# ZhengdiYu/Arbitrary-Hands-3D-Reconstruction

Hardware: AMD Instinct MI355X
Metric: frames/sec (2-hand mesh) at 512x512 batch-64; vertex L2 vs ref (higher is better)
Workload: dtype f32; 1 GPU; configs[2]: synthetic 512x512 RGB batch=64 per GPU, HRNet-W32 backbone, fp32; frames_per_gpu=64, global_batch=64, parallelism=frame-sharded x1, gather=none (one rank), contexts_in_turn=2

## Files before the change

arbitrary-hands-3d-reconstruction_amd/csrc/acrmi_ops.hip:

```cpp
#include "acrmi_ctx.h"

int decode_maps_impl(const float* l_center, const float* r_center, int center_cs, const float* l_params,
                     const float* r_params, int params_cs, const float* l_prior, const float* r_prior, int prior_cs,
                     int B, float conf_thresh, const int32_t* prior_gate, const unsigned* poison, float* slots, void* stream) {
  if (!l_center || !r_center || !l_params || !r_params || !l_prior || !r_prior || !slots || B <= 0 || params_cs < 109 ||
      prior_cs < 106 || center_cs < 1 || !(conf_thresh == conf_thresh))
    return fail(nullptr, ACRMI_EINVAL, "acrmi_decode_maps: bad arguments");
  DecodeArgs d{};
  d.center[0] = l_center; d.center[1] = r_center; d.center_cs = center_cs;
  d.params[0] = l_params; d.params[1] = r_params; d.params_cs = params_cs;
  d.prior[0] = l_prior; d.prior[1] = r_prior; d.prior_cs = prior_cs;
  d.B = B; d.slots = slots; d.thresh = conf_thresh;
  d.prior_gate = prior_gate;
  d.poison = poison;
  hipError_t e = launch_decode(d, (hipStream_t)stream);
  if (e != hipSuccess) return fail(nullptr, ACRMI_EHIP, "decode launch: %s", hipGetErrorString(e));
  return ACRMI_OK;
}

extern "C" {

int acrmi_decode_maps_gated(const float* l_center, const float* r_center, int center_cs, const float* l_params,
                            const float* r_params, int params_cs, const float* l_prior, const float* r_prior, int prior_cs,
                            int B, float conf_thresh, const int32_t* prior_gate, float* slots, void* stream) {
  return decode_maps_impl(l_center, r_center, center_cs, l_params, r_params, params_cs, l_prior, r_prior, prior_cs, B, conf_thresh,
                          prior_gate, nullptr, slots, stream);
}

int acrmi_decode_maps(const float* l_center, const float* r_center, int center_cs, const float* l_params,
                      const float* r_params, int params_cs, const float* l_prior, const float* r_prior, int prior_cs,
                      int B, float conf_thresh, float* slots, void* stream) {
  return acrmi_decode_maps_gated(l_center, r_center, center_cs, l_params, r_params, params_cs, l_prior, r_prior, prior_cs, B,
                                 conf_thresh, nullptr, slots, stream);
}

int acrmi_conv2d(const float* in, int B, int H, int W, int in_cs, int in_coff, int cin, const float* w_packed,
                 const float* bias, int bias_frame_stride, const float* res, int res_cs, int res_coff, float* out,
                 int out_cs, int out_coff, int cout, int ksize, int stride, int relu, int groups, int algo,
                 void* stream) {
  if (!in || !w_packed || !bias || !out || B <= 0 || H <= 0 || W <= 0 || cin <= 0 || cout <= 0 || groups <= 0)
    return fail(nullptr, ACRMI_EINVAL, "acrmi_conv2d: bad arguments");
  const int bias_map = algo >= 0 ? (algo & ACRMI_CONV_BIAS_MAP) : 0;
  if (algo >= 0) algo &= ~ACRMI_CONV_BIAS_MAP;
  if (bias_map && (!res || algo == 3))
    return fail(nullptr, ACRMI_EINVAL, "acrmi_conv2d: ACRMI_CONV_BIAS_MAP needs res (the map) and an algo other than 3");
  const bool x3s2 = (algo == 6 || algo == 7) && ksize == 3 && stride == 2;
  if (algo != 0 && !x3s2 && !((algo >= 1 && algo <= 7) && (ksize == 3 || (algo >= 6 && ksize == 1)) && stride == (algo == 5 ? 2 : 1)))
    return fail(nullptr, ACRMI_EINVAL, "acrmi_conv2d: algo %d needs a 3x3 stride-%d convolution", algo, algo == 5 ? 2 : 1);
  if (x3s2 && (cin % 32 || cout % 32 || H % 16 || W % 64))
    return fail(nullptr, ACRMI_EINVAL, "acrmi_conv2d: algo 6 / 7 at stride 2 needs Cin %% 32 = 0, Cout %% 32 = 0, H %% 16 == 0, W %% 64 == 0");
  if ((algo == 6 || algo == 7) && !x3s2 && (cin % 32 || cout % 32 || (ksize == 3 ? ((H % 8 || W % 32) && (H % 16 || W % 16)) : ((H * W) % 256 != 0))))
    return fail(nullptr, ACRMI_EINVAL, "acrmi_conv2d: algo 6 / 7 needs Cin %% 32 = 0, Cout %% 32 = 0, H %% 8 == 0, W %% 32 == 0");
  if (algo == 5 && (cin % 16 || cout % 32 || H % 16 || W % 32))
    return fail(nullptr, ACRMI_EINVAL, "acrmi_conv2d: algo 5 needs Cin %% 16 = 0, Cout %% 32 = 0, H %% 16 == 0, W %% 32 == 0");
  if (algo == 3 && (groups != 1 || cin > 32 || cout != 32 || bias_frame_stride != 0 || H % 8 || W % 16 || out_cs % 4 ||
                    out_coff % 4 || (res && (res_cs % 4 || res_coff % 4))))
    return fail(nullptr, ACRMI_EINVAL, "acrmi_conv2d: algo 3 needs groups 1, Cin <= 32, Cout = 32, H %% 8 == 0, W %% 16 == 0");
  if (algo == 4 && (cin < 32 || (cin == 32 && (cout % 32 || H % 8 || W % 32))))
    return fail(nullptr, ACRMI_EINVAL, "acrmi_conv2d: algo 4 needs Cin > 32 (or Cin = 32, Cout %% 32 = 0 on a map of 8x32-pixel tiles)");
  if ((ksize != 1 && ksize != 3) || (stride != 1 && stride != 2))
    return fail(nullptr, ACRMI_EINVAL, "acrmi_conv2d: only 3x3 and 1x1 at stride 1 / 2 are implemented (got k%d s%d)", ksize, stride);
  if (in_cs % 4 || in_coff % 4 || (groups > 1 && cin % 4))
    return fail(nullptr, ACRMI_EINVAL, "acrmi_conv2d: input channel stride/offset must be multiples of 4");
  if (in_coff < 0 || out_coff < 0 || res_coff < 0 || in_coff + groups * cin > in_cs || out_coff + groups * cout > out_cs ||
      (res && res_coff + groups * cout > res_cs) || bias_frame_stride < 0 ||
      (bias_frame_stride > 0 && bias_frame_stride < groups * cout))
    return fail(nullptr, ACRMI_EINVAL, "acrmi_conv2d: channel slice outside its tensor's channel stride");
  ConvArgs a{};
  a.in = in; a.w = w_packed; a.bias = bias; a.res = res; a.out = out;
  a.B = B; a.H = H; a.W = W;
  const int pad = ksize / 2;
  a.Ho = (H + 2 * pad - ksize) / stride + 1; a.Wo = (W + 2 * pad - ksize) / stride + 1;
  a.in_cs = in_cs; a.in_coff = in_coff; a.Cin = cin;
  a.out_cs = out_cs; a.out_coff = out_coff; a.Cout = cout;
  a.res_cs = res_cs; a.res_coff = res_coff;
  a.ks = ksize; a.stride = stride; a.relu = relu; a.groups = groups;
  a.cin8 = (cin + 7) / 8;
  a.n_tiles = cout <= 32 ? 1 : ((cout + 63) / 64) * 2;
  a.bias_fstride = bias_frame_stride;
  a.algo = algo;
  a.res_bcast = bias_map ? 1 : 0;
  hipError_t e = launch_conv(a, (hipStream_t)stream);
  if (e != hipSuccess) return fail(nullptr, ACRMI_EHIP, "conv launch: %s", hipGetErrorString(e));
  return ACRMI_OK;
}

size_t acrmi_conv2d_splitk_workspace(int B, int H, int W, int cout, int splits) {
  if (B <= 0 || H <= 0 || W <= 0 || cout <= 0 || splits < 2) return 0;
  const size_t cnt = (conv_splitk_counters(B, H, W, cout) * sizeof(unsigned) + 255) / 256 * 256;
  return cnt + conv_splitk_ws_floats(B, H, W, cout, splits) * sizeof(float);
}

int acrmi_conv2d_splitk(const float* in, int B, int H, int W, int in_cs, int in_coff, int cin_slice, int splits,
                        const float* w_packed, const float* bias, const float* res, int res_cs, int res_coff, float* out,
                        int out_cs, int out_coff, int cout, int relu, void* workspace, size_t workspace_bytes, void* stream) {
  if (!in || !w_packed || !bias || !out || !workspace || B <= 0 || H <= 0 || W <= 0 || cout <= 0)
    return fail(nullptr, ACRMI_EINVAL, "acrmi_conv2d_splitk: bad arguments");
  if (splits < 2 || splits > 8 || cin_slice < 64 || cin_slice % 32 || cout == 33)
    return fail(nullptr, ACRMI_EINVAL, "acrmi_conv2d_splitk: 2..8 slices of >= 64 channels (a multiple of 32) each; Cout != 33");
  if (in_cs % 4 || in_coff % 4 || in_coff < 0 || out_coff < 0 || res_coff < 0 || in_coff + splits * cin_slice > in_cs ||
      out_coff + cout > out_cs || (res && res_coff + cout > res_cs))
    return fail(nullptr, ACRMI_EINVAL, "acrmi_conv2d_splitk: channel slice outside its tensor's channel stride");
  if (workspace_bytes < acrmi_conv2d_splitk_workspace(B, H, W, cout, splits) || ((uintptr_t)workspace & 15))
    return fail(nullptr, ACRMI_EINVAL, "acrmi_conv2d_splitk: workspace too small (acrmi_conv2d_splitk_workspace) or unaligned");
  ConvArgs a{};
  a.in = in; a.w = w_packed; a.bias = bias; a.res = res; a.out = out;
  a.B = B; a.H = H; a.W = W; a.Ho = H; a.Wo = W;
  a.in_cs = in_cs; a.in_coff = in_coff; a.Cin = cin_slice;
  a.out_cs = out_cs; a.out_coff = out_coff; a.Cout = cout;
  a.res_cs = res_cs; a.res_coff = res_coff;
  a.ks = 3; a.stride = 1; a.relu = relu; a.groups = splits;
  a.cin8 = cin_slice / 8;
  a.n_tiles = cout <= 32 ? 1 : ((cout + 63) / 64) * 2;
  a.algo = 2;
  a.splitk = 1;
  a.split_cnt = reinterpret_cast<unsigned*>(workspace);
  a.split_ws = reinterpret_cast<float*>(reinterpret_cast<char*>(workspace) +
                                        (conv_splitk_counters(B, H, W, cout) * sizeof(unsigned) + 255) / 256 * 256);
  hipError_t e = launch_conv(a, (hipStream_t)stream);
  if (e != hipSuccess) return fail(nullptr, ACRMI_EHIP, "conv launch: %s", hipGetErrorString(e));
  return ACRMI_OK;
}

int acrmi_conv2d_h16(const void* in, int B, int H, int W, int in_cs, int in_coff, int cin, const void* w_packed,
                     const float* bias, int bias_frame_stride, const void* res, int res_cs, int res_coff, void* out,
                     int out_cs, int out_coff, int cout, int ksize, int stride, int relu, int groups, int dtype,
                     int out_f32, void* stream) {
  if (!in || !w_packed || !bias || !out || B <= 0 || H <= 0 || W <= 0 || cin <= 0 || cout <= 0 || groups <= 0 ||
      (dtype != ACRMI_DT_F16 && dtype != ACRMI_DT_BF16))
    return fail(nullptr, ACRMI_EINVAL, "acrmi_conv2d_h16: bad arguments");
  if ((ksize != 1 && ksize != 3) || (stride != 1 && stride != 2) || (out_f32 && stride != 1))
    return fail(nullptr, ACRMI_EINVAL, "acrmi_conv2d_h16: 3x3 and 1x1 at stride 1 / 2 (fp32 output: stride 1 only); got k%d s%d", ksize, stride);
  const int oq = out_f32 ? 4 : 8;
  if (in_cs % 8 || in_coff % 8 || (groups > 1 && cin % 8) || out_cs % oq || (res && res_cs % oq))
    return fail(nullptr, ACRMI_EINVAL, "acrmi_conv2d_h16: channel strides must be multiples of 16 bytes");
  if (in_coff < 0 || out_coff < 0 || res_coff < 0 || in_coff + groups * cin > in_cs || out_coff + groups * cout > out_cs ||
      (res && res_coff + groups * cout > res_cs) || bias_frame_stride < 0 ||
      (bias_frame_stride > 0 && bias_frame_stride < groups * cout))
    return fail(nullptr, ACRMI_EINVAL, "acrmi_conv2d_h16: channel slice outside its tensor's channel stride");
  ConvArgs a{};
  a.in = reinterpret_cast<const float*>(in); a.w = reinterpret_cast<const float*>(w_packed); a.bias = bias;
  a.res = reinterpret_cast<const float*>(res); a.out = reinterpret_cast<float*>(out);
  a.B = B; a.H = H; a.W = W;
  const int pad = ksize / 2;
  a.Ho = (H + 2 * pad - ksize) / stride + 1; a.Wo = (W + 2 * pad - ksize) / stride + 1;
  a.in_cs = in_cs; a.in_coff = in_coff; a.Cin = cin;
  a.out_cs = out_cs; a.out_coff = out_coff; a.Cout = cout;
  a.res_cs = res_cs; a.res_coff = res_coff;
  a.ks = ksize; a.stride = stride; a.relu = relu; a.groups = groups;
  a.cin8 = (cin + 15) / 16;
  a.n_tiles = cout <= 32 ? 1 : ((cout + 63) / 64) * 2;
  a.bias_fstride = bias_frame_stride;
  a.algo = 0; a.dtype = dtype; a.out_f32 = out_f32 ? 1 : 0;
  hipError_t e = launch_conv(a, (hipStream_t)stream);
  if (e != hipSuccess) return fail(nullptr, ACRMI_EHIP, "conv launch: %s", hipGetErrorString(e));
  return ACRMI_OK;
}

int acrmi_preprocess(const uint8_t* bgr_dev, int n, int H, int W, uint8_t* out_rgb_dev, float* offsets_host,
                     void* stream) {
  if (!bgr_dev || !out_rgb_dev || n <= 0 || H <= 0 || W <= 0)
    return fail(nullptr, ACRMI_EINVAL, "acrmi_preprocess: bad arguments");
  const int S = H > W ? H : W;
  int top = 0, right = 0, bottom = 0, left = 0;
  if (W < H) { const int d = H - W; right = (d + 1) / 2; left = d / 2; }
  else if (H < W) { const int d = W - H; top = d / 2; bottom = (d + 1) / 2; }
  if (offsets_host) {
    for (int i = 0; i < n; ++i) {
      float* o = offsets_host + (size_t)i * 10;
      o[0] = (float)S; o[1] = (float)S; o[2] = o[3] = o[4] = o[5] = 0.f;
      o[6] = (float)top; o[7] = (float)right; o[8] = (float)bottom; o[9] = (float)left;
    }
  }
  hipError_t e = launch_preprocess(bgr_dev, n, H, W, S, top, left, 512, out_rgb_dev, (hipStream_t)stream);
  return e == hipSuccess ? ACRMI_OK : fail(nullptr, ACRMI_EHIP, "preprocess: %s", hipGetErrorString(e));
}

int acrmi_preprocess_frames(const acrmi_frame* frames_host, int n, uint8_t* out_rgb_dev, float* offsets_host, void* stream) {
  if (!frames_host || !out_rgb_dev || n <= 0) return fail(nullptr, ACRMI_EINVAL, "acrmi_preprocess_frames: bad arguments");
  for (int i = 0; i < n; ++i)
    if (!frames_host[i].bgr_dev || frames_host[i].H <= 0 || frames_host[i].W <= 0)
      return fail(nullptr, ACRMI_EINVAL, "acrmi_preprocess_frames: frame %d: null pointer or empty size (%d x %d)", i,
                  frames_host[i].H, frames_host[i].W);
  for (int i0 = 0; i0 < n; i0 += PRE_FRAMES_PER_LAUNCH) {
    const int m = n - i0 < PRE_FRAMES_PER_LAUNCH ? n - i0 : PRE_FRAMES_PER_LAUNCH;
    PreBatch pb{};
    for (int i = 0; i < m; ++i) {
      const acrmi_frame& fr = frames_host[i0 + i];
      pb.f[i].bgr = fr.bgr_dev; pb.f[i].H = fr.H; pb.f[i].W = fr.W;
      if (offsets_host) {
        const int H = fr.H, W = fr.W, S = H > W ? H : W;
        int top = 0, right = 0, bottom = 0, left = 0;
        if (W < H) { const int d = H - W; right = (d + 1) / 2; left = d / 2; }
        else if (H < W) { const int d = W - H; top = d / 2; bottom = (d + 1) / 2; }
        float* o = offsets_host + (size_t)(i0 + i) * 10;
        o[0] = (float)S; o[1] = (float)S; o[2] = o[3] = o[4] = o[5] = 0.f;
        o[6] = (float)top; o[7] = (float)right; o[8] = (float)bottom; o[9] = (float)left;
      }
    }
    hipError_t e = launch_preprocess_frames(pb, m, 512, out_rgb_dev + (size_t)i0 * 512 * 512 * 3, (hipStream_t)stream);
    if (e != hipSuccess) return fail(nullptr, ACRMI_EHIP, "preprocess_frames: %s", hipGetErrorString(e));
  }
  return ACRMI_OK;
}

}

namespace {

const int32_t kNv12Matrix[5][6] = {
    {1220542, 2116026, -409993, -852492, 1673527, 16},
    {1220945, 2115221, -410793, -852458, 1673555, 16},
    {1048576, 1858077, -360853, -748826, 1470104, 0},
    {1220945, 2215014, -223607, -558796, 1879825, 16},
    {1048576, 1945738, -196424, -490864, 1651297, 0},
};

int nv12_coef(const char* who, const int32_t* coef6, Nv12Coef& k) {
  const int32_t* c = coef6 ? coef6 : kNv12Matrix[0];
  auto mag = [](int32_t v) { return v < 0 ? -(long long)v : (long long)v; };
  long long m = mag(c[1]);
  if (mag(c[4]) > m) m = mag(c[4]);
  if (mag(c[2]) + mag(c[3]) > m) m = mag(c[2]) + mag(c[3]);
  if (c[5] < 0 || c[5] > 255)
    return fail(nullptr, ACRMI_EINVAL, "%s: y_off %d outside 0..255", who, (int)c[5]);
  if (255 * mag(c[0]) + 128 * m + (1LL << 19) >= (1LL << 31))
    return fail(nullptr, ACRMI_EINVAL, "%s: coefficient row (%d, %d, %d, %d, %d) could overflow the int32 sums", who, (int)c[0],
                (int)c[1], (int)c[2], (int)c[3], (int)c[4]);
  k.cy = c[0]; k.cub = c[1]; k.cug = c[2]; k.cvg = c[3]; k.cvr = c[4]; k.y_off = c[5];
  return ACRMI_OK;
}

int nv12_check_frames(const char* who, const acrmi_nv12_frame* fr, int n) {
  for (int i = 0; i < n; ++i) {
    const acrmi_nv12_frame& f = fr[i];
    if (!f.y_dev || !f.uv_dev) return fail(nullptr, ACRMI_EINVAL, "%s: frame %d: null plane", who, i);
    if (f.H < 2 || f.W < 2 || (f.H & 1) || (f.W & 1))
      return fail(nullptr, ACRMI_EINVAL, "%s: frame %d: size %d x %d (H x W) must be even and >= 2", who, i, f.H, f.W);
    if (f.y_pitch < f.W || f.uv_pitch < f.W)
      return fail(nullptr, ACRMI_EINVAL, "%s: frame %d: pitch (y %d, uv %d) below the width %d", who, i, f.y_pitch, f.uv_pitch, f.W);
  }
  return ACRMI_OK;
}

}

extern "C" {

int acrmi_nv12_matrix(int which, int32_t coef6[6]) {
  if (!coef6 || which < 0 || which > ACRMI_NV12_BT709_FULL)
    return fail(nullptr, ACRMI_EINVAL, "acrmi_nv12_matrix: bad arguments (matrix %d)", which);
  for (int i = 0; i < 6; ++i) coef6[i] = kNv12Matrix[which][i];
  return ACRMI_OK;
}

int acrmi_preprocess_nv12(const acrmi_nv12_frame* frames_host, int n, const int32_t* coef6_host, uint8_t* out_rgb_dev,
                          float* offsets_host, void* stream) {
  if (!frames_host || !out_rgb_dev || n <= 0) return fail(nullptr, ACRMI_EINVAL, "acrmi_preprocess_nv12: bad arguments");
  Nv12Coef k{};
  int rc = nv12_coef("acrmi_preprocess_nv12", coef6_host, k);
  if (rc == ACRMI_OK) rc = nv12_check_frames("acrmi_preprocess_nv12", frames_host, n);
  if (rc != ACRMI_OK) return rc;
  for (int i0 = 0; i0 < n; i0 += NV12_FRAMES_PER_LAUNCH) {
    const int m = n - i0 < NV12_FRAMES_PER_LAUNCH ? n - i0 : NV12_FRAMES_PER_LAUNCH;
    Nv12Batch pb{};
    for (int i = 0; i < m; ++i) {
      const acrmi_nv12_frame& fr = frames_host[i0 + i];
      pb.f[i].y = fr.y_dev; pb.f[i].uv = fr.uv_dev; pb.f[i].H = fr.H; pb.f[i].W = fr.W;
      pb.f[i].y_pitch = fr.y_pitch; pb.f[i].uv_pitch = fr.uv_pitch;
      if (offsets_host) {
        const int H = fr.H, W = fr.W, S = H > W ? H : W;
        int top = 0, right = 0, bottom = 0, left = 0;
        if (W < H) { const int d = H - W; right = (d + 1) / 2; left = d / 2; }
        else if (H < W) { const int d = W - H; top = d / 2; bottom = (d + 1) / 2; }
        float* o = offsets_host + (size_t)(i0 + i) * 10;
        o[0] = (float)S; o[1] = (float)S; o[2] = o[3] = o[4] = o[5] = 0.f;
        o[6] = (float)top; o[7] = (float)right; o[8] = (float)bottom; o[9] = (float)left;
      }
    }
    hipError_t e = launch_preprocess_nv12(pb, k, m, 512, out_rgb_dev + (size_t)i0 * 512 * 512 * 3, (hipStream_t)stream);
    if (e != hipSuccess) return fail(nullptr, ACRMI_EHIP, "preprocess_nv12: %s", hipGetErrorString(e));
  }
  return ACRMI_OK;
}

int acrmi_nv12_to_rgb(const acrmi_nv12_frame* frames_host, int n, const int32_t* coef6_host, int bgr,
                      uint8_t* const* dst_dev_host, void* stream) {
  if (!frames_host || !dst_dev_host || n <= 0) return fail(nullptr, ACRMI_EINVAL, "acrmi_nv12_to_rgb: bad arguments");
  Nv12Coef k{};
  int rc = nv12_coef("acrmi_nv12_to_rgb", coef6_host, k);
  if (rc == ACRMI_OK) rc = nv12_check_frames("acrmi_nv12_to_rgb", frames_host, n);
  if (rc != ACRMI_OK) return rc;
  for (int i = 0; i < n; ++i)
    if (!dst_dev_host[i]) return fail(nullptr, ACRMI_EINVAL, "acrmi_nv12_to_rgb: frame %d: null destination", i);
  for (int i0 = 0; i0 < n; i0 += NV12_FRAMES_PER_LAUNCH) {
    const int m = n - i0 < NV12_FRAMES_PER_LAUNCH ? n - i0 : NV12_FRAMES_PER_LAUNCH;
    Nv12DstBatch pb{};
    for (int i = 0; i < m; ++i) {
      const acrmi_nv12_frame& fr = frames_host[i0 + i];
      pb.f[i].y = fr.y_dev; pb.f[i].uv = fr.uv_dev; pb.f[i].dst = dst_dev_host[i0 + i]; pb.f[i].H = fr.H; pb.f[i].W = fr.W;
      pb.f[i].y_pitch = fr.y_pitch; pb.f[i].uv_pitch = fr.uv_pitch;
    }
    hipError_t e = launch_nv12_to_rgb(pb, k, m, bgr ? 1 : 0, (hipStream_t)stream);
    if (e != hipSuccess) return fail(nullptr, ACRMI_EHIP, "nv12_to_rgb: %s", hipGetErrorString(e));
  }
  return ACRMI_OK;
}

int acrmi_u8norm(const uint8_t* img, int n_pixels, float* out, void* stream) {
  if (!img || !out || n_pixels <= 0) return fail(nullptr, ACRMI_EINVAL, "acrmi_u8norm: bad arguments");
  hipError_t e = launch_u8norm(img, n_pixels, out, (hipStream_t)stream);
  return e == hipSuccess ? ACRMI_OK : fail(nullptr, ACRMI_EHIP, "u8norm: %s", hipGetErrorString(e));
}

int acrmi_bilinear2x(const float* in, int B, int H, int W, int in_cs, int C, float* out, int out_cs, void* stream) {
  if (!in || !out || B <= 0 || H < 2 || W < 2 || C % 4 || in_cs % 4 || out_cs % 4)
    return fail(nullptr, ACRMI_EINVAL, "acrmi_bilinear2x: bad arguments");
  hipError_t e = launch_bilinear2x(in, B, H, W, in_cs, 0, C, out, out_cs, 0, (hipStream_t)stream);
  return e == hipSuccess ? ACRMI_OK : fail(nullptr, ACRMI_EHIP, "bilinear2x: %s", hipGetErrorString(e));
}

int acrmi_fuse_sum(int nterms, const float* const* terms, const int* term_cs, const int* term_shift, int B, int H,
                   int W, int C, float* out, int out_cs, int relu, void* stream) {
  if (nterms < 1 || nterms > 4 || !terms || !term_cs || !term_shift || !out || C % 4)
    return fail(nullptr, ACRMI_EINVAL, "acrmi_fuse_sum: bad arguments");
  FuseArgs f{};
  f.nterms = nterms; f.B = B; f.H = H; f.W = W; f.C = C; f.out = out; f.out_cs = out_cs; f.relu = relu;
  for (int t = 0; t < nterms; ++t) { f.term[t] = terms[t]; f.cs[t] = term_cs[t]; f.shift[t] = term_shift[t]; }
  hipError_t e = launch_fuse_sum(f, (hipStream_t)stream);
  return e == hipSuccess ? ACRMI_OK : fail(nullptr, ACRMI_EHIP, "fuse_sum: %s", hipGetErrorString(e));
}

int acrmi_stem_conv(const uint8_t* img, int B, int H, int W, const float* w_packed, const float* bias, float* out,
                    int out_cs, int out_coff, int relu, void* stream) {
  if (!img || !w_packed || !bias || !out || B <= 0 || !stem_shape_ok(H, W, out_cs, out_coff))
    return fail(nullptr, ACRMI_EINVAL, "acrmi_stem_conv: bad arguments (H %% 16, W %% 128, 64 channels inside out_cs)");
  hipError_t e = launch_stem(img, B, H, W, w_packed, bias, out, out_cs, out_coff, relu, (hipStream_t)stream);
  return e == hipSuccess ? ACRMI_OK : fail(nullptr, ACRMI_EHIP, "stem: %s", hipGetErrorString(e));
}

size_t acrmi_attpool_ws_floats(int B, int C) { return B > 0 && C > 0 ? attpool_ws_floats(B, C) : 0; }

int acrmi_attpool(const float* segm, int segm_cs, const float* feat, int feat_cs, int C, int B, float* ws,
                  float* pooled, void* stream) {
  if (!segm || !feat || !ws || !pooled || B <= 0) return fail(nullptr, ACRMI_EINVAL, "acrmi_attpool: bad arguments");
  hipError_t e = launch_attpool(segm, segm_cs, feat, feat_cs, C, B, 128, 128, ws, pooled, (hipStream_t)stream);
  return e == hipSuccess ? ACRMI_OK : fail(nullptr, ACRMI_EHIP, "attpool: %s", hipGetErrorString(e));
}

int acrmi_parebias(const float* pooled, int C, int part0, const float* lc_w, const float* lin_w, const float* lin_b,
                   const float* mix_wp, const float* mix_b, int B, float* out, int out_stride, void* stream) {
  if (!pooled || !lc_w || !lin_w || !lin_b || !mix_wp || !mix_b || !out || B <= 0 || (C != 256 && C != 320) ||
      (part0 != 0 && part0 != 16) || out_stride < 109 || out_stride > 256)
    return fail(nullptr, ACRMI_EINVAL, "acrmi_parebias: bad arguments");
  PareArgs a{};
  a.pooled = pooled; a.lc_w = lc_w; a.lin_w = lin_w; a.lin_b = lin_b; a.mix_wp = mix_wp; a.mix_b = mix_b;
  a.out = out; a.B = B; a.C = C; a.part0 = part0; a.out_stride = out_stride;
  hipError_t e = launch_parebias(a, (hipStream_t)stream);
  return e == hipSuccess ? ACRMI_OK : fail(nullptr, ACRMI_EHIP, "parebias: %s", hipGetErrorString(e));
}

int acrmi_cam_trans(const float* joints_dev, const float* pj2d_dev, int n, float focal_length, float img_size,
                    float* trans_dev, void* stream) {
  if (n < 0 || (n > 0 && (!joints_dev || !pj2d_dev || !trans_dev)) || !(focal_length > 0.f) || !(img_size > 0.f))
    return fail(nullptr, ACRMI_EINVAL, "acrmi_cam_trans: bad arguments");
  hipError_t e = launch_cam_trans(joints_dev, pj2d_dev, n, focal_length, img_size, trans_dev, (hipStream_t)stream);
  return e == hipSuccess ? ACRMI_OK : fail(nullptr, ACRMI_EHIP, "cam_trans: %s", hipGetErrorString(e));
}

int acrmi_mesh_topology(const int32_t* faces_host, int n_faces, int n_verts, int32_t* blob_host, int n_ints) {
  if (n_faces <= 0 || n_verts <= 0) return fail(nullptr, ACRMI_EINVAL, "acrmi_mesh_topology: bad arguments");
  const long long need = mesh_topology_ints(n_faces, n_verts);
  if (need > 0x7fffffffll) return fail(nullptr, ACRMI_EINVAL, "acrmi_mesh_topology: mesh too large");
  if (!blob_host) return (int)need;
  if (!faces_host || n_ints < need) return fail(nullptr, ACRMI_EINVAL, "acrmi_mesh_topology: bad arguments (%lld ints needed)", need);
  if (!build_mesh_topology(faces_host, n_faces, n_verts, blob_host))
    return fail(nullptr, ACRMI_EINVAL, "acrmi_mesh_topology: a face names a vertex outside [0, %d)", n_verts);
  return (int)need;
}

size_t acrmi_render_workspace(int n_meshes, int n_faces) {
  return n_meshes > 0 && n_faces > 0 ? render_workspace_bytes(n_meshes, n_faces) : 0;
}

int acrmi_rasterize(const float* verts_dev, const float* trans_dev, int n_meshes, int n_verts, int n_faces,
                    const int32_t* topo_dev, const int32_t* topo2_dev, const int32_t* mesh_topo_dev,
                    const int32_t* mesh_frame_dev, const float* rgb_dev, const float* view_dev, float focal,
                    float visible_weight, const uint8_t* img_in_dev, uint8_t* img_out_dev, int n_frames, int H, int W,
                    int32_t* ids_out_dev, void* ws_dev, void* stream) {
  if (!verts_dev || !topo_dev || !mesh_frame_dev || !rgb_dev || !img_in_dev || !img_out_dev || !ws_dev || n_meshes <= 0 ||
      n_verts <= 0 || n_verts > RENDER_MAX_VERTS || n_faces <= 0 || n_frames <= 0 || H <= 0 || W <= 0 || H > 16384 || W > 16384 ||
      (long long)n_meshes * n_faces > 0x7fffffffll || n_frames > 65535 || !(focal > 0.f) ||
      !(visible_weight >= 0.f && visible_weight <= 1.f))
    return fail(nullptr, ACRMI_EINVAL, "acrmi_rasterize: bad arguments");
  RenderArgs a{};
  a.verts = verts_dev; a.trans = trans_dev; a.topo[0] = topo_dev; a.topo[1] = topo2_dev; a.mesh_topo = mesh_topo_dev;
  a.mesh_frame = mesh_frame_dev; a.rgb = rgb_dev; a.view = view_dev; a.focal = focal; a.visible_weight = visible_weight;
  a.img_in = img_in_dev; a.img_out = img_out_dev; a.ids_out = ids_out_dev; a.ws = (char*)ws_dev;
  a.n_meshes = n_meshes; a.n_verts = n_verts; a.n_faces = n_faces; a.n_frames = n_frames; a.H = H; a.W = W;
  hipError_t e = launch_render(a, (hipStream_t)stream);
  return e == hipSuccess ? ACRMI_OK : fail(nullptr, ACRMI_EHIP, "rasterize: %s", hipGetErrorString(e));
}

int acrmi_overlay_tables(int bgr, uint8_t* colors_host, uint8_t* lut_host) {
  if (colors_host) skeleton_default_colors(bgr != 0, colors_host);
  if (lut_host) heatmap_default_lut(bgr != 0, lut_host);
  return ACRMI_OK;
}

static bool overlay_image_ok(int n, int H, int W) {
  return n > 0 && n <= OVERLAY_MAX_FRAMES && H > 0 && W > 0 && H <= OVERLAY_MAX_DIM && W <= OVERLAY_MAX_DIM;
}

int acrmi_draw_skeletons(const float* kps_dev, const int32_t* hand_frame_dev, int n_hands, const uint8_t* colors_host, int bgr,
                         int line_width, int circle_rad, const uint8_t* img_in_dev, uint8_t* img_out_dev, int n_frames, int H,
                         int W, void* stream) {
  if (!kps_dev || !hand_frame_dev || !img_in_dev || !img_out_dev || n_hands <= 0 || !overlay_image_ok(n_frames, H, W) ||
      line_width < 1 || line_width > OVERLAY_MAX_WIDTH || circle_rad < 0 || circle_rad > OVERLAY_MAX_RAD)
    return fail(nullptr, ACRMI_EINVAL, "acrmi_draw_skeletons: bad arguments (line_width 1..%d, circle_rad 0..%d, H, W <= %d)",
                OVERLAY_MAX_WIDTH, OVERLAY_MAX_RAD, OVERLAY_MAX_DIM);
  SkeletonArgs a{};
  a.kps = kps_dev; a.hand_frame = hand_frame_dev; a.n_hands = n_hands; a.n_frames = n_frames; a.H = H; a.W = W;
  a.line_width = line_width; a.circle_rad = circle_rad; a.img_in = img_in_dev; a.img_out = img_out_dev;
  if (colors_host) std::memcpy(a.colors, colors_host, 63);
  else skeleton_default_colors(bgr != 0, a.colors);
  hipError_t e = launch_skeleton(a, (hipStream_t)stream);
  return e == hipSuccess ? ACRMI_OK : fail(nullptr, ACRMI_EHIP, "draw_skeletons: %s", hipGetErrorString(e));
}

int acrmi_draw_heatmaps(const float* maps_l_dev, const float* maps_r_dev, long long frame_stride, int n, int h, int w,
                        const float* view_dev, float weight, const uint8_t* lut_host, int bgr, const uint8_t* img_in_dev,
                        uint8_t* out_l_dev, uint8_t* out_r_dev, int H, int W, void* stream) {
  if (!maps_l_dev || !img_in_dev || !out_l_dev || (maps_r_dev != nullptr) != (out_r_dev != nullptr) || out_l_dev == out_r_dev ||
      (out_r_dev && out_r_dev == img_in_dev) || !overlay_image_ok(n, H, W) || h <= 0 || w <= 0 || h > OVERLAY_MAX_DIM ||
      w > OVERLAY_MAX_DIM || frame_stride < (long long)h * w || !(weight >= 0.f && weight <= 1.f))
    return fail(nullptr, ACRMI_EINVAL, "acrmi_draw_heatmaps: bad arguments");
  HeatmapArgs a{};
  a.maps[0] = maps_l_dev; a.maps[1] = maps_r_dev; a.frame_stride = frame_stride; a.pix_stride = 1; a.dtype = ACRMI_DT_F32;
  a.n = n; a.h = h; a.w = w; a.H = H; a.W = W; a.view = view_dev; a.weight = weight; a.img_in = img_in_dev;
  a.out[0] = out_l_dev; a.out[1] = out_r_dev;
  if (lut_host) std::memcpy(a.lut, lut_host, 768);
  else heatmap_default_lut(bgr != 0, a.lut);
  hipError_t e = launch_heatmap(a, (hipStream_t)stream);
  return e == hipSuccess ? ACRMI_OK : fail(nullptr, ACRMI_EHIP, "draw_heatmaps: %s", hipGetErrorString(e));
}

}
```

arbitrary-hands-3d-reconstruction_amd/csrc/acrmi_program.hip:

```cpp
#include "acrmi_ctx.h"

void free_program(acrmi_ctx* c) {
  for (hipEvent_t e : c->op_ev)
    if (e) (void)hipEventDestroy(e);
  c->op_ev.clear();
  for (float* p : c->buf_ptr)
    if (p) (void)hipFree(p);
  c->buf_ptr.clear();
  c->bufs.clear();
  c->ops.clear();
  for (int l = 0; l < MAX_LANES; ++l) {
    if (c->split_ws[l]) (void)hipFree(c->split_ws[l]);
    if (c->split_cnt[l]) (void)hipFree(c->split_cnt[l]);
    c->split_ws[l] = nullptr; c->split_cnt[l] = nullptr;
  }
  c->split_ws_floats = c->split_counters = 0;
  if (c->att_ws) (void)hipFree(c->att_ws);
  c->att_ws = nullptr;
  if (c->picks) (void)hipFree(c->picks);
  c->picks = nullptr;
  if (c->gate_buf) (void)hipFree(c->gate_buf);
  c->gate_buf = nullptr;
  if (c->range_flag) (void)hipFree(c->range_flag);
  c->range_flag = nullptr;
  c->have_program = false;
  c->last_batch = 0;
}


int run_op(acrmi_ctx* c, const acrmi_op& op, const uint8_t* img, int B, hipStream_t s, int lane) {
  auto ptr = [&](int id) -> float* { return id >= 0 ? c->buf_ptr[id] : nullptr; };
  auto desc = [&](int id) -> const acrmi_buffer_desc& { return c->bufs[id]; };
  auto eptr = [&](int id, int coff) -> float* {
    if (id < 0) return nullptr;
    return reinterpret_cast<float*>(reinterpret_cast<char*>(c->buf_ptr[id]) + (size_t)coff * (c->bufs[id].dtype ? 2 : 4));
  };
  switch (op.kind) {
    case ACRMI_OP_U8NORM: {
      const auto& d = desc(op.out_buf);
      HIPCHK(c, launch_u8norm(img, (long)B * d.h * d.w, ptr(op.out_buf), s));
      return ACRMI_OK;
    }
    case ACRMI_OP_STEM: {
      const auto& d = desc(op.out_buf);
      if (op.ksize == 7) {
        if (d.dtype)
          HIPCHK(c, launch_stem7_h16(img, B, 2 * d.h, 2 * d.w, c->weights + op.w_off, c->weights + op.b_off, ptr(op.out_buf),
                                     d.cs, op.out_coff, op.relu, d.dtype, s));
        else
          HIPCHK(c, launch_stem7(img, B, 2 * d.h, 2 * d.w, c->weights + op.w_off, c->weights + op.b_off, ptr(op.out_buf), d.cs,
                                 op.out_coff, op.relu, s));
        return ACRMI_OK;
      }
      if (d.dtype)
        HIPCHK(c, launch_stem_h16(img, B, 2 * d.h, 2 * d.w, c->weights + op.w_off, c->weights + op.b_off, ptr(op.out_buf),
                                  d.cs, op.out_coff, op.relu, d.dtype, s));
      else
        HIPCHK(c, launch_stem(img, B, 2 * d.h, 2 * d.w, c->weights + op.w_off, c->weights + op.b_off, ptr(op.out_buf), d.cs,
                              op.out_coff, op.relu, s));
      return ACRMI_OK;
    }
    case ACRMI_OP_CONV: {
      const auto& di = desc(op.in_buf);
      const auto& dout = desc(op.out_buf);
      ConvArgs a{};
      a.in = ptr(op.in_buf);
      a.w = c->weights + op.w_off;
      a.bias = op.bias_per_frame ? ptr(op.aux_buf) : c->weights + op.b_off;
      a.res = ptr(op.res_buf);
      a.out = ptr(op.out_buf);
      a.B = B; a.H = di.h; a.W = di.w; a.Ho = dout.h; a.Wo = dout.w;
      a.in_cs = di.cs; a.in_coff = op.in_coff; a.Cin = op.cin;
      a.out_cs = dout.cs; a.out_coff = op.out_coff; a.Cout = op.cout;
      a.res_cs = op.res_buf >= 0 ? desc(op.res_buf).cs : 0; a.res_coff = op.res_coff;
      if (op.flags & ACRMI_CONV_SPLITK) {
        a.splitk = 1; a.split_ws = c->split_ws[lane]; a.split_cnt = c->split_cnt[lane];
      }
      if (op.flags & ACRMI_CONV_BIAS_MAP) {
        a.res = c->weights + op.w_off2; a.res_cs = (op.groups * op.cout + 3) / 4 * 4; a.res_coff = 0; a.res_bcast = 1;
      }
      a.ks = op.ksize; a.stride = op.stride; a.relu = op.relu; a.groups = op.groups;
      a.cin8 = (op.cin + 7) / 8;
      a.n_tiles = op.cout <= 32 ? 1 : ((op.cout + 63) / 64) * 2;
      a.bias_fstride = op.bias_per_frame ? desc(op.aux_buf).cs : 0;
      a.nxt = op.nterms;
      for (int t = 0; t < op.nterms && t < 3; ++t) {
        a.xt[t] = ptr(op.term_buf[t]);
        a.xt_cs[t] = desc(op.term_buf[t]).cs; a.xt_coff[t] = op.term_coff[t]; a.xt_shift[t] = op.term_shift[t];
      }
      if (op.flags & ACRMI_CONV_DUAL) {
        a.out2 = ptr(op.aux_buf); a.out2_cs = desc(op.aux_buf).cs; a.out2_coff = 0;
      }
      a.algo = op.flags & 7;
      a.range_flag = a.algo == 6 ? c->range_flag : nullptr;
      a.dtype = di.dtype;
      a.out_f32 = di.dtype != ACRMI_DT_F32 && dout.dtype == ACRMI_DT_F32;
      HIPCHK(c, launch_conv(a, s));
      return ACRMI_OK;
    }
    case ACRMI_OP_FUSESUM: {
      const auto& dout = desc(op.out_buf);
      FuseArgs f{};
      f.nterms = op.nterms; f.B = B; f.H = dout.h; f.W = dout.w; f.C = op.cout; f.out_cs = dout.cs; f.relu = op.relu;
      f.out = eptr(op.out_buf, op.out_coff);
      for (int t = 0; t < op.nterms; ++t) {
        f.term[t] = eptr(op.term_buf[t], op.term_coff[t]);
        f.cs[t] = desc(op.term_buf[t]).cs;
        f.shift[t] = op.term_shift[t];
      }
      if (dout.dtype) HIPCHK(c, launch_fuse_sum_h16(f, dout.dtype, s));
      else HIPCHK(c, launch_fuse_sum(f, s));
      return ACRMI_OK;
    }
    case ACRMI_OP_BILINEAR2X: {
      const auto& di = desc(op.in_buf);
      if (di.dtype)
        HIPCHK(c, launch_bilinear2x_h16(ptr(op.in_buf), B, di.h, di.w, di.cs, op.in_coff, op.cin, ptr(op.out_buf),
                                        desc(op.out_buf).cs, op.out_coff, di.dtype, s));
      else
        HIPCHK(c, launch_bilinear2x(ptr(op.in_buf), B, di.h, di.w, di.cs, op.in_coff, op.cin, ptr(op.out_buf),
                                    desc(op.out_buf).cs, op.out_coff, s));
      return ACRMI_OK;
    }
    case ACRMI_OP_PAIR1X1: {
      const auto& di = desc(op.in_buf);
      HIPCHK(c, launch_pair1x1(ptr(op.in_buf), di.cs, op.in_coff, ptr(op.res_buf), desc(op.res_buf).cs, op.res_coff, ptr(op.out_buf),
                               desc(op.out_buf).cs, op.out_coff, ptr(op.aux_buf), desc(op.aux_buf).cs, 0, c->weights + op.w_off,
                               (long)B * di.h * di.w, s));
      return ACRMI_OK;
    }
    case ACRMI_OP_MAXPOOL: {
      const auto& di = desc(op.in_buf);
      if (di.dtype)
        HIPCHK(c, launch_maxpool3s2_h16(ptr(op.in_buf), B, di.h, di.w, di.cs, op.in_coff, op.cin, ptr(op.out_buf),
                                        desc(op.out_buf).cs, op.out_coff, di.dtype, s));
      else
        HIPCHK(c, launch_maxpool3s2(ptr(op.in_buf), B, di.h, di.w, di.cs, op.in_coff, op.cin, ptr(op.out_buf),
                                    desc(op.out_buf).cs, op.out_coff, s));
      return ACRMI_OK;
    }
    case ACRMI_OP_POW11: {
      const auto& d = desc(op.out_buf);
      if (d.dtype) HIPCHK(c, launch_pow11_h16(ptr(op.out_buf), (long)B * d.h * d.w, d.cs, op.out_coff, d.dtype, s));
      else HIPCHK(c, launch_pow11(ptr(op.out_buf), (long)B * d.h * d.w, d.cs, op.out_coff, s));
      return ACRMI_OK;
    }
    case ACRMI_OP_ATTPOOL: {
      const auto& ds = desc(op.in_buf);
      const auto& df = desc(op.res_buf);
      HIPCHK(c, launch_attpool(ptr(op.in_buf), ds.cs, eptr(op.res_buf, op.res_coff), df.cs, op.cin, B, df.h, df.w,
                               c->att_ws, ptr(op.out_buf), s, df.dtype));
      return ACRMI_OK;
    }
    case ACRMI_OP_PAREBIAS: {
      PareArgs p{};
      p.pooled = ptr(op.in_buf);
      p.lc_w = c->weights + op.w_off;
      p.lin_w = c->weights + op.w_off2;
      p.lin_b = c->weights + op.b_off2;
      p.mix_wp = c->weights + op.w_off3;
      p.mix_b = c->weights + op.b_off;
      p.out = ptr(op.out_buf);
      p.B = B; p.C = op.cin; p.part0 = op.flags; p.out_stride = desc(op.out_buf).cs;
      HIPCHK(c, launch_parebias(p, s));
      return ACRMI_OK;
    }
    case ACRMI_OP_COORDFILL: {
      const auto& d = desc(op.out_buf);
      if (d.dtype) HIPCHK(c, launch_coordfill_h16(ptr(op.out_buf), c->max_batch, d.h, d.w, d.cs, op.out_coff, d.dtype, s));
      else HIPCHK(c, launch_coordfill(ptr(op.out_buf), c->max_batch, d.h, d.w, d.cs, op.out_coff, s));
      return ACRMI_OK;
    }
    case ACRMI_OP_POINTHEADS: {
      const acrmi_head_layout& h = c->heads;
      const int side = op.flags & 1;
      PointArgs p{};
      p.x34 = ptr(op.in_buf); p.x_cs = desc(op.in_buf).cs;
      p.center[0] = ptr(h.center_buf[0]); p.center[1] = ptr(h.center_buf[1]); p.center_cs = desc(h.center_buf[0]).cs;
      p.w = c->weights + op.w_off;
      p.mix_w = c->weights + op.w_off2;
      p.bias = ptr(op.aux_buf); p.bias_stride = desc(op.aux_buf).cs;
      p.p109 = ptr(op.res_buf); p.p109_cs = desc(op.res_buf).cs;
      p.prior = ptr(h.prior_buf[side]); p.prior_cs = desc(h.prior_buf[side]).cs;
      p.final_ = ptr(op.out_buf); p.final_cs = desc(op.out_buf).cs;
      p.picks = c->picks; p.side = side; p.B = B; p.thresh = c->conf_thresh;
      p.prior_when_both = c->batch_prior ? 1 : 0;
      HIPCHK(c, launch_point_heads(p, s));
      return ACRMI_OK;
    }
    default:
      return fail(c, ACRMI_EINVAL, "unknown op kind %d", op.kind);
  }
}

bool op_active(const acrmi_op& op, bool point) {
  return op.kind != ACRMI_OP_COORDFILL && op.mode != (point ? ACRMI_MODE_DENSE : ACRMI_MODE_POINT);
}

static void op_rw(const acrmi_ctx* c, const acrmi_op& op, std::vector<int>& R, std::vector<int>& W) {
  R.clear(); W.clear();
  const int n_bufs = (int)c->bufs.size();
  auto r = [&](int id) { if (id >= 0) R.push_back(id); };
  auto w = [&](int id) { if (id >= 0) W.push_back(id); };
  switch (op.kind) {
    case ACRMI_OP_U8NORM: case ACRMI_OP_STEM: w(op.out_buf); break;
    case ACRMI_OP_CONV:
      r(op.in_buf); r(op.res_buf); if (op.bias_per_frame) r(op.aux_buf);
      for (int t = 0; t < op.nterms; ++t) r(op.term_buf[t]);
      w(op.out_buf);
      if (op.flags & ACRMI_CONV_DUAL) w(op.aux_buf);
      break;
    case ACRMI_OP_FUSESUM: for (int t = 0; t < op.nterms; ++t) r(op.term_buf[t]); w(op.out_buf); break;
    case ACRMI_OP_BILINEAR2X: case ACRMI_OP_MAXPOOL: r(op.in_buf); w(op.out_buf); break;
    case ACRMI_OP_PAIR1X1: r(op.in_buf); r(op.res_buf); w(op.out_buf); w(op.aux_buf); break;
    case ACRMI_OP_POW11: r(op.out_buf); w(op.out_buf); break;
    case ACRMI_OP_ATTPOOL: r(op.in_buf); r(op.res_buf); w(op.out_buf); w(n_bufs); break;
    case ACRMI_OP_PAREBIAS: r(op.in_buf); w(op.out_buf); break;
    case ACRMI_OP_POINTHEADS:
      r(op.in_buf); r(op.aux_buf); r(c->heads.center_buf[0]); r(c->heads.center_buf[1]);
      w(op.res_buf); w(op.out_buf); w(c->heads.prior_buf[op.flags & 1]); w(n_bufs + 1);
      break;
    default: break;
  }
}

void build_schedule(acrmi_ctx* c, bool point, bool large) {
  Schedule& S = c->sched[point ? 1 : 0][large ? 1 : 0];
  const int n = (int)c->ops.size(), nb = (int)c->bufs.size() + 2;
  S = Schedule();
  S.deps.assign(n, std::vector<int>());
  S.leaf.assign(n, 1);
  std::vector<int> last_writer(nb, -1), R, W;
  std::vector<std::vector<int>> readers(nb);
  for (int j = 0; j < n; ++j) {
    if (!op_active(c->ops[j], point)) continue;
    S.order.push_back(j);
    op_rw(c, c->ops[j], R, W);
    std::vector<int>& deps = S.deps[j];
    auto dep = [&](int i) { if (i >= 0 && i != j && std::find(deps.begin(), deps.end(), i) == deps.end()) deps.push_back(i); };
    for (int b : R) dep(last_writer[b]);
    for (int b : W) { dep(last_writer[b]); for (int i : readers[b]) dep(i); }
    for (int b : R) readers[b].push_back(j);
    for (int b : W) { last_writer[b] = j; readers[b].clear(); }
    for (int d : deps) S.leaf[d] = 0;
  }
  const int want = c->want_lanes > 0 ? c->want_lanes : (large ? AUTO_LANES_LARGE : AUTO_LANES_SMALL);
  const int max_lanes = std::max(1, std::min(want, MAX_LANES));
  S.lane.assign(n, 0);
  S.wait.assign(n, std::vector<int>());
  S.signal.assign(n, 0);
  std::vector<int> lane_tail(max_lanes, -1);
  const std::vector<float>& ms = c->op_ms[point ? 1 : 0];
  const bool planned = c->lane_plan && !large && max_lanes > 1 && (int)ms.size() == n;
  constexpr float SYNC_MS = 0.002f, EVENT_MS = 0.002f;
  static const float WAIT_MS = experiment_env("ACRMI_PLAN_WAIT_US") ? 1e-3f * (float)atof(experiment_env("ACRMI_PLAN_WAIT_US")) : 0.016f;
  std::vector<float> fin(planned ? n : 0, 0.f), lane_free(max_lanes, 0.f);
  static const bool rank_order = !(experiment_env("ACRMI_PLAN_RANK") && atoi(experiment_env("ACRMI_PLAN_RANK")) == 0);
  if (planned && rank_order) {
    std::vector<float> ru(n, 0.f);
    std::vector<std::vector<int>> succ(n);
    for (int j : S.order)
      for (int d : S.deps[j]) succ[d].push_back(j);
    for (int k = (int)S.order.size() - 1; k >= 0; --k) {
      const int j = S.order[k];
      float m = 0.f;
      for (int s2 : succ[j]) m = std::max(m, ru[s2]);
      ru[j] = m + std::max(ms[j], 1e-4f);
    }
    std::stable_sort(S.order.begin(), S.order.end(), [&](int x, int y) { return ru[x] > ru[y]; });
  }
  std::vector<int> pos(n, -1);
  for (int k = 0; k < (int)S.order.size(); ++k) pos[S.order[k]] = k;
  for (int j : S.order) {
    int lane = -1;
    if (planned) {
      float best = 0.f;
      bool best_prod = false;
      for (int l = 0; l < max_lanes; ++l) {
        float start = lane_free[l];
        unsigned others = 0;
        bool prod = false;
        for (int d : S.deps[j]) {
          if (S.lane[d] == l) { prod = true; continue; }
          others |= 1u << S.lane[d];
          start = std::max(start, fin[d] + WAIT_MS);
        }
        start += SYNC_MS * (float)__builtin_popcount(others);
        if (lane < 0 || start < best - 1e-6f || (start < best + 1e-6f && prod && !best_prod)) { lane = l; best = start; best_prod = prod; }
      }
      fin[j] = best + std::max(ms[j] - EVENT_MS, 0.002f);
      lane_free[lane] = fin[j] + 0.5f * SYNC_MS;
      S.n_lanes = std::max(S.n_lanes, lane + 1);
    } else {
      for (int d : S.deps[j])
        if (lane_tail[S.lane[d]] == d) { lane = S.lane[d]; break; }
      if (lane < 0) {
        if (S.n_lanes < max_lanes) lane = S.n_lanes++;
        else lane = (int)(std::min_element(lane_tail.begin(), lane_tail.end()) - lane_tail.begin());
      }
    }
    S.lane[j] = lane;
    std::vector<int> latest(max_lanes, -1);
    for (int d : S.deps[j])
      if (S.lane[d] != lane && (latest[S.lane[d]] < 0 || pos[d] > pos[latest[S.lane[d]]])) latest[S.lane[d]] = d;
    for (int l = 0; l < max_lanes; ++l)
      if (latest[l] >= 0) { S.wait[j].push_back(latest[l]); S.signal[latest[l]] = 1; }
    lane_tail[lane] = j;
  }
  if (getenv("ACRMI_DEBUG_SCHED")) {
    std::vector<int> depth(n, 0);
    int edges = 0, maxd = 0;
    for (int j : S.order) {
      for (int d : S.deps[j]) depth[j] = std::max(depth[j], depth[d] + 1);
      edges += (int)S.deps[j].size();
      maxd = std::max(maxd, depth[j] + 1);
    }
    int waits = 0;
    for (int j : S.order) waits += (int)S.wait[j].size();
    fprintf(stderr, "[acrmi] schedule(%s, %s batches, %s): %zu ops, %d edges, critical path %d ops; %d lanes, %d cross-lane waits\n",
            point ? "point" : "dense", large ? "large" : "small", planned ? "planned from measured op times" : "structural",
            S.order.size(), edges, maxd, S.n_lanes, waits);
  }
}


extern "C" {

int acrmi_set_program(acrmi_ctx* c, const acrmi_buffer_desc* bufs, int n_bufs, const acrmi_op* ops, int n_ops,
                      const acrmi_head_layout* heads, int max_batch) {
  if (!c || !bufs || !ops || !heads || n_bufs <= 0 || n_ops <= 0 || max_batch <= 0)
    return fail(c, ACRMI_EINVAL, "acrmi_set_program: bad arguments");
  if (!c->weights) return fail(c, ACRMI_ESTATE, "acrmi_set_program: load weights first");
  ON_DEVICE(c);
  int prog_dt = ACRMI_DT_F32;
  for (int i = 0; i < n_bufs; ++i) {
    const auto& d = bufs[i];
    if (d.dtype < ACRMI_DT_F32 || d.dtype > ACRMI_DT_BF16) return fail(c, ACRMI_EINVAL, "buffer %d: unknown dtype %d", i, d.dtype);
    if (d.h <= 0 || d.w <= 0 || d.cs <= 0 || d.cs % (d.dtype ? 8 : 4)) return fail(c, ACRMI_EINVAL, "buffer %d: bad geometry", i);
    if (d.dtype) {
      if (prog_dt && prog_dt != d.dtype) return fail(c, ACRMI_EINVAL, "buffer %d: f16 and bf16 buffers in one program", i);
      prog_dt = d.dtype;
    }
  }
  auto bdt = [&](int id) { return id >= 0 ? bufs[id].dtype : (int)ACRMI_DT_F32; };
  auto buf_ok = [&](int id) { return id >= 0 && id < n_bufs; };
  auto w_ok = [&](long long off, long long n) { return off >= 0 && n >= 0 && (unsigned long long)(off + n) <= c->n_weights; };
  {
    const int hb[8] = {heads->center_buf[0], heads->center_buf[1], heads->params_buf[0], heads->params_buf[1],
                       heads->prior_buf[0], heads->prior_buf[1], heads->segm_buf, heads->backbone_buf};
    for (int id : hb)
      if (!buf_ok(id)) return fail(c, ACRMI_EINVAL, "head layout references buffer %d of %d", id, n_bufs);
    for (int k = 0; k < 7; ++k)
      if (bufs[hb[k]].dtype != ACRMI_DT_F32) return fail(c, ACRMI_EINVAL, "head layout: head maps must be fp32 buffers");
    if (bufs[heads->params_buf[0]].cs < 109 || bufs[heads->params_buf[1]].cs < 109 || bufs[heads->prior_buf[0]].cs < 106 ||
        bufs[heads->prior_buf[1]].cs < 106)
      return fail(c, ACRMI_EINVAL, "head layout: params/prior buffers are too narrow");
    for (int k = 0; k < 6; ++k)
      if (bufs[hb[k]].h != 64 || bufs[hb[k]].w != 64) return fail(c, ACRMI_EINVAL, "head layout: head maps must be 64x64");
  }
  for (int i = 0; i < n_ops; ++i) {
    const acrmi_op& op = ops[i];
    const int ids[4] = {op.in_buf, op.out_buf, op.res_buf, op.aux_buf};
    for (int id : ids)
      if (id >= n_bufs || id < -1) return fail(c, ACRMI_EINVAL, "op %d references buffer %d of %d", i, id, n_bufs);
    if (op.mode < ACRMI_MODE_BOTH || op.mode > ACRMI_MODE_POINT) return fail(c, ACRMI_EINVAL, "op %d: bad mode", i);
    bool need_in = false, need_out = true;
    switch (op.kind) {
      case ACRMI_OP_U8NORM: case ACRMI_OP_POW11: case ACRMI_OP_COORDFILL: case ACRMI_OP_STEM: break;
      case ACRMI_OP_CONV: case ACRMI_OP_BILINEAR2X: case ACRMI_OP_MAXPOOL: case ACRMI_OP_PAIR1X1: case ACRMI_OP_ATTPOOL: case ACRMI_OP_PAREBIAS: case ACRMI_OP_POINTHEADS:
        need_in = true;
        break;
      case ACRMI_OP_FUSESUM: break;
      default: return fail(c, ACRMI_EINVAL, "op %d: unknown kind %d", i, op.kind);
    }
    if ((need_in && !buf_ok(op.in_buf)) || (need_out && !buf_ok(op.out_buf)))
      return fail(c, ACRMI_EINVAL, "op %d (kind %d): missing input/output buffer", i, op.kind);
    if (op.in_coff < 0 || op.out_coff < 0 || op.res_coff < 0) return fail(c, ACRMI_EINVAL, "op %d: negative channel offset", i);
    if (op.kind == ACRMI_OP_CONV) {
      const int idt = bufs[op.in_buf].dtype, odt = bufs[op.out_buf].dtype;
      if (op.in_coff % (idt ? 8 : 4) || (op.ksize != 1 && op.ksize != 3) || op.stride < 1 || op.stride > 2 || op.cin <= 0 || op.cout <= 0 ||
          op.groups <= 0)
        return fail(c, ACRMI_EINVAL, "op %d: unsupported conv geometry", i);
      const int algo = op.flags & 7;
      if (algo > 7) return fail(c, ACRMI_EINVAL, "op %d: unknown conv algo %d", i, algo);
      if (idt ? (algo != 0 || (odt != idt && odt != ACRMI_DT_F32) || (odt == ACRMI_DT_F32 && op.stride != 1) ||
                 (op.groups > 1 && op.cin % 2))
              : odt != ACRMI_DT_F32)
        return fail(c, ACRMI_EINVAL, "op %d: conv buffer types do not fit (in %d, out %d, algo %d)", i, idt, odt, algo);
      if (op.res_buf >= 0 && bufs[op.res_buf].dtype != odt)
        return fail(c, ACRMI_EINVAL, "op %d: the residual must have the type of the output", i);
      const bool splitk = (op.flags & ACRMI_CONV_SPLITK) != 0;
      if (splitk && (algo != 2 || idt || op.groups < 2 || op.groups > 8 || op.cin % 32 || op.cin < 64 || op.cout == 33 ||
                     op.bias_per_frame))
        return fail(c, ACRMI_EINVAL, "op %d: split-K needs algo 2, fp32, 2..8 slices of Cin %% 32 == 0, Cin >= 64 channels each", i);
      if (op.flags & ACRMI_CONV_BIAS_MAP) {
        const long long mcs = (op.groups * op.cout + 3) / 4 * 4;
        if (splitk || op.res_buf >= 0 || idt || algo == 3 || !w_ok(op.w_off2, (long long)bufs[op.out_buf].h * bufs[op.out_buf].w * mcs))
          return fail(c, ACRMI_EINVAL, "op %d: a position-bias map needs an fp32 conv without a residual buffer (not algo 3) and "
                      "[Ho][Wo][round4(groups*Cout)] floats inside the blob at w_off2", i);
      }
      const bool dual = (op.flags & ACRMI_CONV_DUAL) != 0;
      if (dual && (algo != 3 || op.nterms < 1 || op.bias_per_frame || !buf_ok(op.aux_buf) || bufs[op.aux_buf].dtype != ACRMI_DT_F32 ||
                   bufs[op.aux_buf].h != bufs[op.out_buf].h || bufs[op.aux_buf].w != bufs[op.out_buf].w || bufs[op.aux_buf].cs % 4 ||
                   bufs[op.aux_buf].cs < op.cout || op.aux_buf == op.out_buf || op.aux_buf == op.in_buf || op.aux_buf == op.res_buf))
        return fail(c, ACRMI_EINVAL, "op %d: a second output needs algo 3, 1..3 terms and an fp32 map of the output's size in aux_buf", i);
      if (op.nterms) {
        const int ho_ = bufs[op.out_buf].h, wo_ = bufs[op.out_buf].w;
        if (op.nterms < 0 || op.nterms > 3 || idt || (op.flags & ACRMI_CONV_BIAS_MAP) || splitk ||
            (dual ? false : (op.ksize != 3 || op.stride != 2 || (algo != 0 && algo != 5) || op.cout % 32 || op.cin <= 16 ||
                             op.out_coff % 4 || bufs[op.out_buf].cs % 4)))
          return fail(c, ACRMI_EINVAL, "op %d: extra residual terms need an fp32 3x3 stride-2 convolution (algo 0 / 5) with Cin > 16, "
                      "Cout %% 32 = 0 and 16-byte aligned output channels - or ACRMI_CONV_DUAL", i);
        for (int t = 0; t < op.nterms; ++t) {
          const int tb = op.term_buf[t];
          if (!buf_ok(tb) || bufs[tb].dtype != ACRMI_DT_F32 || op.term_coff[t] < 0 || op.term_coff[t] % 4 || bufs[tb].cs % 4 ||
              op.term_shift[t] < 0 || op.term_shift[t] > 3 || op.term_coff[t] + op.groups * op.cout > bufs[tb].cs ||
              (bufs[tb].h << op.term_shift[t]) != ho_ || (bufs[tb].w << op.term_shift[t]) != wo_ || tb == op.out_buf ||
              (dual && tb == op.aux_buf))
            return fail(c, ACRMI_EINVAL, "op %d: residual term %d does not fit the output", i, t);
        }
      }
      if (op.bias_per_frame && buf_ok(op.aux_buf) && bufs[op.aux_buf].dtype != ACRMI_DT_F32)
        return fail(c, ACRMI_EINVAL, "op %d: the per-frame bias must be fp32", i);
      if (algo != 0 && !((algo == 6 || algo == 7) && op.ksize == 3 && op.stride == 2) &&
          !((op.ksize == 3 || (algo >= 6 && op.ksize == 1)) && op.stride == (algo == 5 ? 2 : 1)))
        return fail(c, ACRMI_EINVAL, "op %d: algo %d needs a 3x3 stride-%d convolution", i, algo, algo == 5 ? 2 : 1);
      if (algo == 3 && (op.groups != 1 || op.cin > 32 || op.cout != 32 || op.bias_per_frame || bufs[op.out_buf].h % 8 ||
                        bufs[op.out_buf].w % 16 || op.out_coff % 4 || op.res_coff % 4))
        return fail(c, ACRMI_EINVAL, "op %d: algo 3 needs groups 1, Cin <= 32, Cout = 32, a map of 8x16-pixel tiles", i);
      const int ogroups = splitk ? 1 : op.groups;
      if (op.in_coff + op.groups * op.cin > bufs[op.in_buf].cs || op.out_coff + ogroups * op.cout > bufs[op.out_buf].cs ||
          (op.res_buf >= 0 && op.res_coff + ogroups * op.cout > bufs[op.res_buf].cs) ||
          (op.groups > 1 && op.cin % (bufs[op.in_buf].dtype == ACRMI_DT_F32 ? 4 : 8)))
        return fail(c, ACRMI_EINVAL, "op %d: channel slice outside its buffer's channel stride", i);
      const int pad = op.ksize / 2;
      const int ho = (bufs[op.in_buf].h + 2 * pad - op.ksize) / op.stride + 1, wo = (bufs[op.in_buf].w + 2 * pad - op.ksize) / op.stride + 1;
      if (ho != bufs[op.out_buf].h || wo != bufs[op.out_buf].w ||
          (op.res_buf >= 0 && (bufs[op.res_buf].h != ho || bufs[op.res_buf].w != wo)))
        return fail(c, ACRMI_EINVAL, "op %d: output/residual buffer geometry does not match the convolution", i);
      const long long n_tiles = op.cout <= 32 ? 1 : ((op.cout + 63) / 64) * 2;
      if (algo == 4 && (op.cin < 32 || (op.cin == 32 && (op.cout % 32 || ho % 8 || wo % 32))))
        return fail(c, ACRMI_EINVAL, "op %d: algo 4 needs Cin > 32, or Cin = 32 with Cout %% 32 = 0 on a map of 8x32-pixel tiles", i);
      if ((algo == 6 || algo == 7) && op.stride == 2 &&
          (op.ksize != 3 || ho % 8 || wo % 32 || bufs[op.in_buf].h != 2 * ho || bufs[op.in_buf].w != 2 * wo || op.nterms > 0))
        return fail(c, ACRMI_EINVAL, "op %d: algo 6 / 7 at stride 2 needs a 3x3 convolution onto a map of 8x32-pixel tiles, even input size, no extra residual terms", i);
      if ((algo == 6 || algo == 7) && (idt || op.cin % 32 || op.cout % 32 || op.out_coff % 4 || op.res_coff % 4 ||
                                       (op.ksize == 3 ? ((ho % 8 || wo % 32) && (ho % 16 || wo % 16)) : ((ho * wo) % 256 != 0))))
        return fail(c, ACRMI_EINVAL, "op %d: algo 6 / 7 needs fp32 storage, Cin %% 32 = 0, Cout %% 32 = 0, a map of 8x32- or 16x16-pixel tiles (3x3) / of whole 256-pixel items (1x1)", i);
      if (algo == 5 && (idt || op.cin % 16 || op.cout % 32 || bufs[op.in_buf].h % 2 || bufs[op.in_buf].w % 2 || ho % 8 || wo % 16 ||
                        op.out_coff % 4 || op.res_coff % 4))
        return fail(c, ACRMI_EINVAL, "op %d: algo 5 needs fp32, Cin %% 16 = 0, Cout %% 32 = 0, an output map of 8x16-pixel tiles", i);
      const long long taps = algo >= 6 ? op.ksize * op.ksize : algo == 5 ? 28 : algo == 4 ? 24 : (algo >= 2 ? 16 : (algo == 1 ? 12 : op.ksize * op.ksize));
      const long long ksteps = idt ? (op.cin + 15) / 16 : (op.cin + 7) / 8;
      const long long wn = algo == 3 ? 16384 : (long long)op.groups * taps * ksteps * n_tiles * 256 + (algo >= 6 ? 1 : 0);
      if (!w_ok(op.w_off, wn)) return fail(c, ACRMI_EINVAL, "op %d: packed weights outside the blob", i);
      if (op.bias_per_frame) {
        if (!buf_ok(op.aux_buf) || bufs[op.aux_buf].cs < op.groups * op.cout)
          return fail(c, ACRMI_EINVAL, "op %d: per-frame bias buffer missing or too narrow", i);
      } else if (!w_ok(op.b_off, (long long)op.groups * n_tiles * 32)) {
        return fail(c, ACRMI_EINVAL, "op %d: bias outside the blob", i);
      }
    }
    if (op.kind == ACRMI_OP_STEM) {
      if (bufs[op.out_buf].dtype && (bufs[op.out_buf].cs % 8 || op.out_coff % 8))
        return fail(c, ACRMI_EINVAL, "op %d: a 16-bit stem output needs channel stride / offset in multiples of 8", i);
      if (op.ksize != 3 && op.ksize != 7) return fail(c, ACRMI_EINVAL, "op %d: the stem kernels are 3x3 and 7x7 (stride 2)", i);
      const bool ok = op.ksize == 7 ? stem7_shape_ok(2 * bufs[op.out_buf].h, 2 * bufs[op.out_buf].w, bufs[op.out_buf].cs, op.out_coff)
                                    : stem_shape_ok(2 * bufs[op.out_buf].h, 2 * bufs[op.out_buf].w, bufs[op.out_buf].cs, op.out_coff);
      if (op.cout != 64 || !ok)
        return fail(c, ACRMI_EINVAL, "op %d: the stem kernel needs 64 output channels and a map of 8x64-pixel strips", i);
      if (!w_ok(op.w_off, (op.ksize == 7 ? 74 : 14) * 2 * 64) || !w_ok(op.b_off, 64))
        return fail(c, ACRMI_EINVAL, "op %d: stem weights outside the blob", i);
    }
    if (op.kind == ACRMI_OP_FUSESUM) {
      const int vq = bufs[op.out_buf].dtype ? 8 : 4;
      if (op.nterms < 1 || op.nterms > 4 || op.cout <= 0 || op.cout % vq || op.out_coff % vq || op.out_coff + op.cout > bufs[op.out_buf].cs)
        return fail(c, ACRMI_EINVAL, "op %d: bad fuse-sum geometry", i);
      for (int t = 0; t < op.nterms; ++t) {
        if (!buf_ok(op.term_buf[t]) || op.term_coff[t] < 0 || bufs[op.term_buf[t]].dtype != bufs[op.out_buf].dtype ||
            op.term_coff[t] % vq || op.term_shift[t] < 0 || op.term_shift[t] > 3 ||
            op.term_coff[t] + op.cout > bufs[op.term_buf[t]].cs ||
            (bufs[op.term_buf[t]].h << op.term_shift[t]) != bufs[op.out_buf].h ||
            (bufs[op.term_buf[t]].w << op.term_shift[t]) != bufs[op.out_buf].w)
          return fail(c, ACRMI_EINVAL, "op %d: fuse-sum term %d does not fit the output", i, t);
      }
    }
    if (op.kind == ACRMI_OP_PAIR1X1) {
      if (!buf_ok(op.res_buf) || !buf_ok(op.aux_buf) || op.cin != 64 || op.cout != 256)
        return fail(c, ACRMI_EINVAL, "op %d: the 1x1 pair is 64 -> 256 (+ residual) -> 64 with in, res, out and aux buffers", i);
      const int ids4[4] = {op.in_buf, op.res_buf, op.out_buf, op.aux_buf};
      for (int id : ids4)
        if (bufs[id].dtype != ACRMI_DT_F32 || bufs[id].h != bufs[op.in_buf].h || bufs[id].w != bufs[op.in_buf].w)
          return fail(c, ACRMI_EINVAL, "op %d: the 1x1 pair's buffers must be fp32 maps of one size", i);
      if (op.in_coff % 4 || op.res_coff % 4 || op.out_coff % 4 || op.in_coff + 64 > bufs[op.in_buf].cs ||
          op.res_coff + 256 > bufs[op.res_buf].cs || op.out_coff + 256 > bufs[op.out_buf].cs || bufs[op.aux_buf].cs < 64 ||
          op.out_buf == op.in_buf || op.aux_buf == op.in_buf || op.aux_buf == op.out_buf || op.aux_buf == op.res_buf)
        return fail(c, ACRMI_EINVAL, "op %d: the 1x1 pair's channel slices do not fit / its buffers alias", i);
      if (!w_ok(op.w_off, PAIR1X1_FLOATS)) return fail(c, ACRMI_EINVAL, "op %d: pair weights outside the blob", i);
    }
    if (op.kind == ACRMI_OP_MAXPOOL) {
      const int vq = bufs[op.in_buf].dtype ? 8 : 4;
      if (op.cin <= 0 || bufs[op.in_buf].dtype != bufs[op.out_buf].dtype || op.cin % vq || op.in_coff % vq || op.out_coff % vq ||
          op.in_coff + op.cin > bufs[op.in_buf].cs || op.out_coff + op.cin > bufs[op.out_buf].cs ||
          bufs[op.out_buf].h != (bufs[op.in_buf].h - 1) / 2 + 1 || bufs[op.out_buf].w != (bufs[op.in_buf].w - 1) / 2 + 1)
        return fail(c, ACRMI_EINVAL, "op %d: bad max-pool geometry", i);
    }
    if (op.kind == ACRMI_OP_BILINEAR2X &&
        (op.cin <= 0 || bufs[op.in_buf].dtype != bufs[op.out_buf].dtype || op.cin % (bufs[op.in_buf].dtype ? 8 : 4) ||
         op.in_coff % (bufs[op.in_buf].dtype ? 8 : 4) || op.out_coff % (bufs[op.in_buf].dtype ? 8 : 4) || op.in_coff + op.cin > bufs[op.in_buf].cs ||
         op.out_coff + op.cin > bufs[op.out_buf].cs || bufs[op.out_buf].h != 2 * bufs[op.in_buf].h ||
         bufs[op.out_buf].w != 2 * bufs[op.in_buf].w))
      return fail(c, ACRMI_EINVAL, "op %d: bad bilinear geometry", i);
    if ((op.kind == ACRMI_OP_POW11 && op.out_coff >= bufs[op.out_buf].cs) ||
        (op.kind == ACRMI_OP_COORDFILL && op.out_coff + 2 > bufs[op.out_buf].cs))
      return fail(c, ACRMI_EINVAL, "op %d: channel outside the buffer", i);
    if (op.kind == ACRMI_OP_ATTPOOL) {
      if (buf_ok(op.res_buf) && (bufs[op.in_buf].dtype != ACRMI_DT_F32 || bufs[op.out_buf].dtype != ACRMI_DT_F32 ||
                                 (bufs[op.res_buf].dtype != ACRMI_DT_F32 && op.cin != 256)))
        return fail(c, ACRMI_EINVAL, "op %d: attention pooling reads fp32 logits, writes fp32, and pools 256 channels of a 16-bit map", i);
      if (!buf_ok(op.res_buf) || (op.cin != 32 && op.cin != 64 && op.cin != 256 && op.cin != 320) ||
          op.res_coff + op.cin > bufs[op.res_buf].cs || bufs[op.in_buf].cs < 33 || bufs[op.in_buf].h != 2 * bufs[op.res_buf].h ||
          bufs[op.in_buf].w != 2 * bufs[op.res_buf].w || (long long)bufs[op.out_buf].h * bufs[op.out_buf].w * bufs[op.out_buf].cs < 32LL * op.cin)
        return fail(c, ACRMI_EINVAL, "op %d: bad attention-pool geometry", i);
    }
    if ((op.kind == ACRMI_OP_PAREBIAS || op.kind == ACRMI_OP_POINTHEADS || op.kind == ACRMI_OP_U8NORM) &&
        (bdt(op.in_buf) || bdt(op.out_buf) || bdt(op.res_buf) || bdt(op.aux_buf)))
      return fail(c, ACRMI_EINVAL, "op %d (kind %d): fp32 buffers only", i, op.kind);
    if (op.kind == ACRMI_OP_PAREBIAS) {
      const long long shape_n = (op.cin == 320 ? 64 : 256) * 16;
      if ((op.cin != 256 && op.cin != 320) || (op.flags != 0 && op.flags != 16) || bufs[op.out_buf].cs < 109 || bufs[op.out_buf].cs > 256 ||
          (long long)bufs[op.in_buf].h * bufs[op.in_buf].w * bufs[op.in_buf].cs < 32LL * op.cin || !w_ok(op.w_off, 6 * 256 * 16) ||
          !w_ok(op.w_off2, 10 * shape_n) || !w_ok(op.b_off2, 10) || !w_ok(op.w_off3, 109 * 106) || !w_ok(op.b_off, 109))
        return fail(c, ACRMI_EINVAL, "op %d: bad pare-bias geometry or weights", i);
    }
    if (op.kind == ACRMI_OP_POINTHEADS) {
      const bool ok = buf_ok(op.res_buf) && buf_ok(op.aux_buf) &&
                      bufs[op.in_buf].h == 128 && bufs[op.in_buf].w == 128 && bufs[op.in_buf].cs == 36 &&
                      bufs[op.res_buf].h == 64 && bufs[op.out_buf].h == 64 && bufs[op.res_buf].cs >= 109 &&
                      bufs[op.out_buf].cs >= 109 && bufs[op.aux_buf].cs >= 109 && op.mode == ACRMI_MODE_POINT &&
                      w_ok(op.w_off, 3LL * TP_TOWER_FLOATS) && w_ok(op.w_off2, 109LL * TP_EXIT_N);
      if (!ok) return fail(c, ACRMI_EINVAL, "op %d: unsupported point-heads geometry", i);
    }
  }
  free_program(c);
  c->bufs.assign(bufs, bufs + n_bufs);
  c->ops.assign(ops, ops + n_ops);
  c->heads = *heads;
  c->max_batch = max_batch;
  c->buf_ptr.assign(n_bufs, nullptr);
  for (int i = 0; i < n_bufs; ++i) {
    const auto& d = bufs[i];
    const size_t bytes = (size_t)max_batch * d.h * d.w * d.cs * (d.dtype ? 2 : sizeof(float));
    hipError_t e = hipMalloc(&c->buf_ptr[i], bytes);
    if (e != hipSuccess) return fail(c, ACRMI_ENOMEM, "hipMalloc(%zu) for buffer %d: %s", bytes, i, hipGetErrorString(e));
    HIPCHK(c, hipMemset(c->buf_ptr[i], 0, bytes));
  }
  for (int i = 0; i < n_ops; ++i) {
    const acrmi_op& op = ops[i];
    if (op.kind != ACRMI_OP_CONV || !(op.flags & ACRMI_CONV_SPLITK)) continue;
    const auto& d = bufs[op.out_buf];
    c->split_ws_floats = std::max(c->split_ws_floats, conv_splitk_ws_floats(max_batch, d.h, d.w, op.cout, op.groups));
    c->split_counters = std::max(c->split_counters, conv_splitk_counters(max_batch, d.h, d.w, op.cout));
  }
  if (c->split_ws_floats)
    for (int l = 0; l < MAX_LANES; ++l) {
      HIPCHK(c, hipMalloc(&c->split_ws[l], c->split_ws_floats * sizeof(float)));
      HIPCHK(c, hipMalloc(&c->split_cnt[l], c->split_counters * sizeof(unsigned)));
      HIPCHK(c, hipMemset(c->split_cnt[l], 0, c->split_counters * sizeof(unsigned)));
    }
  c->att_ws_floats = attpool_ws_floats(max_batch, 320);
  HIPCHK(c, hipMalloc(&c->att_ws, c->att_ws_floats * sizeof(float)));
  HIPCHK(c, hipMalloc(&c->picks, (size_t)max_batch * 4 * sizeof(int)));
  HIPCHK(c, hipMalloc(&c->gate_buf, (size_t)max_batch * sizeof(int)));
  for (int i = 0; i < n_ops; ++i)
    if (ops[i].kind == ACRMI_OP_CONV && (ops[i].flags & 7) == 6 && !c->range_flag) {
      HIPCHK(c, hipMalloc(&c->range_flag, sizeof(unsigned)));
      HIPCHK(c, hipMemset(c->range_flag, 0, sizeof(unsigned)));
    }
  c->op_ms[0].clear(); c->op_ms[1].clear();
  for (int v = 0; v < 4; ++v) build_schedule(c, v & 1, v & 2);
  c->op_ev.assign(n_ops, nullptr);
  c->have_program = true;
  for (const acrmi_op& op : c->ops)
    if (op.kind == ACRMI_OP_COORDFILL) {
      int r = run_op(c, op, nullptr, max_batch, nullptr);
      if (r) return r;
    }
  HIPCHK(c, hipDeviceSynchronize());
  return ACRMI_OK;
}

}

static unsigned lane_event_flags() {
  static const unsigned f = [] {
    const char* e = experiment_env("ACRMI_EVENT_FLAGS");
    if (e) fprintf(stderr, "[acrmi] WARNING: ACRMI_EVENT_FLAGS=%s - lane events created with non-default flags (experiment)\n", e);
    return hipEventDisableTiming | (e ? (unsigned)strtoul(e, nullptr, 16) : 0u);
  }();
  return f;
}

static int run_program_lanes(acrmi_ctx* c, const uint8_t* img, int B, hipStream_t user, bool point) {
  const Schedule& S = c->sched[point ? 1 : 0][B > AUTO_SMALL_BATCH ? 1 : 0];
  for (int l = 1; l < S.n_lanes; ++l) {
    if (!c->lanes[l]) HIPCHK(c, hipStreamCreateWithFlags(&c->lanes[l], hipStreamNonBlocking));
    if (!c->join_ev[l]) HIPCHK(c, hipEventCreateWithFlags(&c->join_ev[l], lane_event_flags()));
  }
  if (!c->fork_ev) HIPCHK(c, hipEventCreateWithFlags(&c->fork_ev, lane_event_flags()));
  auto st = [&](int l) { return l == 0 ? user : c->lanes[l]; };
  HIPCHK(c, hipEventRecord(c->fork_ev, user));
  for (int l = 1; l < S.n_lanes; ++l) HIPCHK(c, hipStreamWaitEvent(c->lanes[l], c->fork_ev, 0));
  int r = ACRMI_OK;
  for (int j : S.order) {
    hipStream_t s = st(S.lane[j]);
    static const int ablate = [] {
      const char* e = experiment_env("ACRMI_ABLATE_LANE_SYNC");
      const int v = e ? atoi(e) : 0;
      if (v) fprintf(stderr, "[acrmi] WARNING: ACRMI_ABLATE_LANE_SYNC=%d - cross-lane synchronisation is DISABLED, results are WRONG "
                             "(timing experiment only)\n", v);
      return v;
    }();
    if (!(ablate & 1)) for (int d : S.wait[j]) HIPCHK(c, hipStreamWaitEvent(s, c->op_ev[d], 0));
    r = run_op(c, c->ops[j], img, B, s, S.lane[j]);
    if (r) break;
    if (S.signal[j] && !(ablate & 2)) {
      if (!c->op_ev[j]) HIPCHK(c, hipEventCreateWithFlags(&c->op_ev[j], lane_event_flags()));
      HIPCHK(c, hipEventRecord(c->op_ev[j], s));
    }
  }
  for (int l = 1; l < S.n_lanes; ++l) {
    HIPCHK(c, hipEventRecord(c->join_ev[l], c->lanes[l]));
    HIPCHK(c, hipStreamWaitEvent(user, c->join_ev[l], 0));
  }
  return r;
}

int run_program(acrmi_ctx* c, const uint8_t* img, int B, void* stream, bool point, int first_op) {
  if (!c || (!img && first_op <= 0)) return fail(c, ACRMI_EINVAL, "acrmi_backbone_heads: bad arguments");
  if (!c->have_program) return fail(c, ACRMI_ESTATE, "acrmi_backbone_heads: no program");
  if (B <= 0 || B > c->max_batch) return fail(c, ACRMI_EINVAL, "batch %d outside 1..%d", B, c->max_batch);
  ON_DEVICE(c);
  c->last_batch = B;
  static const bool dbg_sync = getenv("ACRMI_DEBUG_SYNC") != nullptr;
  if (c->sched[point ? 1 : 0][B > AUTO_SMALL_BATCH ? 1 : 0].n_lanes > 1 && !dbg_sync && first_op <= 0)
    return run_program_lanes(c, img, B, (hipStream_t)stream, point);
  int i = 0;
  for (const acrmi_op& op : c->ops) {
    ++i;
    if (!op_active(op, point) || i - 1 < first_op) continue;
    if (dbg_sync) fprintf(stderr, "[acrmi] op %d kind %d B %d\n", i - 1, (int)op.kind, B), fflush(stderr);
    int r = run_op(c, op, img, B, (hipStream_t)stream);
    if (r) return r;
    if (dbg_sync) HIPCHK(c, hipStreamSynchronize((hipStream_t)stream));
  }
  return ACRMI_OK;
}
```

arbitrary-hands-3d-reconstruction_amd/csrc/conv_wino3.inc:

```
template <int TH, bool DUAL = false>
__device__ __forceinline__ void wino3_store_waves(const ConvArgs& a, const ConvWork& wk, const float* stage, int sw, int lane,
                                                  int my_items, int vb) {
  constexpr int TW = 16, STILE = TH * TW * 32, NI = TH * TW / 8 / 2;
  const int pin = lane >> 3, q = lane & 7;
  const unsigned lane_out = (unsigned)(pin * a.out_cs + 4 * q) * 4u;
  const unsigned lane_out2 = (unsigned)(pin * a.out2_cs + 4 * q) * 4u;
  int soff[NI];
#pragma unroll
  for (int i = 0; i < NI; ++i) {
    const int t = sw * NI + i, row = t >> 1, col = 8 * (t & 1) + pin;
    soff[i] = (row * TW + col) * 32 + 4 * (q ^ (((col >> 1) + 4 * ((row >> 1) & 1)) & 7));
  }
  f32x4 tv[DUAL ? 3 : 1][NI];
  auto request_terms = [&](int kk) {
    if constexpr (DUAL) {
      const ItemPos ip = item_pos(wk, vb + kk * (int)gridDim.x);
#pragma unroll
      for (int tt = 0; tt < 3; ++tt) {
        const bool on = tt < a.nxt;
        const int sh = on ? a.xt_shift[tt] : 0, cs = on ? a.xt_cs[tt] : 4;
        const int hs = a.Ho >> sh, wsx = a.Wo >> sh;
        const size_t off = (size_t)ip.b * hs * wsx * cs + (on ? a.xt_coff[tt] : 0);
        const size_t left = on ? ((size_t)a.B * hs * wsx * cs - off) * 4 : 0;
        const __amdgpu_buffer_rsrc_t xr = __builtin_amdgcn_make_buffer_rsrc(
            const_cast<float*>(on ? a.xt[tt] + off : a.in), 0, (int)(unsigned)(left > 0xffffffffu ? 0xffffffffu : left), 0x00020000);
        unsigned xo[2];
#pragma unroll
        for (int hp = 0; hp < 2; ++hp) xo[hp] = (unsigned)((((ip.tx * TW + 8 * hp + pin) >> sh) * cs + 4 * q) * 4);
#pragma unroll
        for (int i = 0; i < NI; ++i) {
          const int t = sw * NI + i;
          const int so = (((ip.ty * TH + (t >> 1)) >> sh) * wsx) * cs * 4;
          tv[tt][i] = __builtin_bit_cast(f32x4, __builtin_amdgcn_raw_buffer_load_b128(xr, xo[t & 1], so, 0));
        }
      }
    }
  };
  auto flush = [&](int kk) {
    const ItemPos ip = item_pos(wk, vb + kk * (int)gridDim.x);
    const size_t tile_pix = ((size_t)ip.b * a.Ho + (size_t)ip.ty * TH) * a.Wo + (size_t)ip.tx * TW;
    float* out_tile = a.out + tile_pix * a.out_cs + a.out_coff;
    const float* st = stage + (kk & 1) * STILE;
    f32x4 v[NI];
#pragma unroll
    for (int i = 0; i < NI; ++i) v[i] = *reinterpret_cast<const f32x4*>(st + soff[i]);
#pragma unroll
    for (int i = 0; i < NI; ++i) {
      const int t = sw * NI + i;
      char* ub = reinterpret_cast<char*>(out_tile + ((t >> 1) * a.Wo + 8 * (t & 1)) * a.out_cs);
      __builtin_nontemporal_store(v[i], reinterpret_cast<f32x4*>(ub + lane_out));
    }
    if constexpr (DUAL) {
      float* out2_tile = a.out2 + tile_pix * a.out2_cs + a.out2_coff;
#pragma unroll
      for (int i = 0; i < NI; ++i) {
        const int t = sw * NI + i;
        f32x4 y = ((v[i] + tv[0][i]) + tv[1][i]) + tv[2][i];
        y[0] = vrelu1(y[0]); y[1] = vrelu1(y[1]); y[2] = vrelu1(y[2]); y[3] = vrelu1(y[3]);
        char* ub = reinterpret_cast<char*>(out2_tile + ((t >> 1) * a.Wo + 8 * (t & 1)) * a.out2_cs);
        __builtin_nontemporal_store(y, reinterpret_cast<f32x4*>(ub + lane_out2));
      }
    }
  };
  if (my_items >= 1) request_terms(0);
  __syncthreads();
  for (int k = 0; k < my_items; ++k) {
    __syncthreads();
    if (k >= 1) {
      flush(k - 1);
      request_terms(k);
    }
  }
  __syncthreads();
  if (my_items >= 1) flush(my_items - 1);
}

#ifndef ACRMI_W3_ABLATE
#define ACRMI_W3_ABLATE 0
#endif
template <int TH, int NLW, bool PIPE, int LPRIO = 0, bool DMA = false, int NSW = 0, bool DUAL = false>
__global__ __launch_bounds__((TH / 2 + NLW + NSW) * 64, 1) void conv_wino3_kernel(const ConvArgs a, const ConvWork wk) {
  constexpr int W3_ABLATE = ACRMI_W3_ABLATE;
  static_assert(!DUAL || NSW == 2, "the second output is written by the store waves");
  constexpr int TW = 16, PH = TH + 2, PW = TW + 2, CK = 32, CP = CK + 4;
  constexpr int NCW = TH / 2;
  constexpr int RAWBUF = PH * PW * CP;
  constexpr int WFLOATS = 16 * 2 * 2 * 256;
  constexpr int STILE = TH * TW * 32;
  static_assert(NSW == 0 || (NSW == 2 && TH == 8), "store waves: two, 8x16-pixel items");
  extern __shared__ f32x4 smem4[];
  float* lds = reinterpret_cast<float*>(smem4);
  float* wlds = lds + 2 * RAWBUF;
  float* stage = wlds + WFLOATS;

  const int tid = threadIdx.x, lane = tid & 63;
  const int wave = __builtin_amdgcn_readfirstlane(tid >> 6);
  const int cin_pad = a.cin8 * 8;
  const int vb = virtual_block(a);
  const int my_items = wk.total > vb ? (wk.total - 1 - vb) / (int)gridDim.x + 1 : 0;
  if constexpr (NSW > 0) {
    if (wave >= NCW + NLW) {
      wino3_store_waves<TH, DUAL>(a, wk, stage, wave - NCW - NLW, lane, my_items, vb);
      return;
    }
  }
  if (wave >= NCW) {
    if constexpr (DMA) dma_loader<3, 1, TH, TW, CK, NLW>(a, wk, lds, tid - NCW * 64, my_items, 1, vb);
    else ws_loader<3, 1, TH, TW, CK, NLW, NoHook, false, LPRIO>(a, wk, lds, tid - NCW * 64, my_items, cin_pad);
    if constexpr (NSW > 0) __syncthreads();
    return;
  }
  {
    const f32x4* src = reinterpret_cast<const f32x4*>(a.w);
    f32x4* dst = reinterpret_cast<f32x4*>(wlds);
    constexpr int PER = WFLOATS / 4 / (NCW * 64);
    f32x4 tmp[PER];
#pragma unroll
    for (int i = 0; i < PER; ++i) tmp[i] = src[tid + i * NCW * 64];
#pragma unroll
    for (int i = 0; i < PER; ++i) dst[tid + i * NCW * 64] = tmp[i];
  }
  const int ch = wave & 1, sg = wave >> 1;
  const int j = lane & 15, kq = lane >> 4;
  const int in_a = (j < 4) || (j >= 12);
  const int brow = in_a ? 0 : 1;
  const int bcol = in_a ? (j < 4 ? j : j - 8) : j - 4;
  const int by = 2 * sg + brow;
  const int worg = ((2 * by) * PW + 2 * bcol) * CP + 4 * kq;
  const float* wfrag = wlds + ch * 256 + lane * 4;
  const bool has_res = a.res != nullptr;
  const int lane_pix = (2 * by) * a.Wo + 2 * bcol;
  const unsigned lane_out = (unsigned)(lane_pix * a.out_cs + 16 * ch + 4 * kq) * 4u;
  const unsigned lane_res = (unsigned)(lane_pix * a.res_cs + 16 * ch + 4 * kq) * 4u;
  const f32x4 bias4 = *reinterpret_cast<const f32x4*>(a.bias + 16 * ch + 4 * kq);
  const int stage_off = ((2 * by) * TW + 2 * bcol) * 32 + 4 * ((4 * ch + kq) ^ ((bcol + 4 * brow) & 7));

  typedef float f32x2 __attribute__((ext_vector_type(2)));
  auto pk_add4 = [](const f32x4& b, const f32x4& c) -> f32x4 {
    f32x2 lo, hi;
    const f32x2 b0 = {b[0], b[1]}, b1 = {b[2], b[3]}, c0 = {c[0], c[1]}, c1 = {c[2], c[3]};
    asm("v_pk_add_f32 %0, %1, %2" : "=v"(lo) : "v"(b0), "v"(c0));
    asm("v_pk_add_f32 %0, %1, %2" : "=v"(hi) : "v"(b1), "v"(c1));
    return f32x4{lo[0], lo[1], hi[0], hi[1]};
  };
  auto pk_sub4 = [](const f32x4& b, const f32x4& c) -> f32x4 {
    f32x2 lo, hi;
    const f32x2 b0 = {b[0], b[1]}, b1 = {b[2], b[3]}, c0 = {c[0], c[1]}, c1 = {c[2], c[3]};
    asm("v_pk_add_f32 %0, %1, %2 neg_lo:[0,1] neg_hi:[0,1]" : "=v"(lo) : "v"(b0), "v"(c0));
    asm("v_pk_add_f32 %0, %1, %2 neg_lo:[0,1] neg_hi:[0,1]" : "=v"(hi) : "v"(b1), "v"(c1));
    return f32x4{lo[0], lo[1], hi[0], hi[1]};
  };
  auto bt4 = [&](f32x4& x0, f32x4& x1, f32x4& x2, f32x4& x3) {
    x0 = pk_sub4(x0, x2);
    x3 = pk_sub4(x1, x3);
    const f32x4 t = pk_add4(x1, x2);
    x2 = pk_sub4(x2, x1);
    x1 = t;
  };
  f32x4 acc[16];
  f32x4 va[16], vb_[16];
  f32x4 wr[4];
  f32x4 rv[4];

  auto read_column = [&](f32x4 (&d)[16], const float* patch, int s, int wx) {
    if (W3_ABLATE & 2) return;
#pragma unroll
    for (int wy = 0; wy < 4; ++wy)
      d[wy * 4 + wx] = *reinterpret_cast<const f32x4*>(patch + worg + (wy * PW + wx) * CP + 16 * s);
  };
  auto read_window = [&](f32x4 (&d)[16], const float* patch, int s) {
#pragma unroll
    for (int wx = 0; wx < 4; ++wx) read_column(d, patch, s, wx);
  };
  auto transform_piece = [&](f32x4 (&d)[16], int piece) {
    if (W3_ABLATE & 1) return;
    if (piece < 4) bt4(d[piece], d[4 + piece], d[8 + piece], d[12 + piece]);
    else bt4(d[(piece - 4) * 4], d[(piece - 4) * 4 + 1], d[(piece - 4) * 4 + 2], d[(piece - 4) * 4 + 3]);
  };
  auto ring_load = [&](int g) {
    if ((W3_ABLATE & 4) && g > 1) return;
    const int gg = g & 15, s = gg >> 3, p0 = (gg & 7) * 2;
    wr[(g & 1) * 2] = *reinterpret_cast<const f32x4*>(wfrag + (p0 * 2 + s) * 512);
    wr[(g & 1) * 2 + 1] = *reinterpret_cast<const f32x4*>(wfrag + ((p0 + 1) * 2 + s) * 512);
  };
  auto mfma_step = [&](int s, const f32x4 (&v)[16], auto zero_tag, auto between) {
    constexpr bool ZERO = decltype(zero_tag)::value;
#pragma unroll
    for (int pr = 0; pr < 8; ++pr) {
      __builtin_amdgcn_sched_barrier(0);
      const int g = s * 8 + pr;
      ring_load(g + 1);
      __builtin_amdgcn_sched_barrier(0);
#pragma unroll
      for (int e = 0; e < 4; ++e)
#pragma unroll
        for (int h = 0; h < 2; ++h) {
          const int pos = 2 * pr + h;
          const float wv = wr[(g & 1) * 2 + h][e];
          if (ZERO && e == 0) {
            const f32x4 zero = {0.f, 0.f, 0.f, 0.f};
            acc[pos] = __builtin_amdgcn_mfma_f32_16x16x4f32(wv, v[pos][e], zero, 0, 0, 0);
          } else {
            acc[pos] = __builtin_amdgcn_mfma_f32_16x16x4f32(wv, v[pos][e], acc[pos], 0, 0, 0);
          }
        }
      __builtin_amdgcn_sched_barrier(0);
      between(pr);
    }
  };

  const bool stamp = a.dbg && blockIdx.x == 0 && tid == 0;
  int ns_ = 0;
  if (stamp) a.dbg[ns_++] = clock64();
  __syncthreads();
  if (my_items > 0) {
    ring_load(0);
    read_window(va, lds, 0);
#pragma unroll
    for (int p = 0; p < 8; ++p) transform_piece(va, p);
    if (PIPE) read_column(vb_, lds, 1, 0);
  }
  int w = vb;
  for (int k = 0; k < my_items; ++k, w += (int)gridDim.x) {
    if (stamp && ns_ < 60) a.dbg[ns_++] = clock64();
    const float* patch = lds + (k & 1) * RAWBUF;
    const float* patch_next = k + 1 < my_items ? lds + ((k + 1) & 1) * RAWBUF : patch;
    const ItemPos ip = item_pos(wk, w);
    const size_t tile_pix = ((size_t)ip.b * a.Ho + (size_t)ip.ty * TH) * a.Wo + (size_t)ip.tx * TW;
    float* out_tile = a.out + tile_pix * a.out_cs + a.out_coff;
    auto request_res = [&]() {
      if (has_res) {
        const float* res_tile = a.res + tile_pix * a.res_cs + a.res_coff;
#pragma unroll
        for (int q = 0; q < 4; ++q) {
          const char* ub = reinterpret_cast<const char*>(res_tile + ((q >> 1) * a.Wo + (q & 1)) * a.res_cs);
          rv[q] = __builtin_nontemporal_load(reinterpret_cast<const f32x4*>(ub + lane_res));
        }
      }
    };
    if (PIPE) request_res();
    if (PIPE) {
      mfma_step(0, va, std::true_type(), [&](int pr) {
        if (pr < 3) read_column(vb_, patch, 1, pr + 1);
        transform_piece(vb_, pr);
      });
    } else {
      mfma_step(0, va, std::true_type(), [&](int) {});
      read_window(vb_, patch, 1);
#pragma unroll
      for (int p = 0; p < 8; ++p) transform_piece(vb_, p);
    }
    __builtin_amdgcn_sched_barrier(0);
    if (stamp && ns_ < 60) a.dbg[ns_++] = clock64();
    __syncthreads();
    if (stamp && ns_ < 60) a.dbg[ns_++] = clock64();
    if (PIPE) {
      read_column(va, patch_next, 0, 0);
      mfma_step(1, vb_, std::false_type(), [&](int pr) {
        if (pr < 3) read_column(va, patch_next, 0, pr + 1);
        transform_piece(va, pr);
        if (pr == 7) read_column(vb_, patch_next, 1, 0);
      });
    } else {
      mfma_step(1, vb_, std::false_type(), [&](int) {});
    }
    __builtin_amdgcn_sched_barrier(0);
    if (stamp && ns_ < 60) a.dbg[ns_++] = clock64();
    {
      if (!PIPE) request_res();
      f32x4 r0[4], r1[4];
#pragma unroll
      for (int py = 0; py < 4; ++py) {
        r0[py] = pk_add4(pk_add4(acc[py * 4], acc[py * 4 + 1]), acc[py * 4 + 2]);
        r1[py] = pk_sub4(pk_sub4(acc[py * 4 + 1], acc[py * 4 + 2]), acc[py * 4 + 3]);
      }
      f32x4 y[4];
      y[0] = pk_add4(pk_add4(r0[0], r0[1]), r0[2]);
      y[1] = pk_add4(pk_add4(r1[0], r1[1]), r1[2]);
      y[2] = pk_sub4(pk_sub4(r0[1], r0[2]), r0[3]);
      y[3] = pk_sub4(pk_sub4(r1[1], r1[2]), r1[3]);
#pragma unroll
      for (int q = 0; q < 4; ++q) {
        f32x4 o4 = pk_add4(y[q], bias4);
        if (has_res) o4 = pk_add4(o4, rv[q]);
        if (a.relu) {
          o4[0] = vrelu1(o4[0]); o4[1] = vrelu1(o4[1]); o4[2] = vrelu1(o4[2]); o4[3] = vrelu1(o4[3]);
        }
        if constexpr (NSW > 0) {
          *reinterpret_cast<f32x4*>(stage + (k & 1) * STILE + stage_off + ((q >> 1) * TW + (q & 1)) * 32) = o4;
        } else {
          char* ub = reinterpret_cast<char*>(out_tile + ((q >> 1) * a.Wo + (q & 1)) * a.out_cs);
          __builtin_nontemporal_store(o4, reinterpret_cast<f32x4*>(ub + lane_out));
        }
      }
    }
    __builtin_amdgcn_sched_barrier(0);
    if (!PIPE) {
      read_window(va, patch_next, 0);
#pragma unroll
      for (int p = 0; p < 8; ++p) transform_piece(va, p);
    }
    __builtin_amdgcn_sched_barrier(0);
    if (stamp && ns_ < 60) a.dbg[ns_++] = clock64();
  }
  if constexpr (NSW > 0) __syncthreads();
  if (stamp) a.dbg[63] = ns_;
}

template <int NLW, bool DMA, bool RES>
__global__ __launch_bounds__((4 + NLW) * 64, 1) void conv_wino3b_kernel(const ConvArgs a, const ConvWork wk) {
  constexpr int TH = 16, TW = 16, PH = TH + 2, PW = TW + 2, CK = 32, CP = CK + 4, NCW = 4;
  constexpr int RAWBUF = PH * PW * CP;
  constexpr int WFLOATS = 16 * 2 * 2 * 256;
  extern __shared__ f32x4 smem4[];
  float* lds = reinterpret_cast<float*>(smem4);
  float* wlds = lds + 2 * RAWBUF;

  const int tid = threadIdx.x, lane = tid & 63;
  const int wave = __builtin_amdgcn_readfirstlane(tid >> 6);
  const int cin_pad = a.cin8 * 8;
  const int vb = virtual_block(a);
  const int my_items = wk.total > vb ? (wk.total - 1 - vb) / (int)gridDim.x + 1 : 0;
  if (wave >= NCW) {
    if constexpr (DMA) dma_loader<3, 1, TH, TW, CK, NLW>(a, wk, lds, tid - NCW * 64, my_items, 1, vb);
    else ws_loader<3, 1, TH, TW, CK, NLW, NoHook, false, 3>(a, wk, lds, tid - NCW * 64, my_items, cin_pad);
    return;
  }
  {
    const f32x4* src = reinterpret_cast<const f32x4*>(a.w);
    f32x4* dst = reinterpret_cast<f32x4*>(wlds);
    constexpr int PER = WFLOATS / 4 / (NCW * 64);
    f32x4 tmp[PER];
#pragma unroll
    for (int i = 0; i < PER; ++i) tmp[i] = src[tid + i * NCW * 64];
#pragma unroll
    for (int i = 0; i < PER; ++i) dst[tid + i * NCW * 64] = tmp[i];
  }
  const int sg = wave;
  const int j = lane & 15, kq = lane >> 4;
  const int in_a = (j < 4) || (j >= 12);
  const int brow = in_a ? 0 : 1;
  const int bcol = in_a ? (j < 4 ? j : j - 8) : j - 4;
  const int by = 2 * sg + brow;
  const int worg = ((2 * by) * PW + 2 * bcol) * CP + 4 * kq;
  const float* wfrag = wlds + lane * 4;
  constexpr bool has_res = RES;
  const int lane_pix = (2 * by) * a.Wo + 2 * bcol;
  const unsigned lane_out = (unsigned)(lane_pix * a.out_cs + 4 * kq) * 4u;
  const unsigned lane_res = (unsigned)(lane_pix * a.res_cs + 4 * kq) * 4u;

  typedef float f32x2 __attribute__((ext_vector_type(2)));
  auto pk_add4 = [](const f32x4& b, const f32x4& c) -> f32x4 {
    f32x2 lo, hi;
    const f32x2 b0 = {b[0], b[1]}, b1 = {b[2], b[3]}, c0 = {c[0], c[1]}, c1 = {c[2], c[3]};
    asm("v_pk_add_f32 %0, %1, %2" : "=v"(lo) : "v"(b0), "v"(c0));
    asm("v_pk_add_f32 %0, %1, %2" : "=v"(hi) : "v"(b1), "v"(c1));
    return f32x4{lo[0], lo[1], hi[0], hi[1]};
  };
  auto pk_sub4 = [](const f32x4& b, const f32x4& c) -> f32x4 {
    f32x2 lo, hi;
    const f32x2 b0 = {b[0], b[1]}, b1 = {b[2], b[3]}, c0 = {c[0], c[1]}, c1 = {c[2], c[3]};
    asm("v_pk_add_f32 %0, %1, %2 neg_lo:[0,1] neg_hi:[0,1]" : "=v"(lo) : "v"(b0), "v"(c0));
    asm("v_pk_add_f32 %0, %1, %2 neg_lo:[0,1] neg_hi:[0,1]" : "=v"(hi) : "v"(b1), "v"(c1));
    return f32x4{lo[0], lo[1], hi[0], hi[1]};
  };
  auto bt4 = [&](f32x4& x0, f32x4& x1, f32x4& x2, f32x4& x3) {
    x0 = pk_sub4(x0, x2);
    x3 = pk_sub4(x1, x3);
    const f32x4 t = pk_add4(x1, x2);
    x2 = pk_sub4(x2, x1);
    x1 = t;
  };
  f32x4 acc[16][2];
  f32x4 va[16], vb_[16];
  f32x4 wr[8];

  auto read_column = [&](f32x4 (&d)[16], const float* patch, int s, int wx) {
#pragma unroll
    for (int wy = 0; wy < 4; ++wy)
      d[wy * 4 + wx] = *reinterpret_cast<const f32x4*>(patch + worg + (wy * PW + wx) * CP + 16 * s);
  };
  auto transform_piece = [&](f32x4 (&d)[16], int piece) {
    if (piece < 4) bt4(d[piece], d[4 + piece], d[8 + piece], d[12 + piece]);
    else bt4(d[(piece - 4) * 4], d[(piece - 4) * 4 + 1], d[(piece - 4) * 4 + 2], d[(piece - 4) * 4 + 3]);
  };
  auto ring_load = [&](int g) {
    const int gg = g & 15, s = gg >> 3, p0 = (gg & 7) * 2;
#pragma unroll
    for (int h2 = 0; h2 < 2; ++h2)
#pragma unroll
      for (int h = 0; h < 2; ++h)
        wr[(g & 1) * 4 + h2 * 2 + h] = *reinterpret_cast<const f32x4*>(wfrag + (((p0 + h2) * 2 + s) * 2 + h) * 256);
  };
  auto mfma_step = [&](int s, const f32x4 (&v)[16], auto zero_tag, auto between) {
    constexpr bool ZERO = decltype(zero_tag)::value;
#pragma unroll
    for (int pr = 0; pr < 8; ++pr) {
      __builtin_amdgcn_sched_barrier(0);
      const int g = s * 8 + pr;
      ring_load(g + 1);
      __builtin_amdgcn_sched_barrier(0);
#pragma unroll
      for (int e = 0; e < 4; ++e)
#pragma unroll
        for (int h2 = 0; h2 < 2; ++h2)
#pragma unroll
          for (int h = 0; h < 2; ++h) {
            const int pos = 2 * pr + h2;
            const float wv = wr[(g & 1) * 4 + h2 * 2 + h][e];
            if (ZERO && e == 0) {
              const f32x4 zero = {0.f, 0.f, 0.f, 0.f};
              acc[pos][h] = __builtin_amdgcn_mfma_f32_16x16x4f32(wv, v[pos][e], zero, 0, 0, 0);
            } else {
              acc[pos][h] = __builtin_amdgcn_mfma_f32_16x16x4f32(wv, v[pos][e], acc[pos][h], 0, 0, 0);
            }
          }
      __builtin_amdgcn_sched_barrier(0);
      between(pr);
    }
  };
  auto refill = [&](f32x4 (&nx)[16], const float* patch, int s, int pr) {
    if (pr == 3) { read_column(nx, patch, s, 0); read_column(nx, patch, s, 1); }
    if (pr == 5) { read_column(nx, patch, s, 2); transform_piece(nx, 0); transform_piece(nx, 1); }
    if (pr == 7) { read_column(nx, patch, s, 3); transform_piece(nx, 2); }
  };
  auto finish = [&](f32x4 (&nx)[16]) {
    transform_piece(nx, 3);
#pragma unroll
    for (int p = 4; p < 8; ++p) transform_piece(nx, p);
  };

  const bool stamp = a.dbg && blockIdx.x == 0 && tid == 0;
  int ns_ = 0;
  if (stamp) a.dbg[ns_++] = clock64();
  __syncthreads();
  if (my_items > 0) {
    ring_load(0);
#pragma unroll
    for (int wx = 0; wx < 4; ++wx) read_column(va, lds, 0, wx);
#pragma unroll
    for (int p = 0; p < 8; ++p) transform_piece(va, p);
  }
  int w = vb;
  for (int k = 0; k < my_items; ++k, w += (int)gridDim.x) {
    if (stamp && ns_ < 60) a.dbg[ns_++] = clock64();
    const float* patch = lds + (k & 1) * RAWBUF;
    const float* patch_next = k + 1 < my_items ? lds + ((k + 1) & 1) * RAWBUF : patch;
    const ItemPos ip = item_pos(wk, w);
    const size_t tile_pix = ((size_t)ip.b * a.Ho + (size_t)ip.ty * TH) * a.Wo + (size_t)ip.tx * TW;
    float* out_tile = a.out + tile_pix * a.out_cs + a.out_coff;
    mfma_step(0, va, std::true_type(), [&](int pr) { refill(vb_, patch, 1, pr); });
    finish(vb_);
    __builtin_amdgcn_sched_barrier(0);
    if (stamp && ns_ < 60) a.dbg[ns_++] = clock64();
    __syncthreads();
    if (stamp && ns_ < 60) a.dbg[ns_++] = clock64();
    f32x4 rv[2][4];
    auto request_res = [&](int h) {
      if (has_res) {
        const float* res_tile = a.res + tile_pix * a.res_cs + a.res_coff;
#pragma unroll
        for (int q = 0; q < 4; ++q) {
          const char* ub = reinterpret_cast<const char*>(res_tile + ((q >> 1) * a.Wo + (q & 1)) * a.res_cs + 16 * h);
          rv[h][q] = __builtin_nontemporal_load(reinterpret_cast<const f32x4*>(ub + lane_res));
        }
      }
    };
    mfma_step(1, vb_, std::false_type(), [&](int pr) {
      if (RES) {
        if (pr == 2) request_res(0);
        if (pr == 4) request_res(1);
      } else {
        if (pr == 3) { read_column(va, patch_next, 0, 0); read_column(va, patch_next, 0, 1); }
        if (pr == 5) { transform_piece(va, 0); transform_piece(va, 1); }
      }
    });
    __builtin_amdgcn_sched_barrier(0);
    if (stamp && ns_ < 60) a.dbg[ns_++] = clock64();
#pragma unroll
    for (int h = 0; h < 2; ++h) {
      f32x4 y[4];
#pragma unroll
      for (int py = 0; py < 4; ++py) {
        const f32x4 r0 = pk_add4(pk_add4(acc[py * 4][h], acc[py * 4 + 1][h]), acc[py * 4 + 2][h]);
        const f32x4 r1 = pk_sub4(pk_sub4(acc[py * 4 + 1][h], acc[py * 4 + 2][h]), acc[py * 4 + 3][h]);
        if (py == 0) { y[0] = r0; y[1] = r1; }
        if (py == 1) { y[0] = pk_add4(y[0], r0); y[1] = pk_add4(y[1], r1); y[2] = r0; y[3] = r1; }
        if (py == 2) { y[0] = pk_add4(y[0], r0); y[1] = pk_add4(y[1], r1); y[2] = pk_sub4(y[2], r0); y[3] = pk_sub4(y[3], r1); }
        if (py == 3) { y[2] = pk_sub4(y[2], r0); y[3] = pk_sub4(y[3], r1); }
      }
      const f32x4 bias4 = *reinterpret_cast<const f32x4*>(a.bias + 16 * h + 4 * kq);
#pragma unroll
      for (int q = 0; q < 4; ++q) {
        f32x4 o4 = pk_add4(y[q], bias4);
        if (has_res) o4 = pk_add4(o4, rv[h][q]);
        if (a.relu) {
          o4[0] = vrelu1(o4[0]); o4[1] = vrelu1(o4[1]); o4[2] = vrelu1(o4[2]); o4[3] = vrelu1(o4[3]);
        }
        char* ub = reinterpret_cast<char*>(out_tile + ((q >> 1) * a.Wo + (q & 1)) * a.out_cs + 16 * h);
        __builtin_nontemporal_store(o4, reinterpret_cast<f32x4*>(ub + lane_out));
      }
    }
    __builtin_amdgcn_sched_barrier(0);
    if (RES) {
      read_column(va, patch_next, 0, 0);
      read_column(va, patch_next, 0, 1);
    }
    read_column(va, patch_next, 0, 2);
    read_column(va, patch_next, 0, 3);
    if (RES) { transform_piece(va, 0); transform_piece(va, 1); }
    transform_piece(va, 2);
    finish(va);
    __builtin_amdgcn_sched_barrier(0);
    if (stamp && ns_ < 60) a.dbg[ns_++] = clock64();
  }
  if (stamp) a.dbg[63] = ns_;
}

static bool wino3_ok(const ConvArgs& a) {
  return a.ks == 3 && a.stride == 1 && a.groups == 1 && a.Cin <= 32 && a.Cout == 32 && a.n_tiles == 1 &&
         a.bias_fstride == 0 && a.Ho % 8 == 0 && a.Wo % 16 == 0 && a.out_cs % 4 == 0 && a.out_coff % 4 == 0 &&
         a.in_cs % 4 == 0 && a.in_coff % 4 == 0 && (!a.res || (a.res_cs % 4 == 0 && a.res_coff % 4 == 0));
}

template <int NLW, bool DMA, bool RES>
static hipError_t launch_wino3b_impl(const ConvArgs& a, hipStream_t s) {
  constexpr size_t lds = (2 * (size_t)18 * 18 * 36 + 16 * 2 * 2 * 256) * sizeof(float);
  static_assert(lds <= 160 * 1024, "two patch buffers and the layer's weights must fit the 160 KiB LDS");
  return launch_conv_kernel(CONV_KERNEL(conv_wino3b_kernel<NLW, DMA, RES>), (4 + NLW) * 64, lds, a.Wo / 16, a.Ho / 16, 1, a, s);
}

template <int TH, int NLW, bool PIPE, int LPRIO = 0, bool DMA = false, int NSW = 0, bool DUAL = false>
static hipError_t launch_wino3_impl(const ConvArgs& a, hipStream_t s) {
  constexpr size_t lds = (2 * (size_t)(TH + 2) * 18 * 36 + 16 * 2 * 2 * 256 + (NSW > 0 ? 2 * TH * 16 * 32 : 0)) * sizeof(float);
  static_assert(lds <= 160 * 1024, "two patch buffers, the layer's weights and the staging tiles must fit the 160 KiB LDS");
  return launch_conv_kernel(CONV_KERNEL(conv_wino3_kernel<TH, NLW, PIPE, LPRIO, DMA, NSW, DUAL>), (TH / 2 + NLW + NSW) * 64, lds,
                            a.Wo / 16, a.Ho / TH, 1, a, s);
}

static hipError_t launch_wino3(const ConvArgs& a, hipStream_t s) {
  if (!wino3_ok(a)) return hipErrorInvalidValue;
  const bool dma_ok = conv_dma_ok(a);
  if (a.out2) {
    if (!dma_ok || a.nxt < 1 || a.nxt > 3 || a.out2_cs % 4 || a.out2_coff % 4) return hipErrorInvalidValue;
    return launch_wino3_impl<8, 2, true, 0, true, 2, true>(a, s);
  }
  if (g_force_cfg == 831) return launch_wino3_impl<8, 2, true, 0>(a, s);
  if (g_force_cfg == 833) return launch_wino3_impl<8, 2, true, 3>(a, s);
  if (g_force_cfg == 834) return launch_wino3_impl<8, 2, true, 1>(a, s);
  if (dma_ok && g_force_cfg == 836) return launch_wino3_impl<8, 1, true, 0, true>(a, s);
  if (g_force_cfg == 832 && a.Ho % 16 == 0) return launch_wino3_impl<16, 4, false>(a, s);
  if (g_force_cfg == 837 && a.Ho % 16 == 0) {
    if (a.res) return dma_ok ? launch_wino3b_impl<2, true, true>(a, s) : launch_wino3b_impl<2, false, true>(a, s);
    return dma_ok ? launch_wino3b_impl<2, true, false>(a, s) : launch_wino3b_impl<2, false, false>(a, s);
  }
  if (dma_ok && g_force_cfg != 839) return launch_wino3_impl<8, 2, true, 0, true, 2>(a, s);
  if (dma_ok) return launch_wino3_impl<8, 2, true, 0, true>(a, s);
  return launch_wino3_impl<8, 2, true, 3>(a, s);
}
```

arbitrary-hands-3d-reconstruction_amd/ops.py:

```python
import ctypes as C

import numpy as np
import torch

from . import _lib
from .packer import (DT_BF16, DT_F16, PRECISIONS, pack_conv, pack_conv_h16, pack_conv_x3, pack_stem, pack_wino3, n_tiles_for,
                     winograd_weights, winograd2d_weights, winograd24_weights, polyphase2_weights)


def _p(t):
    return C.c_void_p(t.data_ptr()) if t is not None else None


def _s(t):
    return C.c_void_p(torch.cuda.current_stream(t.device).cuda_stream)


def _need_cuda(*ts):
    for t in ts:
        if t is not None and not t.is_cuda:
            raise _lib.AcrmiError('device tensors required: libacrmi has no CPU path')


def to_nhwc(x_nchw, cs=None, device='cuda'):
    B, Cc, H, W = x_nchw.shape
    cs = cs or (Cc + 3) // 4 * 4
    out = torch.zeros(B, H, W, cs, dtype=torch.float32, device=device)
    out[..., :Cc] = x_nchw.permute(0, 2, 3, 1).to(device)
    return out


def conv2d(x, weight, bias=None, stride=1, relu=False, residual=None, groups=1, cin=None, in_coff=0, out=None,
           out_coff=0, out_cs=None, frame_bias=None, algo='direct'):
    _need_cuda(x, residual, out, frame_bias)
    w = weight.detach().cpu().numpy() if hasattr(weight, 'detach') else np.asarray(weight)
    cout_t, cin_g, k, _ = w.shape
    cout = cout_t // groups
    b = np.zeros(cout_t, np.float32) if bias is None else (
        bias.detach().cpu().numpy() if hasattr(bias, 'detach') else np.asarray(bias))
    if algo in ('split16', 'split_bf16'):
        if k not in (1, 3) or stride not in (1, 2) or (k == 1 and stride != 1):
            raise ValueError('the split-operand kernels are for 3x3 (stride 1 or 2) and 1x1 stride-1 convolutions')
        tr = None
    elif algo == 'polyphase2':
        if k != 3 or stride != 2:
            raise ValueError('the polyphase kernel is for 3x3 stride-2 convolutions')
        tr = polyphase2_weights
    elif algo in ('winograd', 'winograd2d', 'winograd2d_lds', 'winograd24'):
        if k != 3 or stride != 1:
            raise ValueError('winograd needs a 3x3 stride-1 convolution')
        tr = {'winograd': winograd_weights, 'winograd24': winograd24_weights}.get(algo, winograd2d_weights)
    elif algo == 'direct':
        tr = lambda t: t
    else:
        raise ValueError('algo must be "direct", "winograd", "winograd2d", "winograd2d_lds", "winograd24", "polyphase2", "split16" or "split_bf16"')
    algo_id = {'direct': 0, 'winograd': 1, 'winograd2d': 2, 'winograd2d_lds': 3, 'winograd24': 4, 'polyphase2': 5, 'split16': 6, 'split_bf16': 7}[algo]
    if algo_id == 3:
        if groups != 1 or cout != 32 or cin_g > 32:
            raise ValueError('winograd2d_lds needs groups = 1, Cout = 32, Cin <= 32')
        packed = [pack_wino3(w.astype(np.float64), b)]
    elif algo_id in (6, 7):
        packed = [pack_conv_x3([(w[g * cout:(g + 1) * cout].astype(np.float64), b[g * cout:(g + 1) * cout]) for g in range(groups)],
                               DT_BF16 if algo_id == 7 else DT_F16)]
    else:
        packed = [pack_conv(tr(w[g * cout:(g + 1) * cout].astype(np.float64)), b[g * cout:(g + 1) * cout])
                  for g in range(groups)]
    wp = torch.from_numpy(np.concatenate([p[0] for p in packed])).to(x.device)
    bp = torch.from_numpy(np.concatenate([p[1] for p in packed])).to(x.device)
    B, H, W, cs = x.shape
    cin = cin_g if cin is None else cin
    pad = k // 2
    Ho, Wo = (H + 2 * pad - k) // stride + 1, (W + 2 * pad - k) // stride + 1
    if out is None:
        out_cs = out_cs or (cout_t + 3) // 4 * 4
        out = torch.zeros(B, Ho, Wo, out_cs, dtype=torch.float32, device=x.device)
    bias_t, fstride = bp, 0
    if frame_bias is not None:
        bias_t, fstride = frame_bias.contiguous(), frame_bias.shape[-1]
    if residual is not None and residual.shape[0] == 1 and B > 1:
        algo_id |= _lib.CONV_BIAS_MAP
    L = _lib.lib()
    _lib.check(L.acrmi_conv2d(_p(x), B, H, W, cs, in_coff, cin, _p(wp), _p(bias_t), fstride, _p(residual),
                              residual.shape[-1] if residual is not None else 0, 0, _p(out), out.shape[-1], out_coff,
                              cout, k, stride, int(relu), groups, algo_id, _s(x)))
    return out


def conv2d_splitk(x, weight, bias=None, splits=2, relu=False, residual=None, in_coff=0, out=None, out_coff=0, out_cs=None,
                  workspace=None):
    _need_cuda(x, residual, out, workspace)
    w = weight.detach().cpu().numpy() if hasattr(weight, 'detach') else np.asarray(weight)
    cout, cin, k, _ = w.shape
    if k != 3 or cin % splits:
        raise ValueError('split-K needs a 3x3 convolution whose Cin is a multiple of the slice count')
    ks = cin // splits
    b = np.zeros(cout, np.float32) if bias is None else (
        bias.detach().cpu().numpy() if hasattr(bias, 'detach') else np.asarray(bias))
    packed = [pack_conv(winograd2d_weights(w[:, s * ks:(s + 1) * ks].astype(np.float64)), b) for s in range(splits)]
    wp = torch.from_numpy(np.concatenate([p[0] for p in packed])).to(x.device)
    bp = torch.from_numpy(np.concatenate([p[1] for p in packed])).to(x.device)
    B, H, W, cs = x.shape
    if out is None:
        out_cs = out_cs or (cout + 3) // 4 * 4
        out = torch.zeros(B, H, W, out_cs, dtype=torch.float32, device=x.device)
    L = _lib.lib()
    need = int(L.acrmi_conv2d_splitk_workspace(B, H, W, cout, splits))
    if workspace is None:
        workspace = torch.zeros(need, dtype=torch.uint8, device=x.device)
    _lib.check(L.acrmi_conv2d_splitk(_p(x), B, H, W, cs, in_coff, ks, splits, _p(wp), _p(bp), _p(residual),
                                     residual.shape[-1] if residual is not None else 0, 0, _p(out), out.shape[-1], out_coff,
                                     cout, int(relu), _p(workspace), workspace.numel(), _s(x)))
    return out


def to_nhwc16(x_nchw, precision='fp16', cs=None, device='cuda'):
    B, Cc, H, W = x_nchw.shape
    cs = cs or (Cc + 7) // 8 * 8
    out = torch.zeros(B, H, W, cs, dtype=torch.float16 if precision == 'fp16' else torch.bfloat16, device=device)
    out[..., :Cc] = x_nchw.permute(0, 2, 3, 1).to(device).to(out.dtype)
    return out


def conv2d_h16(x, weight, bias=None, stride=1, relu=False, residual=None, groups=1, cin=None, in_coff=0, out=None,
               out_coff=0, out_cs=None, frame_bias=None, out_f32=False):
    _need_cuda(x, residual, out, frame_bias)
    if x.dtype not in (torch.float16, torch.bfloat16):
        raise ValueError('x must be float16 or bfloat16')
    dt = DT_F16 if x.dtype == torch.float16 else DT_BF16
    w = weight.detach().cpu().numpy() if hasattr(weight, 'detach') else np.asarray(weight)
    cout_t, cin_g, k, _ = w.shape
    cout = cout_t // groups
    b = np.zeros(cout_t, np.float32) if bias is None else (
        bias.detach().cpu().numpy() if hasattr(bias, 'detach') else np.asarray(bias))
    packed = [pack_conv_h16(w[g * cout:(g + 1) * cout].astype(np.float64), b[g * cout:(g + 1) * cout], dt) for g in range(groups)]
    wp = torch.from_numpy(np.concatenate([p[0] for p in packed]).view(np.int16)).to(x.device)
    bp = torch.from_numpy(np.concatenate([p[1] for p in packed])).to(x.device)
    B, H, W, cs = x.shape
    cin = cin_g if cin is None else cin
    pad = k // 2
    Ho, Wo = (H + 2 * pad - k) // stride + 1, (W + 2 * pad - k) // stride + 1
    odt = torch.float32 if out_f32 else x.dtype
    if out is None:
        q = 4 if out_f32 else 8
        out_cs = out_cs or (cout_t + q - 1) // q * q
        out = torch.zeros(B, Ho, Wo, out_cs, dtype=odt, device=x.device)
    if out.dtype != odt or (residual is not None and residual.dtype != odt):
        raise ValueError('out / residual must be %s' % odt)
    bias_t, fstride = bp, 0
    if frame_bias is not None:
        bias_t, fstride = frame_bias.contiguous().float(), frame_bias.shape[-1]
    _lib.check(_lib.lib().acrmi_conv2d_h16(_p(x), B, H, W, cs, in_coff, cin, _p(wp), _p(bias_t), fstride, _p(residual),
                                           residual.shape[-1] if residual is not None else 0, 0, _p(out), out.shape[-1],
                                           out_coff, cout, k, stride, int(relu), groups, dt, int(bool(out_f32)), _s(x)))
    return out


def preprocess(bgr_frames):
    _need_cuda(bgr_frames)
    if bgr_frames.dtype != torch.uint8 or bgr_frames.dim() != 4 or bgr_frames.shape[-1] != 3:
        raise ValueError('frames must be uint8 [n,H,W,3] BGR')
    n, H, W, _ = bgr_frames.shape
    out = torch.empty(n, 512, 512, 3, dtype=torch.uint8, device=bgr_frames.device)
    offsets = np.zeros((n, 10), np.float32)
    src = bgr_frames.contiguous()
    _lib.check(_lib.lib().acrmi_preprocess(_p(src), n, H, W, _p(out), offsets.ctypes.data_as(C.c_void_p), _s(src)))
    return out, torch.from_numpy(offsets)


def preprocess_frames(bgr_frames):
    frames = list(bgr_frames)
    if not frames:
        raise ValueError('no frames')
    _need_cuda(*frames)
    keep = []
    arr = (_lib.Frame * len(frames))()
    for i, f in enumerate(frames):
        if f.dtype != torch.uint8 or f.dim() != 3 or f.shape[-1] != 3 or f.device != frames[0].device:
            raise ValueError('frames must be uint8 [H,W,3] BGR tensors on one device')
        f = f.contiguous()
        keep.append(f)
        arr[i].bgr_dev, arr[i].H, arr[i].W = f.data_ptr(), f.shape[0], f.shape[1]
    n = len(frames)
    out = torch.empty(n, 512, 512, 3, dtype=torch.uint8, device=frames[0].device)
    offsets = np.zeros((n, 10), np.float32)
    _lib.check(_lib.lib().acrmi_preprocess_frames(arr, n, _p(out), offsets.ctypes.data_as(C.c_void_p), _s(out)))
    return out, torch.from_numpy(offsets)


def nv12_matrix(name_or_row='cv601'):
    if isinstance(name_or_row, str):
        which = _lib.NV12_MATRICES.get(name_or_row)
        if which is None:
            raise ValueError('unknown NV12 matrix %r: one of %s, or a row of six integers' % (name_or_row, sorted(_lib.NV12_MATRICES)))
        row = np.zeros(6, np.int32)
        _lib.check(_lib.lib().acrmi_nv12_matrix(which, row.ctypes.data_as(C.c_void_p)))
        return row
    row = np.asarray(name_or_row.cpu() if hasattr(name_or_row, 'cpu') else name_or_row)
    if row.shape != (6,) or row.dtype.kind not in 'iu' or np.abs(row.astype(np.int64)).max() >= 2 ** 31:
        raise ValueError('an NV12 matrix is a name or six int32 integers (cy, cub, cug, cvg, cvr, y_off)')
    return np.ascontiguousarray(row.astype(np.int32))


def _nv12_plane(t, what, i):
    if not isinstance(t, torch.Tensor) or t.dtype != torch.uint8:
        raise ValueError('NV12 frame %d: %s must be a uint8 tensor' % (i, what))


def _nv12_item(item, i):
    if isinstance(item, torch.Tensor):
        _nv12_plane(item, 'the surface', i)
        if item.dim() != 2 or item.shape[0] % 3:
            raise ValueError('NV12 frame %d: one tensor must be [H*3/2, W], got %s' % (i, tuple(item.shape)))
        H, W = item.shape[0] // 3 * 2, item.shape[1]
        if H < 2 or W < 2 or H % 2 or W % 2:
            raise ValueError('NV12 frame %d: H and W must be even and >= 2, got %d x %d' % (i, H, W))
        if item.stride(1) != 1 or item.stride(0) < W:
            raise ValueError('NV12 frame %d: rows must be dense (innermost stride 1, pitch >= W), got strides %s' % (i, item.stride()))
        p = item.stride(0)
        return item.data_ptr(), item.data_ptr() + H * p, H, W, p, p, (item,)
    if not isinstance(item, tuple) or len(item) != 2:
        raise ValueError('NV12 frame %d: a uint8 tensor [H*3/2, W] or a tuple (y [H,W], uv [H/2,W] or [H/2,W/2,2])' % i)
    y, uv = item
    _nv12_plane(y, 'y', i)
    _nv12_plane(uv, 'uv', i)
    if y.dim() != 2:
        raise ValueError('NV12 frame %d: y must be [H,W], got %s' % (i, tuple(y.shape)))
    H, W = y.shape
    if H < 2 or W < 2 or H % 2 or W % 2:
        raise ValueError('NV12 frame %d: H and W must be even and >= 2, got %d x %d' % (i, H, W))
    if tuple(uv.shape) not in ((H // 2, W), (H // 2, W // 2, 2)):
        raise ValueError('NV12 frame %d: uv must be [H/2,W] or [H/2,W/2,2] for y %s, got %s' % (i, tuple(y.shape), tuple(uv.shape)))
    if y.stride(1) != 1 or y.stride(0) < W:
        raise ValueError('NV12 frame %d: y rows must be dense (innermost stride 1, pitch >= W), got strides %s' % (i, y.stride()))
    inner_ok = uv.stride(-1) == 1 and (uv.dim() == 2 or W == 2 or uv.stride(1) == 2)
    uv_pitch = uv.stride(0) if H > 2 else W
    if not inner_ok or uv_pitch < W:
        raise ValueError('NV12 frame %d: uv rows must be dense interleaved U, V bytes (pitch >= W), got strides %s' % (i, uv.stride()))
    if y.device != uv.device:
        raise ValueError('NV12 frame %d: y and uv are on different devices' % i)
    return y.data_ptr(), uv.data_ptr(), H, W, y.stride(0), uv_pitch, (y, uv)


def _nv12_frames(frames):
    if isinstance(frames, torch.Tensor) and frames.dim() == 3:
        items = list(frames.unbind(0))
    elif isinstance(frames, (torch.Tensor, tuple)):
        items = [frames]
    else:
        items = list(frames)
    if not items:
        raise ValueError('no frames')
    arr = (_lib.NV12Frame * len(items))()
    keep, sizes = [], []
    for i, item in enumerate(items):
        yp, uvp, H, W, ypitch, uvpitch, bound = _nv12_item(item, i)
        if max(ypitch, uvpitch) >= 2 ** 31:
            raise ValueError('NV12 frame %d: pitch beyond int32' % i)
        arr[i].y_dev, arr[i].uv_dev, arr[i].H, arr[i].W, arr[i].y_pitch, arr[i].uv_pitch = yp, uvp, H, W, ypitch, uvpitch
        keep.extend(bound)
        sizes.append((H, W))
    if any(t.device != keep[0].device for t in keep):
        raise ValueError('NV12 frames must all be on one device')
    _need_cuda(*keep)
    return arr, sizes, keep[0].device, keep


def preprocess_nv12(frames, matrix='cv601'):
    coef = nv12_matrix(matrix)
    arr, sizes, dev, keep = _nv12_frames(frames)
    n = len(sizes)
    out = torch.empty(n, 512, 512, 3, dtype=torch.uint8, device=dev)
    offsets = np.zeros((n, 10), np.float32)
    _lib.check(_lib.lib().acrmi_preprocess_nv12(arr, n, coef.ctypes.data_as(C.c_void_p), _p(out),
                                                offsets.ctypes.data_as(C.c_void_p), _s(out)))
    del keep
    return out, torch.from_numpy(offsets)


def nv12_to_bgr(frames, matrix='cv601', rgb=False):
    coef = nv12_matrix(matrix)
    arr, sizes, dev, keep = _nv12_frames(frames)
    n = len(sizes)
    if all(s == sizes[0] for s in sizes):
        out = torch.empty(n, sizes[0][0], sizes[0][1], 3, dtype=torch.uint8, device=dev)
        dst = [out[i] for i in range(n)]
    else:
        out = dst = [torch.empty(H, W, 3, dtype=torch.uint8, device=dev) for H, W in sizes]
    ptrs = (C.c_void_p * n)(*[d.data_ptr() for d in dst])
    _lib.check(_lib.lib().acrmi_nv12_to_rgb(arr, n, coef.ctypes.data_as(C.c_void_p), 0 if rgb else 1, ptrs, _s(dst[0])))
    del keep
    return out


def cam_trans(joints, pj2d, focal_length=600.0, img_size=512.0):
    _need_cuda(joints, pj2d)
    n = joints.shape[0]
    if tuple(joints.shape[1:]) != (21, 3) or tuple(pj2d.shape) != (n, 21, 2):
        raise ValueError('joints must be [n,21,3] and pj2d [n,21,2]')
    out = torch.empty(n, 3, dtype=torch.float32, device=joints.device)
    j, p = joints.contiguous().float(), pj2d.contiguous().float()
    _lib.check(_lib.lib().acrmi_cam_trans(_p(j), _p(p), n, float(focal_length), float(img_size), _p(out), _s(joints)))
    return out


def u8norm(img):
    _need_cuda(img)
    B, H, W, _ = img.shape
    out = torch.empty(B, H, W, 4, dtype=torch.float32, device=img.device)
    src = img.contiguous()
    _lib.check(_lib.lib().acrmi_u8norm(_p(src), B * H * W, _p(out), _s(src)))
    return out


def stem_conv(img, w, b, relu=True):
    _need_cuda(img)
    B, H, W, _ = img.shape
    wp, bp = pack_stem(np.asarray(w, np.float64), np.asarray(b, np.float64))
    wd, bd = torch.from_numpy(wp).to(img.device), torch.from_numpy(bp).to(img.device)
    out = torch.empty(B, H // 2, W // 2, 64, dtype=torch.float32, device=img.device)
    src = img.contiguous()
    _lib.check(_lib.lib().acrmi_stem_conv(_p(src), B, H, W, _p(wd), _p(bd), _p(out), 64, 0, int(relu), _s(src)))
    return out


def bilinear2x(x, channels=None):
    _need_cuda(x)
    B, H, W, cs = x.shape
    Cc = channels or cs
    out = torch.zeros(B, 2 * H, 2 * W, Cc, dtype=torch.float32, device=x.device)
    _lib.check(_lib.lib().acrmi_bilinear2x(_p(x), B, H, W, cs, Cc, _p(out), Cc, _s(x)))
    return out


def fuse_sum(terms, shifts, relu=True):
    _need_cuda(*terms)
    B, H, W, Cc = terms[0].shape
    n = len(terms)
    out = torch.empty(B, H, W, Cc, dtype=torch.float32, device=terms[0].device)
    ptrs = (C.c_void_p * n)(*[t.data_ptr() for t in terms])
    cs = (C.c_int * n)(*[t.shape[-1] for t in terms])
    sh = (C.c_int * n)(*shifts)
    _lib.check(_lib.lib().acrmi_fuse_sum(n, ptrs, cs, sh, B, H, W, Cc, _p(out), Cc, int(relu), _s(out)))
    return out


def attpool(segm, feat, channels):
    _need_cuda(segm, feat)
    B = segm.shape[0]
    ws = torch.empty(int(_lib.lib().acrmi_attpool_ws_floats(B, channels)), dtype=torch.float32, device=segm.device)
    pooled = torch.empty(B, 32, channels, dtype=torch.float32, device=segm.device)
    _lib.check(_lib.lib().acrmi_attpool(_p(segm), segm.shape[-1], _p(feat), feat.shape[-1], channels, B, _p(ws),
                                        _p(pooled), _s(segm)))
    return pooled


def parebias(pooled, lc_w, lin_w, lin_b, mix_wp, mix_b, part0):
    _need_cuda(pooled)
    B, _, Cc = pooled.shape
    dev = pooled.device
    w = [torch.as_tensor(np.ascontiguousarray(np.asarray(a, np.float32))).to(dev) for a in (lc_w, lin_w, lin_b, mix_wp, mix_b)]
    out = torch.zeros(B, 112, dtype=torch.float32, device=dev)
    src = pooled.contiguous().float()
    _lib.check(_lib.lib().acrmi_parebias(_p(src), Cc, int(part0), _p(w[0]), _p(w[1]), _p(w[2]), _p(w[3]), _p(w[4]), B,
                                         _p(out), 112, _s(src)))
    return out


def decode_maps(l_center, r_center, l_params, r_params, l_prior, r_prior, conf_thresh=0.35, prior_gate=None):
    _need_cuda(l_center, r_center, l_params, r_params, l_prior, r_prior, prior_gate)
    B = l_center.shape[0]
    slots = torch.empty(B, 2, _lib.SLOT, dtype=torch.float32, device=l_center.device)
    gate = None if prior_gate is None else prior_gate.to(torch.int32).contiguous()
    if gate is not None and gate.numel() != B:
        raise ValueError('prior_gate must hold one int per frame')
    _lib.check(_lib.lib().acrmi_decode_maps_gated(_p(l_center), _p(r_center), l_center.shape[-1], _p(l_params), _p(r_params),
                                                  l_params.shape[-1], _p(l_prior), _p(r_prior), l_prior.shape[-1], B,
                                                  float(conf_thresh), _p(gate), _p(slots), _s(slots)))
    return slots


def prior_gate(slots):
    _need_cuda(slots)
    if slots.dtype != torch.float32 or not slots.is_contiguous():
        raise ValueError('slots must be a contiguous float32 device tensor')
    gate = torch.empty(slots.shape[0], dtype=torch.int32, device=slots.device)
    _lib.check(_lib.lib().acrmi_prior_gate(None, _p(slots), slots.shape[0], _p(gate), _s(slots)))
    return gate


HAND_COLORS_RGB = ((0.46, 0.59, 0.64), (0.94, 0.71, 0.53))


def mesh_topology(faces, n_verts):
    f = faces.detach().cpu().numpy() if hasattr(faces, 'detach') else np.asarray(faces)
    if f.ndim != 2 or f.shape[1] != 3:
        raise ValueError('faces must be [F,3]')
    f = np.ascontiguousarray(f.astype(np.int32))
    L = _lib.lib()
    n = _lib.check(L.acrmi_mesh_topology(None, f.shape[0], int(n_verts), None, 0))
    blob = np.empty(n, np.int32)
    _lib.check(L.acrmi_mesh_topology(f.ctypes.data_as(C.c_void_p), f.shape[0], int(n_verts), blob.ctypes.data_as(C.c_void_p), n))
    return blob


def view_from_offsets(offsets):
    o = torch.as_tensor(offsets, dtype=torch.float32)
    return torch.stack([o[:, 0] / 512., o[:, 1] / 512., o[:, 5] - o[:, 9], o[:, 2] - o[:, 6]], 1)


def _topology_on(t, n_verts, device):
    if isinstance(t, torch.Tensor) and t.dim() == 1 and t.dtype == torch.int32:
        blob = t
    elif isinstance(t, np.ndarray) and t.ndim == 1 and t.dtype == np.int32:
        blob = torch.from_numpy(t)
    else:
        blob = torch.from_numpy(mesh_topology(t, n_verts))
    return blob.to(device).contiguous()


def render_meshes(verts, faces, images, mesh_frame=None, trans=None, colors=None, view=None, focal_length=1265.,
                  visible_weight=0.9, out=None, return_ids=False, topo_index=None):
    _need_cuda(verts, images, out)
    if verts.dim() != 3 or verts.shape[-1] != 3 or verts.shape[0] < 1:
        raise ValueError('verts must be [M,V,3]')
    if images.dtype != torch.uint8 or images.dim() != 4 or images.shape[-1] != 3 or images.shape[0] < 1:
        raise ValueError('images must be uint8 [N,H,W,3]')
    dev = images.device
    M, V, _ = verts.shape
    N, H, W, _ = images.shape
    pair = isinstance(faces, (tuple, list)) and len(faces) == 2 and not np.isscalar(faces[0]) and np.ndim(faces[0]) >= 1
    topos = [_topology_on(t, V, dev) for t in (faces if pair else [faces])]
    head = [t[:2].tolist() for t in topos]
    F = head[0][0]
    if any(h != [F, V] for h in head):
        raise ValueError('topology is for (faces, verts) = %s, verts have %d vertices' % (head, V))
    v = verts.to(dev, torch.float32).contiguous()
    t = None if trans is None else trans.to(dev, torch.float32).contiguous().view(M, 3)
    if mesh_frame is None:
        if M % N:
            raise ValueError('mesh_frame is needed when the frames do not divide the meshes')
        mesh_frame = torch.arange(M, dtype=torch.int32) // (M // N)
    mf = torch.as_tensor(mesh_frame).to(dev, torch.int32).contiguous()
    if mf.numel() != M:
        raise ValueError('mesh_frame must hold one int per mesh')
    ti = None
    if topo_index is not None:
        ti = torch.as_tensor(topo_index).to(dev, torch.int32).contiguous()
        if ti.numel() != M or not pair:
            raise ValueError('topo_index needs a pair of topologies and one int per mesh')
    c = torch.as_tensor(HAND_COLORS_RGB[1] if colors is None else colors, dtype=torch.float32)
    c = (c.view(1, 3).repeat(M, 1) if c.numel() == 3 else c.reshape(M, 3)).to(dev).contiguous()
    vw = None
    if view is not None:
        vw = torch.as_tensor(view, dtype=torch.float32).to(dev).contiguous()
        if tuple(vw.shape) != (N, 4):
            raise ValueError('view must be [N,4]')
    src = images.contiguous()
    if out is None:
        out = torch.empty_like(src)
    elif out.dtype != torch.uint8 or tuple(out.shape) != (N, H, W, 3) or not out.is_contiguous() or out.device != dev:
        raise ValueError('out must be a contiguous uint8 tensor shaped like images, on their device')
    ids = torch.empty(N, H, W, dtype=torch.int32, device=dev) if return_ids else None
    L = _lib.lib()
    ws = torch.empty(int(L.acrmi_render_workspace(M, F)) + 256, dtype=torch.uint8, device=dev)
    ws_p = (ws.data_ptr() + 255) // 256 * 256
    _lib.check(L.acrmi_rasterize(_p(v), _p(t), M, V, F, _p(topos[0]), _p(topos[1]) if pair else None, _p(ti), _p(mf), _p(c),
                                 _p(vw), float(focal_length), float(visible_weight), _p(src), _p(out), N, H, W, _p(ids),
                                 C.c_void_p(ws_p), _s(src)))
    return (out, ids) if return_ids else out


SKELETON_PARENTS = (1, 2, 3, 20, 5, 6, 7, 20, 9, 10, 11, 20, 13, 14, 15, 20, 17, 18, 19, 20, -1)
MANO2INTERHAND = (4, 3, 2, 1, 8, 7, 6, 5, 12, 11, 10, 9, 16, 15, 14, 13, 20, 19, 18, 17, 0)
SKELETON_COLORS_RGB = ((230, 230, 0), (255, 51, 51), (255, 102, 102), (255, 153, 153),
                       (230, 230, 0), (51, 255, 51), (102, 255, 102), (153, 255, 153),
                       (230, 230, 0), (255, 153, 51), (255, 178, 102), (255, 204, 153),
                       (230, 230, 0), (51, 153, 255), (102, 178, 255), (153, 204, 255),
                       (230, 230, 0), (255, 51, 255), (255, 102, 255), (255, 153, 255), (230, 230, 0))


def overlay_tables(bgr=False):
    colors, lut = np.empty((21, 3), np.uint8), np.empty((256, 3), np.uint8)
    _lib.check(_lib.lib().acrmi_overlay_tables(int(bool(bgr)), colors.ctypes.data_as(C.c_void_p), lut.ctypes.data_as(C.c_void_p)))
    return colors, lut


def _check_images(images, name='images'):
    if not isinstance(images, torch.Tensor) or images.dtype != torch.uint8 or images.dim() != 4 or images.shape[-1] != 3 \
            or images.shape[0] < 1:
        raise ValueError('%s must be a uint8 tensor [N,H,W,3]' % name)


def _check_dst(dst, src, name='dst'):
    if dst.dtype != torch.uint8 or tuple(dst.shape) != tuple(src.shape) or not dst.is_contiguous() or dst.device != src.device:
        raise ValueError('%s must be a contiguous uint8 tensor shaped like images, on their device' % name)


def draw_skeletons(kps, images, hand_frame=None, colors=None, line_width=3, circle_rad=3, bgr=False, dst=None):
    _check_images(images)
    if not isinstance(kps, torch.Tensor) or kps.dim() != 3 or tuple(kps.shape[1:]) != (21, 2) or kps.shape[0] < 1 or \
            kps.dtype != torch.float32:
        raise ValueError('kps must be a float32 tensor [M,21,2]')
    _need_cuda(kps, images, dst)
    dev = images.device
    M, N = kps.shape[0], images.shape[0]
    if hand_frame is None:
        if M % N:
            raise ValueError('hand_frame is needed when the frames do not divide the hands')
        hand_frame = torch.arange(M, dtype=torch.int32) // (M // N)
    hf = torch.as_tensor(hand_frame).to(dev, torch.int32).contiguous()
    if hf.numel() != M:
        raise ValueError('hand_frame must hold one int per hand')
    col = None
    if colors is not None:
        col = np.ascontiguousarray(np.asarray(colors.cpu() if hasattr(colors, 'cpu') else colors))
        if col.shape != (21, 3) or col.dtype != np.uint8:
            raise ValueError('colors must be uint8 [21,3]')
    k = kps.to(dev).contiguous()
    src = images.contiguous()
    if dst is None:
        dst = torch.empty_like(src)
    else:
        _check_dst(dst, src)
    _lib.check(_lib.lib().acrmi_draw_skeletons(_p(k), _p(hf), M, None if col is None else col.ctypes.data_as(C.c_void_p),
                                               int(bool(bgr)), int(line_width), int(circle_rad), _p(src), _p(dst), N,
                                               src.shape[1], src.shape[2], _s(src)))
    return dst


def draw_heatmaps(maps, images, view=None, weight=0.7, bgr=False, lut=None):
    _check_images(images)
    if not isinstance(maps, torch.Tensor) or not maps.is_floating_point() or maps.dim() not in (3, 4) or \
            (maps.dim() == 4 and maps.shape[1] != 2) or maps.shape[0] != images.shape[0]:
        raise ValueError('maps must be a float tensor [N,2,h,w] or [N,h,w] with one row per image')
    _need_cuda(maps, images)
    dev = images.device
    N, H, W, _ = images.shape
    m = maps.to(dev, torch.float32).contiguous()
    h, w = m.shape[-2:]
    two = m.dim() == 4
    vw = None
    if view is not None:
        vw = torch.as_tensor(view, dtype=torch.float32).to(dev).contiguous()
        if tuple(vw.shape) != (N, 4):
            raise ValueError('view must be [N,4]')
    tab = None
    if lut is not None:
        tab = np.ascontiguousarray(np.asarray(lut.cpu() if hasattr(lut, 'cpu') else lut))
        if tab.shape != (256, 3) or tab.dtype != np.uint8:
            raise ValueError('lut must be uint8 [256,3]')
    src = images.contiguous()
    out = torch.empty((2 if two else 1, N, H, W, 3), dtype=torch.uint8, device=dev)
    right = C.c_void_p(m.data_ptr() + 4 * h * w) if two else None
    _lib.check(_lib.lib().acrmi_draw_heatmaps(_p(m), right, (2 if two else 1) * h * w, N, h, w, _p(vw), float(weight),
                                              None if tab is None else tab.ctypes.data_as(C.c_void_p), int(bool(bgr)),
                                              _p(src), _p(out[0]), _p(out[1]) if two else None, H, W, _s(src)))
    return out if two else out[0]
```

arbitrary-hands-3d-reconstruction_amd/packer.py:

```python
import numpy as np

from . import _lib
from .schema import RESNET50, RESNET50_LAYERS, RESNET50_UP, backbone_channels, stage_cfg, state_dict_schema, width_of

EPS = 1e-5
WINOGRAD = True
WINOGRAD_2D = True


def _np(t):
    if hasattr(t, 'detach'):
        t = t.detach().cpu().numpy()
    return np.asarray(t)


def strip_prefix(sd, prefix='module.'):
    for k in ('model_state_dict', 'state_dict'):
        if k in sd and isinstance(sd[k], dict):
            sd = sd[k]
    out = {}
    for k, v in sd.items():
        out[k[len(prefix):] if k.startswith(prefix) else k] = v
    return out


def check_state_dict(sd):
    want = state_dict_schema(width_of(sd))
    missing = [k for k in want if k not in sd and not k.startswith('segmentation_layers.')
               and not k.endswith('num_batches_tracked')]
    if missing:
        raise ValueError('checkpoint is missing %d tensors, e.g. %s' % (len(missing), missing[:3]))
    for k, shp in want.items():
        if k in sd and tuple(_np(sd[k]).shape) != tuple(shp):
            raise ValueError('checkpoint tensor %s has shape %s, expected %s' % (k, tuple(_np(sd[k]).shape), shp))


def n_tiles_for(cout):
    return 1 if cout <= 32 else ((cout + 63) // 64) * 2


def pack_conv(w, b):
    cout, cin, kh, kw = w.shape
    nt = n_tiles_for(cout)
    c8 = (cin + 7) // 8
    wp = np.zeros((nt * 32, c8 * 8, kh, kw), np.float32)
    wp[:cout, :cin] = w
    wp = wp.reshape(nt, 32, c8, 2, 4, kh, kw)
    if cout == 33 and (kh, kw) == (4, 4):
        wp[1, 4::4] = wp[1, 0:1]
    wp = wp.transpose(5, 6, 2, 0, 3, 1, 4)
    bp = np.zeros(nt * 32, np.float32)
    bp[:cout] = b
    return np.ascontiguousarray(wp).reshape(-1), bp


DT_F32, DT_F16, DT_BF16 = 0, 1, 2
PRECISIONS = {'fp32': DT_F32, 'fp16': DT_F16, 'bf16': DT_BF16, 'fp16x3': DT_F32, 'bf16x3': DT_F32}


def round_to(x, dt):
    x = np.asarray(x, np.float32)
    if dt == DT_F16:
        return x.astype(np.float16).astype(np.float32)
    if dt == DT_BF16:
        return (to_bits16(x, dt).astype(np.uint32) << 16).view(np.float32).reshape(x.shape)
    return x


def to_bits16(x, dt):
    x = np.ascontiguousarray(x, np.float32)
    if dt == DT_F16:
        return x.astype(np.float16).view(np.uint16)
    u = x.view(np.uint32).astype(np.uint64)
    return (((u + 0x7FFF + ((u >> 16) & 1)) >> 16) & 0xFFFF).astype(np.uint16)


def pack_conv_h16(w, b, dt):
    cout, cin, kh, kw = w.shape
    nt = n_tiles_for(cout)
    c16 = (cin + 15) // 16
    wp = np.zeros((nt * 32, c16 * 16, kh, kw), np.float64)
    wp[:cout, :cin] = w
    wp = wp.reshape(nt, 32, c16, 2, 8, kh, kw)
    wp = wp.transpose(5, 6, 2, 0, 3, 1, 4)
    bp = np.zeros(nt * 32, np.float32)
    bp[:cout] = b
    return to_bits16(np.ascontiguousarray(wp).reshape(-1), dt), bp


def split16(x, dt=DT_F16):
    x = np.asarray(x, np.float64)
    hi = round_to(x, dt).astype(np.float64)
    lo = round_to(x - hi, dt)
    return hi.astype(np.float32), lo


def x3_weight_shift(ws):
    m = max(float(np.max(np.abs(w))) for w in ws)
    if not np.isfinite(m) or m <= 0.0:
        return 0
    return int(min(30, max(-30, 12 - int(np.floor(np.log2(m))))))


def pack_conv_x3(wb_list, dt=DT_F16):
    shift = x3_weight_shift([w for (w, _) in wb_list])
    out, biases = [], []
    for (w, b) in wb_list:
        cout, cin, kh, kw = w.shape
        assert cin % 16 == 0
        nt = n_tiles_for(cout)
        c16 = cin // 16
        wp = np.zeros((nt * 32, cin, kh, kw), np.float64)
        wp[:cout] = np.asarray(w, np.float64) * 2.0 ** shift
        hi, lo = split16(wp, dt)
        both = np.stack([hi, lo])
        both = both.reshape(2, nt, 32, c16, 2, 8, kh, kw)
        both = both.transpose(6, 7, 3, 1, 0, 4, 2, 5)
        out.append(to_bits16(np.ascontiguousarray(both).reshape(-1), dt).view(np.float32))
        bp = np.zeros(nt * 32, np.float32)
        bp[:cout] = b
        biases.append(bp)
    out.append(np.array([2.0 ** -shift], np.float32))
    return np.concatenate(out), np.concatenate(biases)


def pack_wino3(w, b):
    cout, cin = w.shape[:2]
    assert w.shape[2:] == (3, 3) and cout == 32 and cin <= 32
    u = np.zeros((32, 32, 4, 4))
    u[:cout, :cin] = winograd2d_weights(w)
    u = u.reshape(2, 16, 2, 4, 4, 4, 4)
    u = u.transpose(5, 6, 2, 0, 3, 1, 4)
    bp = np.zeros(32, np.float32)
    bp[:cout] = b
    return np.ascontiguousarray(u, np.float32).reshape(-1), bp


def pack_stem(w, b):
    assert w.shape == (64, 3, 3, 3)
    wk = np.zeros((64, 28))
    wk[:, :27] = np.asarray(w, np.float64).transpose(0, 2, 3, 1).reshape(64, 27)
    frag = wk.reshape(2, 32, 14, 2).transpose(2, 0, 3, 1)
    return np.ascontiguousarray(frag, np.float32).reshape(-1), np.asarray(b, np.float32).copy()


def pack_stem7(w, b):
    assert w.shape == (64, 3, 7, 7)
    wk = np.zeros((64, 148))
    wk[:, :147] = np.asarray(w, np.float64).transpose(0, 2, 3, 1).reshape(64, 147)
    frag = wk.reshape(2, 32, 74, 2).transpose(2, 0, 3, 1)
    return np.ascontiguousarray(frag, np.float32).reshape(-1), np.asarray(b, np.float32).copy()


def pack_pair1x1(w3, b3, w1, b1):
    w3 = np.asarray(w3, np.float64).reshape(256, 64)
    w1 = np.asarray(w1, np.float64).reshape(64, 256)
    a1 = w3.reshape(8, 32, 2, 8, 4).transpose(0, 3, 2, 1, 4).reshape(-1)
    a2 = w1.reshape(2, 32, 8, 4, 2, 4).transpose(2, 0, 3, 4, 1, 5).reshape(-1)
    out = np.concatenate([a1, a2, np.asarray(b3, np.float64).reshape(-1), np.asarray(b1, np.float64).reshape(-1)])
    assert out.size == 256 * 64 + 64 * 256 + 256 + 64
    return out.astype(np.float32)


FUSE_PAIRS = True


STEM_FUSED = True

WINO_G = np.array([[1.0, 0.0, 0.0], [0.5, 0.5, 0.5], [0.5, -0.5, 0.5], [0.0, 0.0, 1.0]])


def winograd_weights(w):
    assert w.shape[2:] == (3, 3)
    return np.einsum('vk,oiyk->oiyv', WINO_G, np.asarray(w, np.float64))


def winograd2d_weights(w):
    assert w.shape[2:] == (3, 3)
    return np.einsum('uy,vx,oiyx->oiuv', WINO_G, WINO_G, np.asarray(w, np.float64))


WINO_G4 = np.array([[1 / 4.0, 0.0, 0.0], [-1 / 6.0, -1 / 6.0, -1 / 6.0], [-1 / 6.0, 1 / 6.0, -1 / 6.0],
                    [1 / 24.0, 1 / 12.0, 1 / 6.0], [1 / 24.0, -1 / 12.0, 1 / 6.0], [0.0, 0.0, 1.0]])


def winograd24_weights(w):
    assert w.shape[2:] == (3, 3)
    return np.einsum('uy,vx,oiyx->oiuv', WINO_G, WINO_G4, np.asarray(w, np.float64))


def polyphase2_weights(w):
    assert w.shape[2:] == (3, 3)
    w = np.asarray(w, np.float64)
    c = {'A0': (1.0, 0.0, 0.0), 'A1': (1.0, 0.0, 1.0), 'A2': (0.0, 0.0, 1.0), 'B': (0.0, 1.0, 0.0)}
    out = np.zeros(w.shape[:2] + (4, 7))
    for oy in range(2):
        for ox in range(2):
            ya, xa = ('A0', 'A2')[oy], ('A0', 'A2')[ox]
            if oy == ox:
                prods = [(ya, xa), (ya, 'B'), ('B', xa), ('B', 'B'), (ya, 'A1'), ('B', 'A1'), ('A1', 'A1')]
            else:
                prods = [(ya, xa), ('B', xa), (ya, 'B'), ('B', 'B'), ('A1', xa), ('A1', 'B'), ('A1', 'A1')]
            for kk, (ty, tx) in enumerate(prods):
                out[:, :, 2 * oy + ox, kk] = np.einsum('oiyx,y,x->oi', w, np.array(c[ty]), np.array(c[tx]))
    return out


POLYPHASE2 = __import__('os').environ.get('ACRMI_PP2', '1') != '0'


POLYPHASE2_SMALL = __import__('os').environ.get('ACRMI_PP2_SMALL', '1') != '0'


def polyphase2_ok(cin, cout, ho, wo):
    return cin % 16 == 0 and cout % 32 == 0 and ho % 8 == 0 and wo % 16 == 0


SPLIT16_STRIDE2 = __import__('os').environ.get('ACRMI_X3_STRIDE2', '1') != '0'


def split16_ok(k, stride, cin, cout, ho, wo):
    if not (cin % 32 == 0 and cin >= 32 and cout % 32 == 0):
        return False
    if stride == 2:
        return SPLIT16_STRIDE2 and k == 3 and ho % 8 == 0 and wo % 32 == 0
    if stride != 1:
        return False
    return (k == 3 and ((ho % 8 == 0 and wo % 32 == 0) or (ho % 16 == 0 and wo % 16 == 0))) or (
        k == 1 and ho * wo > 0 and (ho * wo) % 256 == 0)


def use_winograd(k, stride):
    return k == 3 and stride == 1


WINOGRAD_LDS = True


WINOGRAD_24 = __import__('os').environ.get('ACRMI_WINO24', '1') != '0'


def wino24b_width(cin, cout, ho, wo):
    if not (cin % 32 == 0 and cin >= 32 and cout % 32 == 0):
        return 0
    if ho % 8 == 0 and wo % 32 == 0:
        return 32
    if ho % 16 == 0 and wo % 16 == 0 and cin >= 64 and cout % 64 == 0:
        return 16
    return 0


def conv_algo(k, stride, cin, cout, groups=1, ho=0, wo=0, per_frame_bias=False, wino24=None, split16=False):
    if split16 and split16_ok(k, stride, cin, cout, ho, wo):
        return 7 if split16 == 'bf16' else 6
    if k == 3 and stride == 2:
        big = (WINOGRAD_24 if wino24 is None else wino24) or POLYPHASE2_SMALL
        return 5 if (POLYPHASE2 and big and polyphase2_ok(cin, cout, ho, wo)) else 0
    if not (WINOGRAD and use_winograd(k, stride)):
        return 0
    if (WINOGRAD_2D and WINOGRAD_LDS and groups == 1 and cin <= 32 and cout == 32 and ho % 8 == 0 and wo % 16 == 0
            and not per_frame_bias):
        return 3
    if WINOGRAD_2D and (WINOGRAD_24 if wino24 is None else wino24) and cout != 33:
        if cin > 32 and wo % 32 == 0 and ho % 8 == 0:
            return 4
        if wino24b_width(cin, cout, ho, wo) and (cin > 32 or cout % 64 == 0):
            return 4
    return 2 if WINOGRAD_2D else 1


COORD_BIAS_MAP = True


def coord_bias_map(wc, size, stride):
    f32 = np.float32
    t = ((np.arange(size, dtype=f32) / f32(size - 1)) * f32(2.0) - f32(1.0)).astype(np.float64)
    cm = np.zeros((2, size + 2, size + 2))
    cm[0, 1:-1, 1:-1] = t[None, :]
    cm[1, 1:-1, 1:-1] = t[:, None]
    ho = (size - 1) // stride + 1
    cout = wc.shape[0]
    out = np.zeros((ho, ho, (cout + 3) // 4 * 4))
    for ky in range(3):
        for kx in range(3):
            patch = cm[:, ky:ky + stride * (ho - 1) + 1:stride, kx:kx + stride * (ho - 1) + 1:stride]
            out[:, :, :cout] += np.einsum('chw,oc->hwo', patch, wc[:, :, ky, kx])
    return out


SPLITK_MAX_ITEMS = 32


def splitk_slices(k, stride, cin, cout, groups, ho, wo, per_frame_bias):
    if not (k == 3 and stride == 1 and groups == 1 and not per_frame_bias and cout != 33 and cin >= 128 and cin % 64 == 0):
        return 1
    n_tiles = 1 if cout <= 32 else (cout + 63) // 64 * 2
    items = ((ho + 7) // 8) * ((wo + 15) // 16) * n_tiles
    if items > SPLITK_MAX_ITEMS:
        return 1
    for s in range(min(cin // 64, 8), 1, -1):
        if cin % (32 * s) == 0:
            return s
    return 1


FUSE_EPILOGUE = __import__('os').environ.get('ACRMI_FUSE_EPI', '1') != '0'
FUSE_FULLRES = __import__('os').environ.get('ACRMI_FUSE_EPI0', '1') != '0'


FUSE_PROJECTION = True


class Blob(object):
    def __init__(self):
        self.parts = [np.zeros(64, np.float32)]
        self.n = 64

    def add16(self, bits):
        bits = np.ascontiguousarray(bits, np.uint16).reshape(-1)
        assert bits.size % 2 == 0
        return self.add(bits.view(np.float32))

    def add(self, arr):
        arr = np.ascontiguousarray(arr, np.float32).reshape(-1)
        pad = (-arr.size) % 64
        off = self.n
        self.parts.append(arr)
        if pad:
            self.parts.append(np.zeros(pad, np.float32))
        self.n += arr.size + pad
        return off

    def finish(self):
        return np.concatenate(self.parts)


class Program(object):

    def __init__(self, sd, dt=DT_F32, keep_weights=False, keep_all=False, wino24=None, splitk=False, pairs=False, split16=False):
        self.sd = {k: _np(v) for k, v in sd.items()}
        self.dt = dt
        self.keep_weights = keep_weights
        self.splitk = splitk
        self.pairs = pairs and dt == DT_F32
        self.wino24 = wino24
        self.split16 = split16 if dt == DT_F32 else False
        self.keep_all = keep_all
        self.chan_pad = {}
        self.blob = Blob()
        self.bufs = []
        self.free = {}
        self.ops = []
        self.op_info = []

    def buf(self, h, w, c, persistent=False, f32=False):
        dt = DT_F32 if f32 else self.dt
        q = 4 if dt == DT_F32 else 8
        cs = (c + q - 1) // q * q
        key = (h, w, cs, dt)
        if not persistent and self.free.get(key):
            return self.free[key].pop()
        self.bufs.append((h, w, cs, 1 if persistent else 0, dt))
        return len(self.bufs) - 1

    def release(self, *ids):
        for i in ids:
            h, w, cs, p, dt = self.bufs[i]
            if not p and not self.keep_all:
                assert i not in self.free.setdefault((h, w, cs, dt), []), 'double release of buffer %d' % i
                self.free[(h, w, cs, dt)].append(i)

    def pin(self, i):
        h, w, cs, _, dt = self.bufs[i]
        self.bufs[i] = (h, w, cs, 1, dt)
        return i

    def dtype_of(self, i):
        return self.bufs[i][4]

    def dims(self, i):
        return self.bufs[i][:3]

    def folded(self, conv, bn=None):
        w = self.sd[conv + '.weight'].astype(np.float64)
        b = self.sd.get(conv + '.bias')
        b = np.zeros(w.shape[0]) if b is None else b.astype(np.float64)
        if bn is not None:
            g = self.sd[bn + '.weight'].astype(np.float64)
            scale = g / np.sqrt(self.sd[bn + '.running_var'].astype(np.float64) + EPS)
            w = w * scale[:, None, None, None]
            b = self.sd[bn + '.bias'].astype(np.float64) + (b - self.sd[bn + '.running_mean'].astype(np.float64)) * scale
        return w, b

    def _op(self, name, flops=0.0, **kw):
        op = _lib.Op()
        for f in ('in_buf', 'out_buf', 'res_buf', 'aux_buf'):
            setattr(op, f, -1)
        for k, v in kw.items():
            setattr(op, k, v)
        self.ops.append(op)
        self.op_info.append({'name': name, 'flops': float(flops), 'kind': int(op.kind), 'mode': int(op.mode)})
        return op

    def set_mode(self, mode, first):
        for op, info in zip(self.ops[first:], self.op_info[first:]):
            op.mode = info['mode'] = mode

    def clone_op(self, i, name, flops_scale, **kw):
        op = _lib.Op.from_buffer_copy(bytes(self.ops[i]))
        for k, v in kw.items():
            setattr(op, k, v)
        self.ops.append(op)
        info = dict(self.op_info[i])
        info.update(name=name, flops=info['flops'] * flops_scale, mode=int(op.mode))
        self.op_info.append(info)
        return op

    def conv(self, name, src, wb_list, k, stride, relu, out=None, out_c=None, in_coff=0, out_coff=0, res=None,
             res_coff=0, cin=None, bias_buf=None, bias_map=None, terms=None, dual=None, fp32_kernel=False):
        h, w_, _ = self.dims(src)
        cout, cin_w = wb_list[0][0].shape[:2]
        cin = cin_w if cin is None else cin
        ho, wo = (h + 2 * (k // 2) - k) // stride + 1, (w_ + 2 * (k // 2) - k) // stride + 1
        flop_cout = cout
        if out is None and out_c is None and len(wb_list) == 1 and k == 3 and stride == 1 and cout < 32 and res is None:
            w0, b0 = wb_list[0]
            wp = np.zeros((32,) + w0.shape[1:], w0.dtype)
            wp[:cout] = w0
            bp = np.zeros(32, b0.dtype)
            bp[:cout] = b0
            wb_list, cout = [(wp, bp)], 32
        slices = 1
        if self.splitk and self.dt == DT_F32 and bias_map is None and len(wb_list) == 1:
            slices = splitk_slices(k, stride, cin, cout, 1, ho, wo, bias_buf is not None)
            if slices > 1 and conv_algo(k, stride, cin, cout, 1, ho, wo, bias_buf is not None, False) != 2:
                slices = 1
        if slices > 1:
            w0, b0 = wb_list[0]
            ks = cin // slices
            wb_list, cin = [(w0[:, s * ks:(s + 1) * ks], b0) for s in range(slices)], ks
        if out is None:
            out = self.buf(ho, wo, (out_c or (cout if slices > 1 else cout * len(wb_list))))
        if self.dt != DT_F32:
            assert self.dtype_of(src) == self.dt, 'conv input must be a 16-bit buffer in a 16-bit program'
            assert res is None or self.dtype_of(res) == self.dtype_of(out)
            algo = 0
            packed = [pack_conv_h16(w, b, self.dt) for (w, b) in wb_list]
            w_off = self.blob.add16(np.concatenate([p[0] for p in packed]))
        else:
            algo = 2 if slices > 1 else conv_algo(k, stride, cin, cout, len(wb_list), ho, wo, bias_buf is not None, self.wino24,
                                                    False if ((terms or fp32_kernel) and stride == 2) else self.split16)
            if algo in (6, 7):
                packed = [pack_conv_x3(wb_list, DT_BF16 if algo == 7 else DT_F16)]
            elif algo == 3:
                packed = [pack_wino3(w, b) for (w, b) in wb_list]
            else:
                tr = (lambda t: t, winograd_weights, winograd2d_weights, None, winograd24_weights, polyphase2_weights)[algo]
                packed = [pack_conv(tr(w), b) for (w, b) in wb_list]
            w_off = self.blob.add(np.concatenate([p[0] for p in packed]))
        b_off = self.blob.add(np.concatenate([p[1] for p in packed]))
        flops = 2.0 * ho * wo * flop_cout * cin_w * k * k * (1 if slices > 1 else len(wb_list))
        self._op(name, flops, kind=_lib.OP_CONV, in_buf=src, out_buf=out, res_buf=-1 if res is None else res,
                 in_coff=in_coff, out_coff=out_coff, res_coff=res_coff, cin=cin, cout=cout, ksize=k, stride=stride,
                 relu=int(relu), groups=len(wb_list), w_off=w_off, b_off=b_off, flags=algo,
                 bias_per_frame=0 if bias_buf is None else 1, aux_buf=-1 if bias_buf is None else bias_buf)
        if slices > 1:
            self.ops[-1].flags = algo | _lib.CONV_SPLITK
        if dual:
            out2, terms = dual
            assert algo == 3 and bias_buf is None and self.dims(out2)[:2] == (ho, wo) and out2 != out
            self.ops[-1].flags = algo | _lib.CONV_DUAL
            self.ops[-1].aux_buf = out2
        if terms:
            assert len(terms) <= 3 and self.dt == DT_F32 and len(wb_list) == 1
            assert dual or (k == 3 and stride == 2 and algo in (0, 5))
            op = self.ops[-1]
            op.nterms = len(terms)
            for t, (tb, sh) in enumerate(terms):
                th, tw, tcs = self.dims(tb)
                assert (th << sh, tw << sh) == (ho, wo) and tcs >= cout and tb != out
                op.term_buf[t], op.term_coff[t], op.term_shift[t] = tb, 0, sh
        if bias_map is not None:
            assert res is None and self.dt == DT_F32 and algo != 3
            assert bias_map.shape == (ho, wo, (cout * len(wb_list) + 3) // 4 * 4), bias_map.shape
            self.ops[-1].flags = algo | _lib.CONV_BIAS_MAP
            self.ops[-1].w_off2 = self.blob.add(bias_map)
        self.op_info[-1]['algo'] = ('direct', 'winograd_f23x', 'winograd_f2x2_3x3', 'winograd_f2x2_3x3_lds',
                                    'winograd_f2x4_3x3', 'polyphase_f2x2_s2', 'split_f16x3', 'split_bf16x3')[algo] + ('_splitk%d' % slices if slices > 1 else '')
        ng = len(wb_list)
        esz = lambda b: 4 if self.dtype_of(b) == DT_F32 else 2
        fam = ('conv_ws2_kernel', 'conv_wino_kernel', 'conv_wino2_kernel', 'conv_wino3_kernel', 'conv_wino24_kernel',
               'conv_pp2_kernel', 'conv_x3_kernel', 'conv_x3_kernel')[algo]
        if algo == 4 and wino24b_width(cin, cout, ho, wo):
            fam = 'conv_wino24b_kernel'
        if algo in (6, 7) and k == 1:
            fam = 'conv_x3p_kernel'
        if algo in (6, 7) and stride == 2:
            fam = 'conv_x3s2_kernel'
        if (algo == 0 and k == 1 and stride == 1 and cin % 32 == 0 and cout % 32 == 0 and (ho * wo) % 256 == 0 and
                (WINOGRAD_24 if self.wino24 is None else self.wino24) and
                (ho * wo // 256) * 64 * ng * ((cout // 32) // (2 if cout % 64 == 0 else 1)) >= 512):
            fam = 'conv_p1_kernel'
        if self.dt != DT_F32:
            fam = 'conv_h16_kernel'
        self.op_info[-1]['kernel'] = fam
        self.op_info[-1]['bytes'] = float(h * w_ * cin * ng * esz(src) + ho * wo * (cout if slices > 1 else cout * ng) * esz(out) *
                                          (2 if res is not None else 1) +
                                          sum((ho >> sh) * (wo >> sh) * cout * 4 for (_, sh) in (terms or [])) +
                                          (ho * wo * cout * 4 if dual else 0))
        if self.keep_weights:
            self.op_info[-1]['wb'] = [(np.asarray(w, np.float64), np.asarray(b, np.float64)) for (w, b) in wb_list]
        return out

    def cp(self, c):
        return self.chan_pad.get(c, c)

    def fuse_epilogue_ok(self, cin, cout):
        return FUSE_EPILOGUE and self.dt == DT_F32 and cin > 16 and cin % 8 == 0 and cout % 32 == 0

    def conv_bn(self, src, conv, bn, k, stride, relu, padded=False, **kw):
        w, b = self.folded(conv, bn)
        if padded and (self.cp(w.shape[0]) != w.shape[0] or self.cp(w.shape[1]) != w.shape[1]):
            co, ci = w.shape[:2]
            wp = np.zeros((self.cp(co), self.cp(ci)) + w.shape[2:])
            wp[:co, :ci] = w
            bp = np.zeros(self.cp(co))
            bp[:co] = b
            out = self.conv(conv, src, [(wp, bp)], k, stride, relu, **kw)
            self.op_info[-1]['flops'] *= float(co * ci) / float(wp.shape[0] * wp.shape[1])
            return out
        return self.conv(conv, src, [(w, b)], k, stride, relu, **kw)

    def fuse_sum(self, name, terms, c, relu, out=None, out_coff=0):
        h, w_, _ = self.dims(terms[0][0])
        assert terms[0][1] == 0
        if out is None:
            out = self.buf(h, w_, c)
        op = self._op(name, 0.0, kind=_lib.OP_FUSESUM, out_buf=out, out_coff=out_coff, cout=c, relu=int(relu),
                      nterms=len(terms))
        for t, (b, sh) in enumerate(terms):
            op.term_buf[t], op.term_coff[t], op.term_shift[t] = b, 0, sh
        return out

    def basic_block(self, x, p, dual=None):
        t = self.conv_bn(x, p + '.conv1', p + '.bn1', 3, 1, True, padded=True)
        kw = dict(dual=dual) if dual else {}
        y = self.conv_bn(t, p + '.conv2', p + '.bn2', 3, 1, True, res=x, padded=True, **kw)
        self.release(t, x)
        return y

    def fuse0_ok(self, c, h, w):
        return (FUSE_EPILOGUE and FUSE_FULLRES and self.dt == DT_F32 and not self.splitk and
                conv_algo(3, 1, self.cp(c), self.cp(c), 1, h, w, False, self.wino24, self.split16) == 3)

    def bottleneck(self, x, p, cat=None, stride=1):
        cin = self.sd[p + '.conv1.weight'].shape[1]
        t1 = self.conv_bn(x, p + '.conv1', p + '.bn1', 1, 1, True, cin=cin)
        if cat is not None:
            assert cat == x and stride == 1 and (p + '.downsample.0.weight') in self.sd
            mid = self.sd[p + '.conv2.weight'].shape[0]
            assert mid == cin and self.dims(cat)[2] >= 2 * cin
            self.conv_bn(t1, p + '.conv2', p + '.bn2', 3, 1, True, out=cat, out_coff=cin)
            self.release(t1)
            (wd, bd), (w3, b3) = self.folded(p + '.downsample.0', p + '.downsample.1'), self.folded(p + '.conv3', p + '.bn3')
            y = self.conv(p + '.conv3+downsample', cat, [(np.concatenate([wd, w3], 1), bd + b3)], 1, 1, True)
            self.release(cat)
            return y
        t2 = self.conv_bn(t1, p + '.conv2', p + '.bn2', 3, stride, True)
        self.release(t1)
        if (p + '.downsample.0.weight') in self.sd:
            res = self.conv_bn(x, p + '.downsample.0', p + '.downsample.1', 1, stride, False)
            self.release(x)
        else:
            res = x
        y = self.conv_bn(t2, p + '.conv3', p + '.bn3', 1, 1, True, res=res)
        self.release(t2, res)
        return y

    def bottleneck_chain(self, x, prefix, n, cat=None):
        shapes_ok = all(self.sd['%s.%d.conv3.weight' % (prefix, i)].shape[:2] == (256, 64) and
                        self.sd['%s.%d.conv1.weight' % (prefix, i)].shape[0] == 64 for i in range(n))
        if not (self.pairs and shapes_ok and n >= 2):
            for i in range(n):
                x = self.bottleneck(x, '%s.%d' % (prefix, i), cat=cat if i == 0 else None)
            return x
        t1 = None
        for i in range(n):
            p = '%s.%d' % (prefix, i)
            if t1 is None:
                t1 = self.conv_bn(x, p + '.conv1', p + '.bn1', 1, 1, True, cin=self.sd[p + '.conv1.weight'].shape[1])
            t2 = self.conv_bn(t1, p + '.conv2', p + '.bn2', 3, 1, True)
            self.release(t1)
            if (p + '.downsample.0.weight') in self.sd:
                res = self.conv_bn(x, p + '.downsample.0', p + '.downsample.1', 1, 1, False,
                                   cin=self.sd[p + '.downsample.0.weight'].shape[1])
                self.release(x)
            else:
                res = x
            if i == n - 1:
                y = self.conv_bn(t2, p + '.conv3', p + '.bn3', 1, 1, True, res=res)
                self.release(t2, res)
                return y
            q = '%s.%d' % (prefix, i + 1)
            (w3, b3), (w1, b1) = self.folded(p + '.conv3', p + '.bn3'), self.folded(q + '.conv1', q + '.bn1')
            h, w_, _ = self.dims(t2)
            y, t1 = self.buf(h, w_, 256), self.buf(h, w_, 64)
            self._op(p + '.conv3+' + q + '.conv1', 2.0 * h * w_ * (256 * 64 + 64 * 256), kind=_lib.OP_PAIR1X1, in_buf=t2, res_buf=res,
                     out_buf=y, aux_buf=t1, cin=64, cout=256, ksize=1, stride=1, relu=1, groups=1,
                     w_off=self.blob.add(pack_pair1x1(w3[:, :, 0, 0], b3, w1[:, :, 0, 0], b1)))
            self.op_info[-1]['algo'] = 'pair1x1'
            if self.keep_weights:
                self.op_info[-1]['wb'] = [(np.asarray(w3, np.float64), np.asarray(b3, np.float64)),
                                          (np.asarray(w1, np.float64), np.asarray(b1, np.float64))]
            self.release(t2, res)
            x = y

    def hr_module(self, xs, p, ch, multi_scale=True, final_out=None):
        nb = len(xs)
        xs = list(xs)
        h0, w0, _ = self.dims(xs[0])
        fold0 = nb > 1 and self.fuse0_ok(ch[0], h0, w0)
        for i in range(nb):
            for k in range(3 if (i == 0 and fold0) else 4):
                xs[i] = self.basic_block(xs[i], '%s.branches.%d.%d' % (p, i, k))
        outs = []
        temps = []

        def term(i, j, hosted=None):
            f = '%s.fuse_layers.%d.%d' % (p, i, j)
            if j == i:
                return xs[j], 0
            if j > i:
                t = self.conv_bn(xs[j], f + '.0', f + '.1', 1, 1, False, padded=True)
                temps.append(t)
                return t, j - i
            t = xs[j]
            for k in range(i - j):
                last = k == i - j - 1
                kw = dict(terms=hosted) if (last and hosted) else {}
                if last and j == 0:
                    kw['fp32_kernel'] = True
                t2 = self.conv_bn(t, '%s.%d.0' % (f, k), '%s.%d.1' % (f, k), 3, 2, (not last) or bool(hosted), padded=True, **kw)
                if t is not xs[j]:
                    self.release(t)
                t = t2
            if not hosted:
                temps.append(t)
            return t, 0

        for i in range(nb if multi_scale else 1):
            f0 = '%s.fuse_layers.%d.0' % (p, i)
            if i == 0 and fold0:
                others = [term(0, j) for j in range(1, nb)]
                y0 = final_out if final_out is not None else self.buf(h0, w0, self.cp(ch[0]))
                xs[0] = self.basic_block(xs[0], '%s.branches.0.3' % p, dual=(y0, others))
                self.op_info[-1]['name'] += '+fuse0'
                outs.append(y0)
                continue
            if i >= 1 and final_out is None:
                wl = self.sd['%s.%d.0.weight' % (f0, i - 1)]
                if self.fuse_epilogue_ok(self.cp(wl.shape[1]), self.cp(wl.shape[0])):
                    others = [term(i, j) for j in range(1, nb)]
                    y, _ = term(i, 0, hosted=others)
                    self.op_info[-1]['name'] += '+fuse%d' % i
                    outs.append(y)
                    continue
            terms = [term(i, j) for j in range(nb)]
            if terms[0][1] != 0:
                raise AssertionError('term 0 must be at output resolution')
            if final_out is not None:
                outs.append(self.fuse_sum(p + '.fuse%d' % i, terms, ch[i], True, out=final_out))
            else:
                outs.append(self.fuse_sum(p + '.fuse%d' % i, terms, self.cp(ch[i]), True))
        self.release(*temps)
        self.release(*xs)
        return outs


def point_tower(P, side, k):
    def rows(w, cpad):
        co, ci = w.shape[:2]
        wp = np.zeros((co, cpad, 3, 3))
        wp[:, :ci] = w
        return wp.reshape(co, cpad // 4, 4, 9).transpose(3, 1, 0, 2).reshape(-1)
    pre = '%s_final_layers.%d' % (side, k)
    w, b = P.folded(pre + '.0.0', pre + '.0.1')
    parts = [rows(w, 36), b]
    for blk in range(2):
        for c in (1, 2):
            w, b = P.folded(pre + '.1.%d.0.conv%d' % (blk, c), pre + '.1.%d.0.bn%d' % (blk, c))
            parts += [rows(w, 64), b]
    w, b = P.folded(pre + '.2')
    we = np.zeros((64, 112))
    we[:, :w.shape[0]] = w[:, :, 0, 0].T
    be = np.zeros(112)
    be[:w.shape[0]] = b
    out = np.concatenate([np.asarray(x, np.float64).reshape(-1) for x in parts + [we, be]])
    assert out.size == 9 * 9 * 64 * 4 + 64 + 4 * (9 * 16 * 64 * 4 + 64) + 64 * 112 + 112
    return out


def lower(sd, check=True, point_heads=True, keep_taps=False, precision='fp32', keep_weights=False, keep_all=False,
          wino24=None, splitk=False, pairs=None):
    sd = strip_prefix(sd)
    if check:
        check_state_dict(sd)
    if precision not in PRECISIONS:
        raise ValueError('precision %r: one of %s' % (precision, sorted(PRECISIONS)))
    width = width_of({k: _np(v) for k, v in sd.items() if k in ('backbone.transition1.0.0.weight', 'backbone.layer4.0.conv1.weight')})
    STAGE_CFG = None if width == RESNET50 else stage_cfg(width)
    c0 = backbone_channels(width)
    dt = PRECISIONS[precision]
    point_heads = point_heads and dt == DT_F32 and width == 32
    P = Program(sd, dt, keep_weights, keep_all, wino24, splitk, FUSE_PAIRS and not splitk if pairs is None else pairs,
                split16={'fp16x3': 'fp16', 'bf16x3': 'bf16'}.get(precision, False))
    b = 'backbone.'
    taps = {}
    x34 = None
    if width == RESNET50:
        w, bb = P.folded(b + 'conv1', b + 'bn1')
        x = P.buf(256, 256, 64)
        wp, bp = pack_stem7(w, bb)
        P._op(b + 'conv1', 2.0 * 256 * 256 * 64 * 3 * 49, kind=_lib.OP_STEM, out_buf=x, cin=3, cout=64, ksize=7, stride=2,
              relu=1, groups=1, w_off=P.blob.add(wp), b_off=P.blob.add(bp))
        P.op_info[-1]['algo'] = 'stem7_u8'
        if keep_weights:
            P.op_info[-1]['wb'] = [(np.asarray(w, np.float64), np.asarray(bb, np.float64))]
        if keep_taps:
            taps['stem'] = P.pin(x)
        cat = P.buf(128, 128, 128) if FUSE_PROJECTION else None
        pooled = cat if cat is not None else P.buf(128, 128, 64)
        P._op(b + 'maxpool', 0.0, kind=_lib.OP_MAXPOOL, in_buf=x, out_buf=pooled, cin=64)
        P.release(x)
        x = pooled
        for li, (planes, blocks, stride) in enumerate(RESNET50_LAYERS):
            for i in range(blocks):
                x = P.bottleneck(x, b + 'layer%d.%d' % (li + 1, i), cat=cat if (li == 0 and i == 0) else None,
                                 stride=stride if i == 0 else 1)
        if keep_taps:
            taps['layer4'] = P.pin(x)
        x34 = P.buf(128, 128, c0 + 2, persistent=True)
        P._op('coordfill', 0.0, kind=_lib.OP_COORDFILL, out_buf=x34, out_coff=c0)
        for k, c in enumerate(RESNET50_UP):
            h, w_, cs = P.dims(x)
            cin = P.sd[b + 'deconv_layers.%d.0.weight' % k].shape[1]
            up = P.buf(2 * h, 2 * w_, cin)
            P._op(b + 'deconv_layers.%d.bilinear2x' % k, 0.0, kind=_lib.OP_BILINEAR2X, in_buf=x, out_buf=up, cin=cin)
            P.release(x)
            x = P.conv_bn(up, b + 'deconv_layers.%d.0' % k, b + 'deconv_layers.%d.1' % k, 3, 1, True,
                          out=x34 if k == len(RESNET50_UP) - 1 else None)
            P.release(up)
    else:
        x34 = _lower_hrnet(P, sd, b, STAGE_CFG, c0, keep_taps, keep_weights, taps)
    return _lower_heads(P, sd, b, x34, c0, dt, point_heads, precision, width, taps)


def width_of_sd(sd):
    return width_of({k: v for k, v in sd.items() if k in ('backbone.transition1.0.0.weight', 'backbone.layer4.0.conv1.weight')})


def _lower_hrnet(P, sd, b, STAGE_CFG, c0, keep_taps, keep_weights, taps):
    w, bb = P.folded(b + 'conv1', b + 'bn1')
    if STEM_FUSED:
        x = P.buf(256, 256, 64)
        wp, bp = pack_stem(w, bb)
        P._op(b + 'conv1', 2.0 * 256 * 256 * 64 * 3 * 9, kind=_lib.OP_STEM, out_buf=x, cin=3, cout=64, ksize=3, stride=2,
              relu=1, groups=1, w_off=P.blob.add(wp), b_off=P.blob.add(bp))
        P.op_info[-1]['algo'] = 'stem_u8'
        if keep_weights:
            P.op_info[-1]['wb'] = [(np.asarray(w, np.float64), np.asarray(bb, np.float64))]
    else:
        x0 = P.buf(512, 512, 4)
        P._op('u8norm', 0.0, kind=_lib.OP_U8NORM, out_buf=x0)
        x = P.conv(b + 'conv1', x0, [(w, bb)], 3, 2, True, cin=3)
        P.op_info[-1]['flops'] = 2.0 * 256 * 256 * 64 * 3 * 9
        P.release(x0)
    cat = P.buf(128, 128, 128) if (FUSE_PROJECTION and not P.pairs) else None
    x1 = P.conv_bn(x, b + 'conv2', b + 'bn2', 3, 2, True, out=cat)
    P.release(x)
    x = x1
    if keep_taps:
        taps['stem'] = P.pin(x)
    x = P.bottleneck_chain(x, b + 'layer1', 4, cat=cat)
    if keep_taps:
        taps['layer1'] = P.pin(x)
    t = b + 'transition1'
    if width_of_sd(P.sd) == 48 and P.dt == DT_F32 and (WINOGRAD_24 if P.wino24 is None else P.wino24) and not P.splitk:
        P.chan_pad = {48: 64}
    xs = [P.conv_bn(x, t + '.0.0', t + '.0.1', 3, 1, True, padded=True), P.conv_bn(x, t + '.1.0.0', t + '.1.0.1', 3, 2, True)]
    P.release(x)
    x34 = P.buf(128, 128, c0 + 2, persistent=True)
    P._op('coordfill', 0.0, kind=_lib.OP_COORDFILL, out_buf=x34, out_coff=c0)
    for s in (2, 3, 4):
        ch = STAGE_CFG[s]['channels']
        if s > 2:
            t = b + 'transition%d' % (s - 1)
            i = len(ch) - 1
            xs = xs + [P.conv_bn(xs[-1], t + '.%d.0.0' % i, t + '.%d.0.1' % i, 3, 2, True, padded=True)]
        nmod = STAGE_CFG[s]['modules']
        for m in range(nmod):
            last = (s == 4 and m == nmod - 1)
            xs = P.hr_module(xs, b + 'stage%d.%d' % (s, m), ch, multi_scale=not last,
                             final_out=x34 if last else None)
        if keep_taps and s < 4:
            taps['stage%d' % s] = P.pin(xs[0])
    return x34


def _lower_heads(P, sd, b, x34, c0, dt, point_heads, precision, width, taps):
    u = b + 'hand_segm.segm_head.upsampler.up1.conv.double_conv'
    g = b + 'hand_segm.segm_head.segm_net.double_conv'
    up = P.buf(256, 256, c0)
    P._op('segm.bilinear2x', 0.0, kind=_lib.OP_BILINEAR2X, in_buf=x34, out_buf=up, cin=c0)
    s1 = P.conv_bn(up, u + '.0', u + '.1', 3, 1, True)
    P.release(up)
    s2 = P.conv_bn(s1, u + '.3', u + '.4', 3, 1, True)
    P.release(s1)
    s3 = P.conv_bn(s2, g + '.0', g + '.1', 3, 1, True)
    P.release(s2)
    segm = P.buf(256, 256, 33, persistent=True, f32=True)
    P.conv(g + '.3', s3, [P.folded(g + '.3')], 3, 1, False, out=segm)
    P.release(s3)
    towers = [('l', 2), ('r', 2)] + [(side, k) for side in 'lr' for k in (1, 3, 4)]
    w_list = [P.folded('%s_final_layers.%d.0.0' % t, '%s_final_layers.%d.0.1' % t) for t in towers]
    wcat = np.concatenate([w for w, _ in w_list], 0)
    bcat = np.concatenate([bb for _, bb in w_list], 0)
    coord_map = COORD_BIAS_MAP and dt == DT_F32

    def head_conv(name, wb, stride, **kw):
        w, bb = wb
        if not coord_map:
            return P.conv(name, x34, [(w, bb)], 3, stride, True, cin=c0 + 2, **kw)
        out = P.conv(name, x34, [(w[:, :c0], bb)], 3, stride, True, cin=c0, bias_map=coord_bias_map(w[:, c0:], 128, stride), **kw)
        P.op_info[-1]['flops'] *= (c0 + 2.0) / c0
        return out

    n0 = len(P.ops)
    t0 = head_conv('towers.entry', (wcat, bcat), 2)
    P.set_mode(_lib.MODE_DENSE, n0)
    if point_heads:
        n0 = len(P.ops)
        head_conv('towers.entry.centers', (wcat[:128], bcat[:128]), 2, out=t0)
        P.set_mode(_lib.MODE_POINT, n0)
    for k in range(2):
        c1 = [P.folded('%s_final_layers.%d.1.%d.0.conv1' % (s_, t_, k), '%s_final_layers.%d.1.%d.0.bn1' % (s_, t_, k))
              for s_, t_ in towers]
        c2 = [P.folded('%s_final_layers.%d.1.%d.0.conv2' % (s_, t_, k), '%s_final_layers.%d.1.%d.0.bn2' % (s_, t_, k))
              for s_, t_ in towers]
        n0 = len(P.ops)
        t1 = P.conv('towers.block%d.conv1' % k, t0, c1, 3, 1, True)
        t2 = P.conv('towers.block%d.conv2' % k, t1, c2, 3, 1, True, res=t0)
        P.set_mode(_lib.MODE_DENSE, n0)
        if point_heads and P.split16:
            n1 = len(P.ops)
            P.conv('towers.block%d.conv1.centers' % k, t0, c1[:2], 3, 1, True, out=t1)
            P.conv('towers.block%d.conv2.centers' % k, t1, c2[:2], 3, 1, True, res=t0, out=t2)
            P.set_mode(_lib.MODE_POINT, n1)
        elif point_heads:
            for j in (n0, n0 + 1):
                P.clone_op(j, P.op_info[j]['name'] + '.centers', 2.0 / len(towers), groups=2, mode=_lib.MODE_POINT)
        P.release(t1, t0)
        t0 = t2
    heads = _lib.HeadLayout()

    def padded(w, b, n):
        wp = np.zeros((n,) + w.shape[1:])
        wp[:w.shape[0]] = w
        bp = np.zeros(n)
        bp[:b.shape[0]] = b
        return wp, bp

    p109, final, camb = {}, {}, {}
    mix_w = {}
    for si, (side, mix) in enumerate((('l', 4), ('r', 5))):
        wm = _np(sd['contact_layers.%d.weight' % mix]).astype(np.float64).reshape(109, 218)
        wa = wm[:, :109].copy()
        wa[:, :3] += wm[:, 109:112]
        mix_w[side] = (wa, wm[:, 112:])
        p109[side] = P.buf(64, 64, 109, f32=True) if point_heads else -1
        final[side] = P.buf(64, 64, 128, persistent=True, f32=True)
        camb[side] = P.buf(64, 64, 32)
        center = P.buf(64, 64, 32, persistent=True, f32=True)
        prior = P.buf(64, 64, 128, persistent=True, f32=True)
        name = '%s_final_layers.%%d.2' % side
        tin = lambda k: 64 * towers.index((side, k))
        P.conv(name % 2, t0, [padded(*P.folded(name % 2), 32)], 1, 1, False, out=center, in_coff=tin(2), cin=64)
        P.op_info[-1]['flops'] = 2.0 * 64 * 64 * 64 * 1
        n0 = len(P.ops)
        we, be = P.folded(name % 1)
        wc = wa[:, 3:] @ we[:, :, 0, 0]
        P.conv(side + '.params_mix', t0, [padded(wc[:, :, None, None], wa[:, 3:] @ be, 128)], 1, 1, False,
               out=final[side], in_coff=tin(1), cin=64)
        P.op_info[-1]['flops'] = 2.0 * 64 * 64 * 64 * 106
        P.conv(name % 3, t0, [padded(*P.folded(name % 3), 32)], 1, 1, False, out=camb[side], in_coff=tin(3), cin=64)
        P.op_info[-1]['flops'] = 2.0 * 64 * 64 * 64 * 3
        P._op('%s.cam_pow' % side, 0.0, kind=_lib.OP_POW11, out_buf=camb[side], out_coff=0)
        P.conv(name % 4, t0, [padded(*P.folded(name % 4), 128)], 1, 1, False, out=prior, in_coff=tin(4), cin=64)
        P.op_info[-1]['flops'] = 2.0 * 64 * 64 * 64 * 106
        P.set_mode(_lib.MODE_DENSE, n0)
        heads.center_buf[si], heads.prior_buf[si] = center, prior
    P.release(t0)
    feat = P.buf(128, 128, 256)
    head_conv('contact_layers.1.0', P.folded('contact_layers.1.0', 'contact_layers.1.1'), 1, out=feat)
    pooled = P.buf(1, 32, 256, f32=True)
    P._op('attpool', 2.0 * 32 * 16384 * 320 + 2.0 * 128 * 128 * 256 * 64, kind=_lib.OP_ATTPOOL, in_buf=segm, res_buf=feat,
          out_buf=pooled, cin=256)
    P.op_info[-1]['name'] = 'attpool(+cam_shape_layers.1.0)'
    P.release(feat)
    wcs, bcs = P.folded('cam_shape_layers.1.0')
    wcs = wcs[:, :, 0, 0]
    for si, (side, lc, mix, part0) in enumerate((('l', 2, 4, 16), ('r', 3, 5, 0))):
        wa, wp = mix_w[side]
        bias_buf = P.buf(1, 1, 128, persistent=True, f32=True)
        lw = _np(sd['cam_shape_layers.%d.weight' % lc]).astype(np.float64).reshape(10, 64, 16)
        lin_w = np.einsum('kcj,cd->kdj', lw, wcs).reshape(10, 256 * 16)
        lin_b = _np(sd['cam_shape_layers.%d.bias' % lc]).astype(np.float64) + np.einsum('kcj,c->k', lw, bcs)
        P._op('%s.parebias' % side, 0.0, kind=_lib.OP_PAREBIAS, in_buf=pooled, out_buf=bias_buf, cin=256, flags=part0,
              w_off=P.blob.add(_np(sd['contact_layers.%d.weight' % lc]).reshape(6, 256, 16)),
              w_off2=P.blob.add(lin_w), b_off2=P.blob.add(lin_b),
              w_off3=P.blob.add(wp), b_off=P.blob.add(_np(sd['contact_layers.%d.bias' % mix])))
        n0 = len(P.ops)
        P.conv('contact_layers.%d' % mix, camb[side], [padded(wa[:, :3, None, None], np.zeros(109), 128)], 1, 1, False,
               out=final[side], cin=3, bias_buf=bias_buf, res=final[side])
        P.op_info[-1]['flops'] = 2.0 * 64 * 64 * 109 * 218
        P.set_mode(_lib.MODE_DENSE, n0)
        P.release(camb[side])
        if point_heads:
            mixw = np.zeros((109, 112))
            mixw[:, :109] = wa.T
            P._op('%s.point_heads' % side, 0.0, kind=_lib.OP_POINTHEADS, in_buf=x34, res_buf=p109[side], out_buf=final[side],
                  aux_buf=bias_buf, flags=si, mode=_lib.MODE_POINT,
                  w_off=P.blob.add(np.concatenate([point_tower(P, side, k) for k in (1, 3, 4)])),
                  w_off2=P.blob.add(mixw))
        heads.params_buf[si] = final[side]
    heads.segm_buf, heads.backbone_buf = segm, x34
    return {'blob': P.blob.finish(), 'bufs': P.bufs, 'ops': P.ops, 'heads': heads, 'op_info': P.op_info, 'taps': taps,
            'precision': precision, 'width': width}
```

Measured before the change: 2006 frames/s.

## Extend LDS Winograd conv kernel to Cout 16 and Cout 64 layers

```diff
diff --git a/arbitrary-hands-3d-reconstruction_amd/csrc/acrmi_ops.hip b/arbitrary-hands-3d-reconstruction_amd/csrc/acrmi_ops.hip
--- a/arbitrary-hands-3d-reconstruction_amd/csrc/acrmi_ops.hip
+++ b/arbitrary-hands-3d-reconstruction_amd/csrc/acrmi_ops.hip
@@ -53,9 +53,11 @@
     return fail(nullptr, ACRMI_EINVAL, "acrmi_conv2d: algo 6 / 7 needs Cin %% 32 = 0, Cout %% 32 = 0, H %% 8 == 0, W %% 32 == 0");
   if (algo == 5 && (cin % 16 || cout % 32 || H % 16 || W % 32))
     return fail(nullptr, ACRMI_EINVAL, "acrmi_conv2d: algo 5 needs Cin %% 16 = 0, Cout %% 32 = 0, H %% 16 == 0, W %% 32 == 0");
-  if (algo == 3 && (groups != 1 || cin > 32 || cout != 32 || bias_frame_stride != 0 || H % 8 || W % 16 || out_cs % 4 ||
-                    out_coff % 4 || (res && (res_cs % 4 || res_coff % 4))))
-    return fail(nullptr, ACRMI_EINVAL, "acrmi_conv2d: algo 3 needs groups 1, Cin <= 32, Cout = 32, H %% 8 == 0, W %% 16 == 0");
+  if (algo == 3 && (groups != 1 || cin > 32 || bias_frame_stride != 0 || H % 8 || W % 16 || out_cs % 4 ||
+                    out_coff % 4 || (res && (res_cs % 4 || res_coff % 4)) ||
+                    !(cout == 32 || (cout == 16 && H % 16 == 0) || (cout == 64 && cin <= 16))))
+    return fail(nullptr, ACRMI_EINVAL, "acrmi_conv2d: algo 3 needs groups 1, Cin <= 32, H %% 8 == 0, W %% 16 == 0 and Cout = 32, "
+                "Cout = 16 with H %% 16 == 0, or Cout = 64 with Cin <= 16");
   if (algo == 4 && (cin < 32 || (cin == 32 && (cout % 32 || H % 8 || W % 32))))
     return fail(nullptr, ACRMI_EINVAL, "acrmi_conv2d: algo 4 needs Cin > 32 (or Cin = 32, Cout %% 32 = 0 on a map of 8x32-pixel tiles)");
   if ((ksize != 1 && ksize != 3) || (stride != 1 && stride != 2))
diff --git a/arbitrary-hands-3d-reconstruction_amd/csrc/acrmi_program.hip b/arbitrary-hands-3d-reconstruction_amd/csrc/acrmi_program.hip
--- a/arbitrary-hands-3d-reconstruction_amd/csrc/acrmi_program.hip
+++ b/arbitrary-hands-3d-reconstruction_amd/csrc/acrmi_program.hip
@@ -425,9 +425,12 @@
       if (algo != 0 && !((algo == 6 || algo == 7) && op.ksize == 3 && op.stride == 2) &&
           !((op.ksize == 3 || (algo >= 6 && op.ksize == 1)) && op.stride == (algo == 5 ? 2 : 1)))
         return fail(c, ACRMI_EINVAL, "op %d: algo %d needs a 3x3 stride-%d convolution", i, algo, algo == 5 ? 2 : 1);
-      if (algo == 3 && (op.groups != 1 || op.cin > 32 || op.cout != 32 || op.bias_per_frame || bufs[op.out_buf].h % 8 ||
-                        bufs[op.out_buf].w % 16 || op.out_coff % 4 || op.res_coff % 4))
-        return fail(c, ACRMI_EINVAL, "op %d: algo 3 needs groups 1, Cin <= 32, Cout = 32, a map of 8x16-pixel tiles", i);
+      if (algo == 3 && (op.groups != 1 || op.cin > 32 || op.bias_per_frame || bufs[op.out_buf].h % 8 ||
+                        bufs[op.out_buf].w % 16 || op.out_coff % 4 || op.res_coff % 4 ||
+                        !(op.cout == 32 || (op.cout == 16 && bufs[op.out_buf].h % 16 == 0 && !dual) ||
+                          (op.cout == 64 && op.cin <= 16 && !dual))))
+        return fail(c, ACRMI_EINVAL, "op %d: algo 3 needs groups 1, Cin <= 32, a map of 8x16-pixel tiles and Cout = 32, Cout = 16 "
+                    "(16x16-pixel tiles) or Cout = 64 with Cin <= 16", i);
       const int ogroups = splitk ? 1 : op.groups;
       if (op.in_coff + op.groups * op.cin > bufs[op.in_buf].cs || op.out_coff + ogroups * op.cout > bufs[op.out_buf].cs ||
           (op.res_buf >= 0 && op.res_coff + ogroups * op.cout > bufs[op.res_buf].cs) ||
@@ -452,7 +455,7 @@
         return fail(c, ACRMI_EINVAL, "op %d: algo 5 needs fp32, Cin %% 16 = 0, Cout %% 32 = 0, an output map of 8x16-pixel tiles", i);
       const long long taps = algo >= 6 ? op.ksize * op.ksize : algo == 5 ? 28 : algo == 4 ? 24 : (algo >= 2 ? 16 : (algo == 1 ? 12 : op.ksize * op.ksize));
       const long long ksteps = idt ? (op.cin + 15) / 16 : (op.cin + 7) / 8;
-      const long long wn = algo == 3 ? 16384 : (long long)op.groups * taps * ksteps * n_tiles * 256 + (algo >= 6 ? 1 : 0);
+      const long long wn = algo == 3 ? (op.cout == 16 ? 8192 : 16384) : (long long)op.groups * taps * ksteps * n_tiles * 256 + (algo >= 6 ? 1 : 0);
       if (!w_ok(op.w_off, wn)) return fail(c, ACRMI_EINVAL, "op %d: packed weights outside the blob", i);
       if (op.bias_per_frame) {
         if (!buf_ok(op.aux_buf) || bufs[op.aux_buf].cs < op.groups * op.cout)
diff --git a/arbitrary-hands-3d-reconstruction_amd/csrc/conv_wino3.inc b/arbitrary-hands-3d-reconstruction_amd/csrc/conv_wino3.inc
--- a/arbitrary-hands-3d-reconstruction_amd/csrc/conv_wino3.inc
+++ b/arbitrary-hands-3d-reconstruction_amd/csrc/conv_wino3.inc
@@ -78,14 +78,17 @@
 #ifndef ACRMI_W3_ABLATE
 #define ACRMI_W3_ABLATE 0
 #endif
-template <int TH, int NLW, bool PIPE, int LPRIO = 0, bool DMA = false, int NSW = 0, bool DUAL = false>
-__global__ __launch_bounds__((TH / 2 + NLW + NSW) * 64, 1) void conv_wino3_kernel(const ConvArgs a, const ConvWork wk) {
+template <int TH, int NLW, bool PIPE, int LPRIO = 0, bool DMA = false, int NSW = 0, bool DUAL = false, int FORM = 0>
+__global__ __launch_bounds__(((FORM == 1 ? TH / 4 : TH / 2) + NLW + NSW) * 64, 1) void conv_wino3_kernel(const ConvArgs a, const ConvWork wk) {
   constexpr int W3_ABLATE = ACRMI_W3_ABLATE;
   static_assert(!DUAL || NSW == 2, "the second output is written by the store waves");
+  static_assert(FORM == 0 || (PIPE && !DUAL), "the sized forms are built on the pipelined four-wave kernel");
+  static_assert(FORM != 1 || (TH == 16 && NSW == 0), "Cout 16: 16x16-pixel items, stored by the compute waves");
+  static_assert(FORM != 2 || TH == 8, "one step: 8x16-pixel items");
   constexpr int TW = 16, PH = TH + 2, PW = TW + 2, CK = 32, CP = CK + 4;
-  constexpr int NCW = TH / 2;
+  constexpr int NCW = FORM == 1 ? TH / 4 : TH / 2;
   constexpr int RAWBUF = PH * PW * CP;
-  constexpr int WFLOATS = 16 * 2 * 2 * 256;
+  constexpr int WFLOATS = FORM == 0 ? 16 * 2 * 2 * 256 : 16 * 2 * 256;
   constexpr int STILE = TH * TW * 32;
   static_assert(NSW == 0 || (NSW == 2 && TH == 8), "store waves: two, 8x16-pixel items");
   extern __shared__ f32x4 smem4[];
@@ -116,17 +119,21 @@
     constexpr int PER = WFLOATS / 4 / (NCW * 64);
     f32x4 tmp[PER];
 #pragma unroll
-    for (int i = 0; i < PER; ++i) tmp[i] = src[tid + i * NCW * 64];
+    for (int i = 0; i < PER; ++i) {
+      const int d = tid + i * NCW * 64;
+      tmp[i] = src[FORM == 2 ? (d >> 7) * 256 + (d & 127) : d];
+    }
 #pragma unroll
     for (int i = 0; i < PER; ++i) dst[tid + i * NCW * 64] = tmp[i];
   }
-  const int ch = wave & 1, sg = wave >> 1;
+  const int ch = FORM == 1 ? 0 : wave & 1, sg = FORM == 1 ? wave : wave >> 1;
   const int j = lane & 15, kq = lane >> 4;
   const int in_a = (j < 4) || (j >= 12);
   const int brow = in_a ? 0 : 1;
   const int bcol = in_a ? (j < 4 ? j : j - 8) : j - 4;
   const int by = 2 * sg + brow;
   const int worg = ((2 * by) * PW + 2 * bcol) * CP + 4 * kq;
+  constexpr int WSTRIDE = FORM == 1 ? 256 : 512;
   const float* wfrag = wlds + ch * 256 + lane * 4;
   const bool has_res = a.res != nullptr;
   const int lane_pix = (2 * by) * a.Wo + 2 * bcol;
@@ -180,8 +187,13 @@
   auto ring_load = [&](int g) {
     if ((W3_ABLATE & 4) && g > 1) return;
     const int gg = g & 15, s = gg >> 3, p0 = (gg & 7) * 2;
-    wr[(g & 1) * 2] = *reinterpret_cast<const f32x4*>(wfrag + (p0 * 2 + s) * 512);
-    wr[(g & 1) * 2 + 1] = *reinterpret_cast<const f32x4*>(wfrag + ((p0 + 1) * 2 + s) * 512);
+    if constexpr (FORM == 2) {
+      wr[(g & 1) * 2] = *reinterpret_cast<const f32x4*>(wfrag + p0 * WSTRIDE);
+      wr[(g & 1) * 2 + 1] = *reinterpret_cast<const f32x4*>(wfrag + (p0 + 1) * WSTRIDE);
+    } else {
+      wr[(g & 1) * 2] = *reinterpret_cast<const f32x4*>(wfrag + (p0 * 2 + s) * WSTRIDE);
+      wr[(g & 1) * 2 + 1] = *reinterpret_cast<const f32x4*>(wfrag + ((p0 + 1) * 2 + s) * WSTRIDE);
+    }
   };
   auto mfma_step = [&](int s, const f32x4 (&v)[16], auto zero_tag, auto between) {
     constexpr bool ZERO = decltype(zero_tag)::value;
@@ -209,6 +221,44 @@
     }
   };
 
+  auto request_res = [&](size_t tile_pix) {
+    if (has_res) {
+      const float* res_tile = a.res + tile_pix * a.res_cs + a.res_coff;
+#pragma unroll
+      for (int q = 0; q < 4; ++q) {
+        const char* ub = reinterpret_cast<const char*>(res_tile + ((q >> 1) * a.Wo + (q & 1)) * a.res_cs);
+        rv[q] = __builtin_nontemporal_load(reinterpret_cast<const f32x4*>(ub + lane_res));
+      }
+    }
+  };
+  auto epilogue = [&](int k, float* out_tile) {
+    f32x4 r0[4], r1[4];
+#pragma unroll
+    for (int py = 0; py < 4; ++py) {
+      r0[py] = pk_add4(pk_add4(acc[py * 4], acc[py * 4 + 1]), acc[py * 4 + 2]);
+      r1[py] = pk_sub4(pk_sub4(acc[py * 4 + 1], acc[py * 4 + 2]), acc[py * 4 + 3]);
+    }
+    f32x4 y[4];
+    y[0] = pk_add4(pk_add4(r0[0], r0[1]), r0[2]);
+    y[1] = pk_add4(pk_add4(r1[0], r1[1]), r1[2]);
+    y[2] = pk_sub4(pk_sub4(r0[1], r0[2]), r0[3]);
+    y[3] = pk_sub4(pk_sub4(r1[1], r1[2]), r1[3]);
+#pragma unroll
+    for (int q = 0; q < 4; ++q) {
+      f32x4 o4 = pk_add4(y[q], bias4);
+      if (has_res) o4 = pk_add4(o4, rv[q]);
+      if (a.relu) {
+        o4[0] = vrelu1(o4[0]); o4[1] = vrelu1(o4[1]); o4[2] = vrelu1(o4[2]); o4[3] = vrelu1(o4[3]);
+      }
+      if constexpr (NSW > 0) {
+        *reinterpret_cast<f32x4*>(stage + (k & 1) * STILE + stage_off + ((q >> 1) * TW + (q & 1)) * 32) = o4;
+      } else {
+        char* ub = reinterpret_cast<char*>(out_tile + ((q >> 1) * a.Wo + (q & 1)) * a.out_cs);
+        __builtin_nontemporal_store(o4, reinterpret_cast<f32x4*>(ub + lane_out));
+      }
+    }
+  };
+
   const bool stamp = a.dbg && blockIdx.x == 0 && tid == 0;
   int ns_ = 0;
   if (stamp) a.dbg[ns_++] = clock64();
@@ -218,9 +268,31 @@
     read_window(va, lds, 0);
 #pragma unroll
     for (int p = 0; p < 8; ++p) transform_piece(va, p);
-    if (PIPE) read_column(vb_, lds, 1, 0);
+    if (PIPE && FORM != 2) read_column(vb_, lds, 1, 0);
   }
   int w = vb;
+  if constexpr (FORM == 2) {
+    auto one_step_item = [&](int k, f32x4 (&cur)[16], f32x4 (&nxt)[16]) {
+      const float* patch_next = lds + ((k + 1 < my_items ? k + 1 : k) & 1) * RAWBUF;
+      const ItemPos ip = item_pos(wk, w);
+      const size_t tile_pix = ((size_t)ip.b * a.Ho + (size_t)ip.ty * TH) * a.Wo + (size_t)ip.tx * TW;
+      __syncthreads();
+      read_column(nxt, patch_next, 0, 0);
+      mfma_step(0, cur, std::true_type(), [&](int pr) {
+        if (pr < 3) read_column(nxt, patch_next, 0, pr + 1);
+        transform_piece(nxt, pr);
+        if (pr == 5) request_res(tile_pix);
+      });
+      __builtin_amdgcn_sched_barrier(0);
+      epilogue(k, a.out + tile_pix * a.out_cs + a.out_coff);
+      __builtin_amdgcn_sched_barrier(0);
+      w += (int)gridDim.x;
+    };
+    for (int k = 0; k < my_items; k += 2) {
+      one_step_item(k, va, vb_);
+      if (k + 1 < my_items) one_step_item(k + 1, vb_, va);
+    }
+  } else
   for (int k = 0; k < my_items; ++k, w += (int)gridDim.x) {
     if (stamp && ns_ < 60) a.dbg[ns_++] = clock64();
     const float* patch = lds + (k & 1) * RAWBUF;
@@ -228,17 +300,7 @@
     const ItemPos ip = item_pos(wk, w);
     const size_t tile_pix = ((size_t)ip.b * a.Ho + (size_t)ip.ty * TH) * a.Wo + (size_t)ip.tx * TW;
     float* out_tile = a.out + tile_pix * a.out_cs + a.out_coff;
-    auto request_res = [&]() {
-      if (has_res) {
-        const float* res_tile = a.res + tile_pix * a.res_cs + a.res_coff;
-#pragma unroll
-        for (int q = 0; q < 4; ++q) {
-          const char* ub = reinterpret_cast<const char*>(res_tile + ((q >> 1) * a.Wo + (q & 1)) * a.res_cs);
-          rv[q] = __builtin_nontemporal_load(reinterpret_cast<const f32x4*>(ub + lane_res));
-        }
-      }
-    };
-    if (PIPE) request_res();
+    if (PIPE) request_res(tile_pix);
     if (PIPE) {
       mfma_step(0, va, std::true_type(), [&](int pr) {
         if (pr < 3) read_column(vb_, patch, 1, pr + 1);
@@ -266,34 +328,8 @@
     }
     __builtin_amdgcn_sched_barrier(0);
     if (stamp && ns_ < 60) a.dbg[ns_++] = clock64();
-    {
-      if (!PIPE) request_res();
-      f32x4 r0[4], r1[4];
-#pragma unroll
-      for (int py = 0; py < 4; ++py) {
-        r0[py] = pk_add4(pk_add4(acc[py * 4], acc[py * 4 + 1]), acc[py * 4 + 2]);
-        r1[py] = pk_sub4(pk_sub4(acc[py * 4 + 1], acc[py * 4 + 2]), acc[py * 4 + 3]);
-      }
-      f32x4 y[4];
-      y[0] = pk_add4(pk_add4(r0[0], r0[1]), r0[2]);
-      y[1] = pk_add4(pk_add4(r1[0], r1[1]), r1[2]);
-      y[2] = pk_sub4(pk_sub4(r0[1], r0[2]), r0[3]);
-      y[3] = pk_sub4(pk_sub4(r1[1], r1[2]), r1[3]);
-#pragma unroll
-      for (int q = 0; q < 4; ++q) {
-        f32x4 o4 = pk_add4(y[q], bias4);
-        if (has_res) o4 = pk_add4(o4, rv[q]);
-        if (a.relu) {
-          o4[0] = vrelu1(o4[0]); o4[1] = vrelu1(o4[1]); o4[2] = vrelu1(o4[2]); o4[3] = vrelu1(o4[3]);
-        }
-        if constexpr (NSW > 0) {
-          *reinterpret_cast<f32x4*>(stage + (k & 1) * STILE + stage_off + ((q >> 1) * TW + (q & 1)) * 32) = o4;
-        } else {
-          char* ub = reinterpret_cast<char*>(out_tile + ((q >> 1) * a.Wo + (q & 1)) * a.out_cs);
-          __builtin_nontemporal_store(o4, reinterpret_cast<f32x4*>(ub + lane_out));
-        }
-      }
-    }
+    if (!PIPE) request_res(tile_pix);
+    epilogue(k, out_tile);
     __builtin_amdgcn_sched_barrier(0);
     if (!PIPE) {
       read_window(va, patch_next, 0);
@@ -517,11 +553,17 @@
   if (stamp) a.dbg[63] = ns_;
 }
 
-static bool wino3_ok(const ConvArgs& a) {
-  return a.ks == 3 && a.stride == 1 && a.groups == 1 && a.Cin <= 32 && a.Cout == 32 && a.n_tiles == 1 &&
-         a.bias_fstride == 0 && a.Ho % 8 == 0 && a.Wo % 16 == 0 && a.out_cs % 4 == 0 && a.out_coff % 4 == 0 &&
-         a.in_cs % 4 == 0 && a.in_coff % 4 == 0 && (!a.res || (a.res_cs % 4 == 0 && a.res_coff % 4 == 0));
-}
+static int wino3_form(const ConvArgs& a) {
+  if (!(a.ks == 3 && a.stride == 1 && a.groups == 1 && a.Cin <= 32 && a.bias_fstride == 0 && a.Ho % 8 == 0 && a.Wo % 16 == 0 &&
+        a.out_cs % 4 == 0 && a.out_coff % 4 == 0 && a.in_cs % 4 == 0 && a.in_coff % 4 == 0 &&
+        (!a.res || (a.res_cs % 4 == 0 && a.res_coff % 4 == 0))))
+    return -1;
+  if (a.Cout == 32 && a.n_tiles == 1) return 0;
+  if (a.Cout == 16 && a.n_tiles == 1 && a.Ho % 16 == 0 && !a.out2) return 1;
+  if (a.Cout == 64 && a.n_tiles == 2 && a.Cin <= 16 && !a.out2) return 2;
+  return -1;
+}
+static bool wino3_ok(const ConvArgs& a) { return wino3_form(a) >= 0; }
 
 template <int NLW, bool DMA, bool RES>
 static hipError_t launch_wino3b_impl(const ConvArgs& a, hipStream_t s) {
@@ -530,17 +572,41 @@
   return launch_conv_kernel(CONV_KERNEL(conv_wino3b_kernel<NLW, DMA, RES>), (4 + NLW) * 64, lds, a.Wo / 16, a.Ho / 16, 1, a, s);
 }
 
-template <int TH, int NLW, bool PIPE, int LPRIO = 0, bool DMA = false, int NSW = 0, bool DUAL = false>
+template <int TH, int NLW, bool PIPE, int LPRIO = 0, bool DMA = false, int NSW = 0, bool DUAL = false, int FORM = 0>
 static hipError_t launch_wino3_impl(const ConvArgs& a, hipStream_t s) {
-  constexpr size_t lds = (2 * (size_t)(TH + 2) * 18 * 36 + 16 * 2 * 2 * 256 + (NSW > 0 ? 2 * TH * 16 * 32 : 0)) * sizeof(float);
+  constexpr size_t lds = (2 * (size_t)(TH + 2) * 18 * 36 + (FORM == 0 ? 16 * 2 * 2 * 256 : 16 * 2 * 256) +
+                          (NSW > 0 ? 2 * TH * 16 * 32 : 0)) * sizeof(float);
   static_assert(lds <= 160 * 1024, "two patch buffers, the layer's weights and the staging tiles must fit the 160 KiB LDS");
-  return launch_conv_kernel(CONV_KERNEL(conv_wino3_kernel<TH, NLW, PIPE, LPRIO, DMA, NSW, DUAL>), (TH / 2 + NLW + NSW) * 64, lds,
-                            a.Wo / 16, a.Ho / TH, 1, a, s);
+  return launch_conv_kernel(CONV_KERNEL(conv_wino3_kernel<TH, NLW, PIPE, LPRIO, DMA, NSW, DUAL, FORM>),
+                            ((FORM == 1 ? TH / 4 : TH / 2) + NLW + NSW) * 64, lds, a.Wo / 16, a.Ho / TH, 1, a, s);
+}
+
+static hipError_t launch_wino3_one_step(const ConvArgs& a, bool dma_ok, hipStream_t s) {
+  if (dma_ok) return launch_wino3_impl<8, 2, true, 0, true, 2, false, 2>(a, s);
+  return launch_wino3_impl<8, 2, true, 3, false, 0, false, 2>(a, s);
 }
 
 static hipError_t launch_wino3(const ConvArgs& a, hipStream_t s) {
-  if (!wino3_ok(a)) return hipErrorInvalidValue;
+  const int form = wino3_form(a);
+  if (form < 0) return hipErrorInvalidValue;
   const bool dma_ok = conv_dma_ok(a);
+  if (form == 1) {
+    if (dma_ok) return launch_wino3_impl<16, 2, true, 0, true, 0, false, 1>(a, s);
+    return launch_wino3_impl<16, 2, true, 3, false, 0, false, 1>(a, s);
+  }
+  if (form == 2) {
+    for (int blk = 0; blk < 2; ++blk) {
+      ConvArgs b = a;
+      b.w += blk * 512;
+      b.bias += blk * 32;
+      b.out_coff += blk * 32;
+      b.res_coff += blk * 32;
+      const hipError_t e = launch_wino3_one_step(b, dma_ok, s);
+      if (e != hipSuccess) return e;
+    }
+    return hipSuccess;
+  }
+  if (g_force_cfg == 838 && a.Cin <= 16 && !a.out2) return launch_wino3_one_step(a, dma_ok, s);
   if (a.out2) {
     if (!dma_ok || a.nxt < 1 || a.nxt > 3 || a.out2_cs % 4 || a.out2_coff % 4) return hipErrorInvalidValue;
     return launch_wino3_impl<8, 2, true, 0, true, 2, true>(a, s);
diff --git a/arbitrary-hands-3d-reconstruction_amd/ops.py b/arbitrary-hands-3d-reconstruction_amd/ops.py
--- a/arbitrary-hands-3d-reconstruction_amd/ops.py
+++ b/arbitrary-hands-3d-reconstruction_amd/ops.py
@@ -46,18 +46,22 @@
         if k != 3 or stride != 2:
             raise ValueError('the polyphase kernel is for 3x3 stride-2 convolutions')
         tr = polyphase2_weights
-    elif algo in ('winograd', 'winograd2d', 'winograd2d_lds', 'winograd24'):
+    elif algo in ('winograd', 'winograd2d', 'winograd2d_lds', 'winograd2d_lds1', 'winograd24'):
         if k != 3 or stride != 1:
             raise ValueError('winograd needs a 3x3 stride-1 convolution')
         tr = {'winograd': winograd_weights, 'winograd24': winograd24_weights}.get(algo, winograd2d_weights)
     elif algo == 'direct':
         tr = lambda t: t
     else:
-        raise ValueError('algo must be "direct", "winograd", "winograd2d", "winograd2d_lds", "winograd24", "polyphase2", "split16" or "split_bf16"')
-    algo_id = {'direct': 0, 'winograd': 1, 'winograd2d': 2, 'winograd2d_lds': 3, 'winograd24': 4, 'polyphase2': 5, 'split16': 6, 'split_bf16': 7}[algo]
-    if algo_id == 3:
-        if groups != 1 or cout != 32 or cin_g > 32:
-            raise ValueError('winograd2d_lds needs groups = 1, Cout = 32, Cin <= 32')
+        raise ValueError('algo must be "direct", "winograd", "winograd2d", "winograd2d_lds", "winograd2d_lds1", "winograd24", "polyphase2", "split16" or "split_bf16"')
+    algo_id = {'direct': 0, 'winograd': 1, 'winograd2d': 2, 'winograd2d_lds': 3, 'winograd2d_lds1': 3, 'winograd24': 4, 'polyphase2': 5, 'split16': 6, 'split_bf16': 7}[algo]
+    if algo == 'winograd2d_lds1':
+        if groups != 1 or cout != 64 or cin_g > 16:
+            raise ValueError('winograd2d_lds1 needs groups = 1, Cout = 64, Cin <= 16')
+        packed = [pack_wino3(w.astype(np.float64), b)]
+    elif algo_id == 3:
+        if groups != 1 or cout not in (16, 32) or cin_g > 32:
+            raise ValueError('winograd2d_lds needs groups = 1, Cout = 32 (or 16), Cin <= 32')
         packed = [pack_wino3(w.astype(np.float64), b)]
     elif algo_id in (6, 7):
         packed = [pack_conv_x3([(w[g * cout:(g + 1) * cout].astype(np.float64), b[g * cout:(g + 1) * cout]) for g in range(groups)],
diff --git a/arbitrary-hands-3d-reconstruction_amd/packer.py b/arbitrary-hands-3d-reconstruction_amd/packer.py
--- a/arbitrary-hands-3d-reconstruction_amd/packer.py
+++ b/arbitrary-hands-3d-reconstruction_amd/packer.py
@@ -126,13 +126,25 @@
 
 def pack_wino3(w, b):
     cout, cin = w.shape[:2]
-    assert w.shape[2:] == (3, 3) and cout == 32 and cin <= 32
+    assert w.shape[2:] == (3, 3) and ((cout in (16, 32) and cin <= 32) or (cout == 64 and cin <= 16))
+    bp = np.zeros(max(cout, 32), np.float32)
+    bp[:cout] = b
+    if cout == 64:
+        u = np.zeros((64, 16, 4, 4))
+        u[:, :cin] = winograd2d_weights(w)
+        u = u.reshape(2, 2, 16, 4, 4, 4, 4)
+        u = u.transpose(5, 6, 0, 1, 3, 2, 4)
+        return np.ascontiguousarray(u, np.float32).reshape(-1), bp
+    if cout == 16:
+        u = np.zeros((16, 32, 4, 4))
+        u[:, :cin] = winograd2d_weights(w)
+        u = u.reshape(16, 2, 4, 4, 4, 4)
+        u = u.transpose(4, 5, 1, 2, 0, 3)
+        return np.ascontiguousarray(u, np.float32).reshape(-1), bp
     u = np.zeros((32, 32, 4, 4))
     u[:cout, :cin] = winograd2d_weights(w)
     u = u.reshape(2, 16, 2, 4, 4, 4, 4)
     u = u.transpose(5, 6, 2, 0, 3, 1, 4)
-    bp = np.zeros(32, np.float32)
-    bp[:cout] = b
     return np.ascontiguousarray(u, np.float32).reshape(-1), bp
 
 
@@ -235,6 +247,7 @@
 
 
 WINOGRAD_LDS = True
+WINOGRAD_LDS_SIZES = True
 
 
 WINOGRAD_24 = __import__('os').environ.get('ACRMI_WINO24', '1') != '0'
@@ -250,7 +263,11 @@
     return 0
 
 
-def conv_algo(k, stride, cin, cout, groups=1, ho=0, wo=0, per_frame_bias=False, wino24=None, split16=False):
+def wino3_sized(cin, cout, ho, wo):
+    return wo % 16 == 0 and ((cout == 16 and cin <= 32 and ho % 16 == 0) or (cout == 64 and cin <= 16 and ho % 8 == 0))
+
+
+def conv_algo(k, stride, cin, cout, groups=1, ho=0, wo=0, per_frame_bias=False, wino24=None, split16=False, sized=False):
     if split16 and split16_ok(k, stride, cin, cout, ho, wo):
         return 7 if split16 == 'bf16' else 6
     if k == 3 and stride == 2:
@@ -260,6 +277,8 @@
         return 0
     if (WINOGRAD_2D and WINOGRAD_LDS and groups == 1 and cin <= 32 and cout == 32 and ho % 8 == 0 and wo % 16 == 0
             and not per_frame_bias):
+        return 3
+    if (sized and WINOGRAD_2D and WINOGRAD_LDS and groups == 1 and not per_frame_bias and wino3_sized(cin, cout, ho, wo)):
         return 3
     if WINOGRAD_2D and (WINOGRAD_24 if wino24 is None else wino24) and cout != 33:
         if cin > 32 and wo % 32 == 0 and ho % 8 == 0:
@@ -423,7 +442,11 @@
         cin = cin_w if cin is None else cin
         ho, wo = (h + 2 * (k // 2) - k) // stride + 1, (w_ + 2 * (k // 2) - k) // stride + 1
         flop_cout = cout
-        if out is None and out_c is None and len(wb_list) == 1 and k == 3 and stride == 1 and cout < 32 and res is None:
+        sized = (WINOGRAD_LDS_SIZES and self.dt == DT_F32 and bias_map is None and len(wb_list) == 1 and
+                 conv_algo(k, stride, cin, cout, 1, ho, wo, bias_buf is not None, self.wino24, self.split16, sized=True) == 3)
+        if sized and cout == 16:
+            pass
+        elif out is None and out_c is None and len(wb_list) == 1 and k == 3 and stride == 1 and cout < 32 and res is None:
             w0, b0 = wb_list[0]
             wp = np.zeros((32,) + w0.shape[1:], w0.dtype)
             wp[:cout] = w0
@@ -449,7 +472,7 @@
             w_off = self.blob.add16(np.concatenate([p[0] for p in packed]))
         else:
             algo = 2 if slices > 1 else conv_algo(k, stride, cin, cout, len(wb_list), ho, wo, bias_buf is not None, self.wino24,
-                                                    False if ((terms or fp32_kernel) and stride == 2) else self.split16)
+                                                    False if ((terms or fp32_kernel) and stride == 2) else self.split16, sized=sized)
             if algo in (6, 7):
                 packed = [pack_conv_x3(wb_list, DT_BF16 if algo == 7 else DT_F16)]
             elif algo == 3:
```

Result: no change. 2006 frames/s (median of 2 runs) (+0.0%).
